# iden3/circom-witnesscalc

Measured on AMD Instinct MI355X. Metric: witnesses/sec, higher is better.
Workload: dtype u32

## Files before the change

### circom-witnesscalc_amd/__init__.py

```python
import ctypes
import os
import subprocess

import numpy as np

_HERE = os.path.dirname(os.path.abspath(__file__))
LIB_PATH = os.environ.get("CWC_LIB_PATH") or os.path.join(_HERE, "libcircom_witnesscalc_amd.so")
_lib = None


class GwStatus(ctypes.Structure):
    _fields_ = [("code", ctypes.c_int), ("error_msg", ctypes.c_void_p)]


class GraphInfo(ctypes.Structure):
    _fields_ = [(n, ctypes.c_uint64) for n in ("n_nodes", "n_op", "n_input_nodes", "n_const", "n_inputs",
                                                "n_witness", "depth", "algorithmic_bytes_per_set")]


class Timing(ctypes.Structure):
    _fields_ = [("tile_width", ctypes.c_uint32), ("n_launches", ctypes.c_uint32), ("n_bundles", ctypes.c_uint64),
                ("n_slots", ctypes.c_uint64), ("interp_ms", ctypes.c_float), ("pack_ms", ctypes.c_float),
                ("divider", ctypes.c_uint32), ("streams", ctypes.c_uint32)]


class ProgramStats(ctypes.Structure):
    _fields_ = [("tile_width", ctypes.c_uint32), ("divider", ctypes.c_uint32), ("streams", ctypes.c_uint32), ("n_classes", ctypes.c_uint32),
                ("n_bundles", ctypes.c_uint64), ("n_fused_nodes", ctypes.c_uint64), ("class_bundles", ctypes.c_uint64 * 16),
                ("class_nodes", ctypes.c_uint64 * 16), ("model_wave_cycles", ctypes.c_double), ("lanes_active_mean", ctypes.c_double),
                ("values_per_bundle_mean", ctypes.c_double), ("chain_floor_cycles", ctypes.c_double), ("n_scan_steps", ctypes.c_uint64), ("n_conv_products", ctypes.c_uint64)]


CLASS_NAMES = ["INPUT", "MUL", "LIN", "DIV", "CMPZ", "CMPS", "BIT", "IDIVMOD", "TERN", "DIVREQ", "DIVGET", "MULQ", "SYNC", "MULF", "SCAN"]


class E2eStats(ctypes.Structure):
    _fields_ = [("n_sets", ctypes.c_size_t), ("sub_batch", ctypes.c_size_t), ("parse_threads", ctypes.c_uint32), ("write_threads", ctypes.c_uint32),
                ("parse_seconds", ctypes.c_double), ("wait_for_drain_seconds", ctypes.c_double), ("total_seconds", ctypes.c_double),
                ("witness_bytes", ctypes.c_uint64), ("failed_sets", ctypes.c_uint64)]


class Handoff(ctypes.Structure):
    _fields_ = [("struct_size", ctypes.c_uint32), ("form", ctypes.c_uint32), ("hip_stream", ctypes.c_void_p), ("done_event", ctypes.c_void_p)]


FORM_CANONICAL, FORM_MONTGOMERY = 0, 1


class WitnessCalcError(RuntimeError):
    pass


def pinned_rows(shape):
    import weakref
    n = int(np.prod(shape))
    ptr = lib().gwb_host_alloc(n)
    if not ptr:
        raise WitnessCalcError("gwb_host_alloc(%d) failed" % n)
    buf = (ctypes.c_uint8 * max(n, 1)).from_address(ptr)
    weakref.finalize(buf, lib().gwb_host_free, ptr)
    return np.frombuffer(buf, dtype=np.uint8, count=n).reshape(shape)


EXPORTED_SYMBOLS = [
    "gw_calc_witness", "gwb_graph_load", "gwb_graph_free", "gwb_graph_info", "gwb_graph_serialize",
    "gwb_inputs_from_json", "gwb_set_tile_width", "gwb_calc_witness_batch_device", "gwb_calc_witness_batch_host",
    "gwb_last_timing", "gwb_wtns_size", "gwb_wtns_from_witness", "gwb_graph_export", "gwb_graph_import",
    "gwb_free_status", "gwb_profile_classes", "gwb_pick_tile_width", "gwb_inputs_from_json_batch", "gwb_wtns_save_batch",
    "gwb_host_alloc", "gwb_host_free", "gwb_timing_history", "gwb_calc_witness_batch_handoff", "gwb_ubench_modmul", "gwb_graph_pick_tile_width", "gwb_graph_broadcast",
    "gwb_builder_new", "gwb_builder_free", "gwb_builder_input", "gwb_builder_constant", "gwb_builder_uno", "gwb_builder_duo", "gwb_builder_tres",
    "gwb_builder_witness", "gwb_builder_input_signal", "gwb_builder_node_count", "gwb_builder_finish",
    "gwb_ubench_modmul_block", "gwb_program_stats", "gwb_calc_witness_json_to_wtns", "gwb_model_class_cycles",
    "gwb_graphgen_bigint_class", "gwb_graphgen_rsa_long_div_class", "gwb_graph_op_histogram",
    "gwb_kernel_source_hash", "gwb_pack_schedule", "gwb_pack_schedule_of_blob", "gwb_rccl_unique_id", "gwb_rccl_comm_init", "gwb_rccl_comm_ranks", "gwb_rccl_comm_destroy",
    "gwb_wave_census",
]


def build(verbose=False, diag=False):
    cmd = ["make", "-C", os.path.join(_HERE, "csrc"), "-j4"] + (["all", "diag"] if diag else [])
    if not verbose:
        cmd.insert(1, "-s")
    subprocess.check_call(cmd)
    subprocess.check_call(["make"] + ([] if verbose else ["-s"]) + ["-C", os.path.join(_HERE, "r1cs"), "-j4"])


DIAG_LIB_PATH = os.path.join(_HERE, "libcircom_witnesscalc_amd_diag.so")


def lib():
    global _lib
    if _lib is None:
        if not os.path.exists(LIB_PATH):
            raise WitnessCalcError("HIP extension %s is missing: run __graft_entry__.build() "
                                   "(there is no CPU fallback)" % LIB_PATH)
        try:
            import torch
        except ImportError:
            pass
        L = ctypes.CDLL(LIB_PATH)
        vp, sz, u32p = ctypes.c_void_p, ctypes.c_size_t, ctypes.POINTER(ctypes.c_uint32)
        stp = ctypes.POINTER(GwStatus)
        L.gw_calc_witness.restype = ctypes.c_int
        L.gw_calc_witness.argtypes = [ctypes.c_char_p, vp, sz, ctypes.POINTER(vp), ctypes.POINTER(sz), stp]
        L.gwb_graph_load.restype = ctypes.c_int
        L.gwb_graph_load.argtypes = [vp, sz, ctypes.POINTER(vp), stp]
        L.gwb_graph_free.argtypes = [vp]
        L.gwb_graph_info.argtypes = [vp, ctypes.POINTER(GraphInfo)]
        L.gwb_graph_serialize.argtypes = [vp, ctypes.POINTER(vp), ctypes.POINTER(sz), stp]
        L.gwb_inputs_from_json.argtypes = [vp, ctypes.c_char_p, vp, stp]
        L.gwb_set_tile_width.argtypes = [vp, ctypes.c_uint32]
        L.gwb_calc_witness_batch_device.argtypes = [vp, vp, sz, vp, vp, vp, stp]
        L.gwb_calc_witness_batch_host.argtypes = [vp, vp, sz, vp, vp, stp]
        L.gwb_last_timing.argtypes = [vp, ctypes.POINTER(Timing)]
        L.gwb_host_alloc.restype = ctypes.c_void_p
        L.gwb_host_alloc.argtypes = [sz]
        L.gwb_host_free.restype = None
        L.gwb_host_free.argtypes = [ctypes.c_void_p]
        L.gwb_timing_history.restype = ctypes.c_int
        L.gwb_timing_history.argtypes = [ctypes.c_void_p, sz, ctypes.c_void_p, ctypes.c_void_p, ctypes.POINTER(sz)]
        L.gwb_wtns_size.restype = sz
        L.gwb_wtns_size.argtypes = [sz]
        L.gwb_wtns_from_witness.argtypes = [vp, sz, vp]
        L.gwb_graph_export.argtypes = [vp, ctypes.c_uint32, ctypes.POINTER(vp), ctypes.POINTER(sz), stp]
        L.gwb_graph_import.argtypes = [vp, sz, ctypes.POINTER(vp), stp]
        L.gwb_free_status.argtypes = [stp]
        if hasattr(L, "gwb_graphgen_bigint_class"):
            L.gwb_graphgen_bigint_class.argtypes = [ctypes.c_uint32, ctypes.c_uint32, ctypes.c_uint32, ctypes.POINTER(vp), ctypes.POINTER(sz), stp]
            L.gwb_graphgen_rsa_long_div_class.argtypes = [ctypes.c_uint32, ctypes.c_uint32, ctypes.c_uint32, ctypes.c_int, ctypes.POINTER(vp), ctypes.POINTER(sz), stp]
            L.gwb_graph_op_histogram.argtypes = [vp, ctypes.POINTER(ctypes.c_uint64), sz]
        L.gwb_profile_classes.argtypes = [vp, vp, sz, vp, vp, vp, stp]
        if hasattr(L, "gwb_wave_census"):
            L.gwb_wave_census.argtypes = [vp, vp, sz, vp, vp, vp, sz, stp]
        L.gwb_inputs_from_json_batch.argtypes = [vp, ctypes.c_char_p, sz, vp, sz, ctypes.POINTER(sz), stp]
        L.gwb_wtns_save_batch.argtypes = [vp, sz, sz, ctypes.c_char_p, stp]
        L.gwb_calc_witness_batch_handoff.argtypes = [vp, vp, sz, vp, vp, ctypes.POINTER(Handoff), stp]
        L.gwb_ubench_modmul.restype = ctypes.c_double
        L.gwb_ubench_modmul.argtypes = [ctypes.c_uint32, ctypes.c_uint32]
        L.gwb_ubench_modmul_block.restype = ctypes.c_double
        L.gwb_model_class_cycles.restype = ctypes.c_double
        L.gwb_kernel_source_hash.restype = ctypes.c_char_p
        L.gwb_kernel_source_hash.argtypes = []
        L.gwb_model_class_cycles.argtypes = [ctypes.c_uint32]
        L.gwb_ubench_modmul_block.argtypes = [ctypes.c_uint32, ctypes.c_uint32]
        L.gwb_program_stats.argtypes = [vp, ctypes.c_uint32, ctypes.POINTER(ProgramStats)]
        if hasattr(L, "gwb_pack_schedule"):
            L.gwb_pack_schedule.argtypes = [vp, ctypes.c_uint32, vp, sz, vp, sz, u32p, u32p, u32p, stp]
            L.gwb_pack_schedule_of_blob.argtypes = [vp, sz, vp, sz, vp, sz, u32p, u32p, u32p, stp]
        L.gwb_calc_witness_json_to_wtns.argtypes = [vp, ctypes.c_char_p, sz, ctypes.c_char_p, sz, ctypes.POINTER(sz), vp, sz, ctypes.POINTER(E2eStats), stp]
        L.gwb_graph_pick_tile_width.restype = ctypes.c_uint32
        L.gwb_graph_pick_tile_width.argtypes = [vp, sz]
        L.gwb_pick_tile_width.restype = ctypes.c_uint32
        L.gwb_pick_tile_width.argtypes = [sz]
        u32 = ctypes.c_uint32
        L.gwb_builder_new.restype = vp
        L.gwb_builder_new.argtypes = []
        L.gwb_builder_free.restype = None
        L.gwb_builder_free.argtypes = [vp]
        for name, args in (("input", [u32]), ("constant", [ctypes.c_char_p, sz]), ("uno", [u32, u32]), ("duo", [u32, u32, u32]), ("tres", [u32, u32, u32, u32])):
            f = getattr(L, "gwb_builder_" + name)
            f.restype = u32
            f.argtypes = [vp] + args
        L.gwb_builder_witness.argtypes = [vp, u32]
        L.gwb_builder_input_signal.argtypes = [vp, ctypes.c_char_p, u32, u32]
        L.gwb_builder_node_count.restype = ctypes.c_uint64
        L.gwb_builder_node_count.argtypes = [vp]
        L.gwb_builder_finish.argtypes = [vp, ctypes.POINTER(vp), ctypes.POINTER(sz), stp]
        _lib = L
    return _lib


_libc = ctypes.CDLL(None)
_libc.free.argtypes = [ctypes.c_void_p]


def _take_status(st):
    msg = ctypes.string_at(st.error_msg).decode("utf-8", "replace") if st.error_msg else ""
    lib().gwb_free_status(ctypes.byref(st))
    return msg


def _check(rc, st):
    msg = _take_status(st)
    if rc != 0:
        raise WitnessCalcError(msg or "call failed")


def wtns_save_batch(witness, path_pattern):
    witness = np.ascontiguousarray(witness, dtype=np.uint8)
    st = GwStatus()
    rc = lib().gwb_wtns_save_batch(witness.ctypes.data, witness.shape[1], witness.shape[0], path_pattern.encode(), ctypes.byref(st))
    _check(rc, st)


def ubench_modmul(waves_per_simd=4, iters=2000, block=False):
    if block:
        return float(lib().gwb_ubench_modmul_block(waves_per_simd, iters))
    return float(lib().gwb_ubench_modmul(waves_per_simd, iters))


def kernel_source_hash():
    return lib().gwb_kernel_source_hash().decode()


def model_cycles():
    return {n: float(lib().gwb_model_class_cycles(c)) for c, n in enumerate(CLASS_NAMES)}


def graphgen_native(kind, **kw):
    out, n, st = ctypes.c_void_p(), ctypes.c_size_t(), GwStatus()
    L = lib()
    if kind == "bigint":
        rc = L.gwb_graphgen_bigint_class(int(kw.get("k", 8)), int(kw.get("n_bits", 64)), int(kw.get("rounds", 4)), ctypes.byref(out), ctypes.byref(n), ctypes.byref(st))
    elif kind == "rsa":
        rc = L.gwb_graphgen_rsa_long_div_class(int(kw.get("n", 121)), int(kw.get("k", 17)), int(kw.get("muls", 2)), 1 if kw.get("range_checks", True) else 0,
                                               ctypes.byref(out), ctypes.byref(n), ctypes.byref(st))
    else:
        raise ValueError(kind)
    _check(rc, st)
    data = ctypes.string_at(out.value, n.value)
    _libc.free(out)
    return data


def pick_tile_width(batch):
    return int(lib().gwb_pick_tile_width(batch))


def calc_witness_wtns(inputs_json, graph_data):
    if isinstance(inputs_json, str):
        inputs_json = inputs_json.encode("utf-8")
    graph_data = bytes(graph_data)
    out, n, st = ctypes.c_void_p(), ctypes.c_size_t(), GwStatus()
    rc = lib().gw_calc_witness(inputs_json, graph_data, len(graph_data), ctypes.byref(out), ctypes.byref(n),
                               ctypes.byref(st))
    _check(rc, st)
    data = ctypes.string_at(out.value, n.value)
    _libc.free(out)
    return data


def calc_witness(inputs_json, graph_data):
    w = calc_witness_wtns(inputs_json, graph_data)
    body = w[76:]
    return [int.from_bytes(body[i:i + 32], "little") for i in range(0, len(body), 32)]


def wtns_from_witness(witness):
    if not isinstance(witness, np.ndarray):
        witness = np.frombuffer(b"".join(int(x).to_bytes(32, "little") for x in witness), dtype=np.uint8)
    witness = np.ascontiguousarray(witness, dtype=np.uint8).reshape(-1, 32)
    n = witness.shape[0]
    out = np.zeros(lib().gwb_wtns_size(n), dtype=np.uint8)
    if lib().gwb_wtns_from_witness(witness.ctypes.data, n, out.ctypes.data) != 0:
        raise WitnessCalcError("gwb_wtns_from_witness failed")
    return out.tobytes()


class Graph:

    def __init__(self, graph_data=None, _handle=None):
        self._h = ctypes.c_void_p()
        if _handle is not None:
            self._h = _handle
        else:
            graph_data = bytes(graph_data)
            st = GwStatus()
            rc = lib().gwb_graph_load(graph_data, len(graph_data), ctypes.byref(self._h), ctypes.byref(st))
            _check(rc, st)
        info = GraphInfo()
        lib().gwb_graph_info(self._h, ctypes.byref(info))
        for name, _ in GraphInfo._fields_:
            setattr(self, name, int(getattr(info, name)))

    def close(self):
        if getattr(self, "_h", None) and _lib is not None:
            _lib.gwb_graph_free(self._h)
            self._h = None

    __del__ = close

    @classmethod
    def from_blob(cls, blob):
        blob = bytes(blob)
        h, st = ctypes.c_void_p(), GwStatus()
        rc = lib().gwb_graph_import(blob, len(blob), ctypes.byref(h), ctypes.byref(st))
        _check(rc, st)
        return cls(_handle=h)

    def op_histogram(self):
        h = (ctypes.c_uint64 * 24)()
        if lib().gwb_graph_op_histogram(self._h, h, 24) != 0:
            raise WitnessCalcError("gwb_graph_op_histogram failed")
        names = ["Mul", "Div", "Add", "Sub", "Pow", "Idiv", "Mod", "Eq", "Neq", "Lt", "Gt", "Leq", "Geq", "Land", "Lor", "Shl", "Shr", "Bor", "Band", "Bxor",
                 "Neg", "TernCond", "Input", "Const"]
        return dict(sorted(((nm, int(h[i])) for i, nm in enumerate(names) if h[i]), key=lambda kv: -kv[1]))

    def export_blob(self, tile_width):
        out, n, st = ctypes.c_void_p(), ctypes.c_size_t(), GwStatus()
        rc = lib().gwb_graph_export(self._h, tile_width, ctypes.byref(out), ctypes.byref(n), ctypes.byref(st))
        _check(rc, st)
        data = ctypes.string_at(out.value, n.value)
        _libc.free(out)
        return data

    def serialize(self):
        out, n, st = ctypes.c_void_p(), ctypes.c_size_t(), GwStatus()
        rc = lib().gwb_graph_serialize(self._h, ctypes.byref(out), ctypes.byref(n), ctypes.byref(st))
        _check(rc, st)
        data = ctypes.string_at(out.value, n.value)
        _libc.free(out)
        return data

    def pick_tile_width(self, batch):
        key = int(lib().gwb_graph_pick_tile_width(self._h, batch))
        if key == 0:
            raise WitnessCalcError("gwb_graph_pick_tile_width failed")
        return key

    def set_tile_width(self, t):
        if lib().gwb_set_tile_width(self._h, t) != 0:
            raise WitnessCalcError("tile width must be 0 or a power of two in 1..64")

    def inputs_from_json(self, inputs_json):
        if isinstance(inputs_json, str):
            inputs_json = inputs_json.encode("utf-8")
        row = np.zeros((self.n_inputs, 32), dtype=np.uint8)
        st = GwStatus()
        rc = lib().gwb_inputs_from_json(self._h, inputs_json, row.ctypes.data, ctypes.byref(st))
        _check(rc, st)
        return row

    def inputs_from_json_batch(self, text):
        if isinstance(text, str):
            text = text.encode("utf-8")
        n = ctypes.c_size_t()
        st = GwStatus()
        lib().gwb_inputs_from_json_batch(self._h, text, len(text), None, 0, ctypes.byref(n), ctypes.byref(st))
        msg = _take_status(st)
        if "rows buffer too small" not in msg and msg:
            raise WitnessCalcError(msg)
        rows = np.zeros((n.value, self.n_inputs, 32), dtype=np.uint8)
        st = GwStatus()
        rc = lib().gwb_inputs_from_json_batch(self._h, text, len(text), rows.ctypes.data, n.value, ctypes.byref(n), ctypes.byref(st))
        _check(rc, st)
        return rows

    def json_to_wtns(self, text, path_pattern, first_index=0, with_status=True):
        if isinstance(text, str):
            text = text.encode("utf-8")
        n = ctypes.c_size_t()
        cap = max(1, text.count(b"\n") + 1, text.count(b"{"))
        status = np.zeros(cap, dtype=np.uint32)
        es, st = E2eStats(), GwStatus()
        rc = lib().gwb_calc_witness_json_to_wtns(self._h, text, len(text), path_pattern.encode(), first_index, ctypes.byref(n),
                                                  status.ctypes.data if with_status else None, cap if with_status else 0,
                                                  ctypes.byref(es), ctypes.byref(st))
        _check(rc, st)
        return status[:n.value], {k: getattr(es, k) for k, _ in E2eStats._fields_}

    def calc_witness_batch(self, inputs, out=None):
        inputs = np.ascontiguousarray(inputs, dtype=np.uint8)
        b = inputs.shape[0]
        assert inputs.shape[1:] == (self.n_inputs, 32), inputs.shape
        if out is None:
            wit = np.empty((b, self.n_witness, 32), dtype=np.uint8)
        else:
            wit = out
            assert wit.dtype == np.uint8 and wit.shape == (b, self.n_witness, 32) and wit.flags["C_CONTIGUOUS"]
        status = np.zeros(b, dtype=np.uint32)
        st = GwStatus()
        rc = lib().gwb_calc_witness_batch_host(self._h, inputs.ctypes.data, b, wit.ctypes.data, status.ctypes.data,
                                               ctypes.byref(st))
        _check(rc, st)
        return wit, status

    def calc_witness_batch_device(self, d_inputs, d_witness, d_status, stream=None, montgomery=False, done_event=None):
        import torch
        b = d_inputs.shape[0]
        assert d_inputs.is_cuda and d_witness.is_cuda and d_status.is_cuda
        assert d_inputs.is_contiguous() and d_witness.is_contiguous() and d_status.is_contiguous()
        assert tuple(d_inputs.shape[1:]) == (self.n_inputs, 32) and tuple(d_witness.shape) == (b, self.n_witness, 32)
        s = stream if stream is not None else torch.cuda.current_stream()
        st = GwStatus()
        if montgomery or done_event is not None:
            if done_event is not None:
                done_event.record(s)
            h = Handoff(ctypes.sizeof(Handoff), FORM_MONTGOMERY if montgomery else FORM_CANONICAL, s.cuda_stream,
                        done_event.cuda_event if done_event is not None else None)
            rc = lib().gwb_calc_witness_batch_handoff(self._h, d_inputs.data_ptr(), b, d_witness.data_ptr(), d_status.data_ptr(),
                                                      ctypes.byref(h), ctypes.byref(st))
        else:
            rc = lib().gwb_calc_witness_batch_device(self._h, d_inputs.data_ptr(), b, d_witness.data_ptr(),
                                                     d_status.data_ptr(), s.cuda_stream, ctypes.byref(st))
        _check(rc, st)

    def timing_history(self, max_launches):
        a = np.zeros(max_launches, dtype=np.float32)
        b = np.zeros(max_launches, dtype=np.float32)
        n = ctypes.c_size_t(0)
        if lib().gwb_timing_history(self._h, max_launches, a.ctypes.data, b.ctypes.data, ctypes.byref(n)) != 0:
            raise WitnessCalcError("gwb_timing_history failed")
        return a[:n.value], b[:n.value]

    def profile_classes(self, d_inputs, d_witness, d_status):
        out = np.zeros(96, dtype=np.uint64)
        st = GwStatus()
        rc = lib().gwb_profile_classes(self._h, d_inputs.data_ptr(), d_inputs.shape[0], d_witness.data_ptr(),
                                       d_status.data_ptr(), out.ctypes.data, ctypes.byref(st))
        _check(rc, st)
        names = ["INPUT", "MUL", "LIN", "DIV", "CMPZ", "CMPS", "BIT", "IDIVMOD", "TERN", "DIVREQ", "DIVGET", "MULQ"]
        res = {n: tuple(int(x) for x in out[4 * i:4 * i + 4]) for i, n in enumerate(names)}
        res["MULF"] = tuple(int(x) for x in out[64:68])
        res["SCAN"] = tuple(int(x) for x in out[68:72])
        res["_scan_kinds"] = {k: tuple(int(x) for x in out[72 + 4 * i:76 + 4 * i]) for i, k in enumerate(("carry", "division", "convolution", "borrow", "comparison"))}
        res["_sections"] = {"MUL": tuple(int(x) for x in out[48:54]), "LIN": tuple(int(x) for x in out[56:62])}
        res["_issue_part"] = {"MUL": int(out[92]), "LIN": int(out[93])}
        res["_pack"] = {"cycles": int(out[94]), "passes": int(out[95])}
        n = int(out[63])
        res["_waves"] = {"n": n, "max_cycles": int(out[54]), "min_cycles": (1 << 40) - int(out[55]) if n else 0,
                         "mean_cycles": int(out[62]) // n if n else 0}
        return res

    def wave_census(self, d_inputs, d_witness, d_status):
        out = np.zeros(3 * 8192, dtype=np.uint64)
        st = GwStatus()
        rc = lib().gwb_wave_census(self._h, d_inputs.data_ptr(), d_inputs.shape[0], d_witness.data_ptr(),
                                   d_status.data_ptr(), out.ctypes.data, out.size, ctypes.byref(st))
        _check(rc, st)
        rec = out.reshape(-1, 3)
        idx = [i for i in range(rec.shape[0]) if rec[i, 1]]
        res = []
        for i in idx:
            w0 = int(rec[i, 0])
            role, wpw = (w0 >> 40) & 255, (w0 >> 48) & 255
            res.append({"workgroup": i // wpw, "wave": i % wpw, "xcc": (w0 >> 32) & 15, "se": (w0 >> 13) & 7, "sh": (w0 >> 12) & 1, "cu": (w0 >> 8) & 15, "simd": (w0 >> 4) & 3,
                        "divider": role & 1, "stream": (role >> 1) & 7, "has_tile": (role >> 4) & 1, "start": int(rec[i, 1]), "end": int(rec[i, 2])})
        return res

    def program_stats(self, key=0):
        ps = ProgramStats()
        if lib().gwb_program_stats(self._h, key, ctypes.byref(ps)) != 0:
            raise WitnessCalcError("gwb_program_stats: no such program")
        n = ps.n_classes
        return {"tile_width": ps.tile_width, "divider": ps.divider, "streams": ps.streams, "n_bundles": ps.n_bundles,
                "n_fused_nodes": ps.n_fused_nodes, "n_scan_steps": ps.n_scan_steps, "n_conv_products": ps.n_conv_products, "chain_floor_cycles": ps.chain_floor_cycles, "model_wave_cycles": ps.model_wave_cycles, "lanes_active_mean": ps.lanes_active_mean, "values_per_bundle_mean": ps.values_per_bundle_mean,
                "class_bundles": {CLASS_NAMES[c]: int(ps.class_bundles[c]) for c in range(n) if ps.class_bundles[c]},
                "class_nodes": {CLASS_NAMES[c]: int(ps.class_nodes[c]) for c in range(n) if ps.class_nodes[c]}}

    def pack_schedule(self, key):
        return _pack_schedule(lambda *a: lib().gwb_pack_schedule(self._h, key, *a))

    def last_timing(self):
        t = Timing()
        if lib().gwb_last_timing(self._h, ctypes.byref(t)) != 0:
            raise WitnessCalcError("gwb_last_timing failed")
        return {n: getattr(t, n) for n, _ in Timing._fields_}


def _pack_schedule(call):
    nw, nr, ni, st = ctypes.c_uint32(), ctypes.c_uint32(), ctypes.c_uint32(), GwStatus()
    _check(call(None, 0, None, 0, ctypes.byref(nw), ctypes.byref(nr), ctypes.byref(ni), ctypes.byref(st)), st)
    order, ready = np.zeros(nw.value, dtype=np.uint32), np.zeros(nr.value, dtype=np.uint32)
    _check(call(order.ctypes.data, order.size, ready.ctypes.data, ready.size, ctypes.byref(nw), ctypes.byref(nr), ctypes.byref(ni), ctypes.byref(st)), st)
    return order, ready, int(ni.value)


def pack_schedule_of_blob(blob):
    blob = bytes(blob)
    return _pack_schedule(lambda *a: lib().gwb_pack_schedule_of_blob(blob, len(blob), *a))


R1CS_LIB_PATH = os.environ.get("CWC_R1CS_LIB_PATH") or os.path.join(_HERE, "libcwc_r1cs.so")
R1CS_SATISFIED = 0xFFFFFFFF
_r1cs_lib = None


class R1csInfo(ctypes.Structure):
    _fields_ = [(n, ctypes.c_uint32) for n in ("n_wires", "n_pub_out", "n_pub_in", "n_prv_in", "n_constraints")] + \
               [(n, ctypes.c_uint64) for n in ("n_labels", "n_factors_a", "n_factors_b", "n_factors_c")]


class R1csQapInfo(ctypes.Structure):
    _fields_ = [("n_rows", ctypes.c_uint64), ("domain_power", ctypes.c_uint32), ("domain_size", ctypes.c_uint64),
                ("workspace_bytes_per_row", ctypes.c_uint64)]


class ZkeyInfo(ctypes.Structure):
    _fields_ = [("n_vars", ctypes.c_uint32), ("n_public", ctypes.c_uint32), ("domain_size", ctypes.c_uint32), ("n_coefs", ctypes.c_uint64)]


class PtauInfo(ctypes.Structure):
    _fields_ = [("power", ctypes.c_uint32), ("ceremony_power", ctypes.c_uint32), ("prepared", ctypes.c_uint32),
                ("n_contributions", ctypes.c_uint32)]


def r1cs_lib():
    global _r1cs_lib
    if _r1cs_lib is None:
        if not os.path.exists(R1CS_LIB_PATH):
            raise WitnessCalcError("R1CS library %s is missing: run __graft_entry__.build()" % R1CS_LIB_PATH)
        try:
            import torch
        except ImportError:
            pass
        L = ctypes.CDLL(R1CS_LIB_PATH)
        vp, sz, u32 = ctypes.c_void_p, ctypes.c_size_t, ctypes.c_uint32
        stp = ctypes.POINTER(GwStatus)
        L.gwb_r1cs_load.argtypes = [vp, sz, ctypes.POINTER(vp), stp]
        L.gwb_r1cs_free.restype = None
        L.gwb_r1cs_free.argtypes = [vp]
        L.gwb_r1cs_info.argtypes = [vp, ctypes.POINTER(R1csInfo)]
        L.gwb_r1cs_set_tile_width.argtypes = [vp, u32]
        L.gwb_r1cs_check_batch_device.argtypes = [vp, vp, sz, sz, u32, vp, vp, vp, stp]
        L.gwb_r1cs_check_batch_host.argtypes = [vp, vp, sz, sz, vp, vp, stp]
        L.gwb_r1cs_check_wtns.argtypes = [vp, vp, sz, vp, vp, stp]
        L.gwb_r1cs_qap_info.argtypes = [vp, ctypes.POINTER(R1csQapInfo), stp]
        L.gwb_r1cs_qap_batch_device.argtypes = [vp, vp, sz, sz, u32, vp, u32, vp, stp]
        L.gwb_r1cs_qap_batch_host.argtypes = [vp, vp, sz, sz, vp, u32, stp]
        L.gwb_r1cs_qap_wtns.argtypes = [vp, vp, sz, vp, u32, stp]
        L.gwb_r1cs_qap_time_phases.argtypes = [vp, ctypes.c_int]
        L.gwb_r1cs_qap_phase_ms.argtypes = [vp, ctypes.POINTER(ctypes.c_float)]
        L.gwb_r1cs_modmul_rate.argtypes = [ctypes.POINTER(ctypes.c_double)]
        L.gwb_zkey_load.argtypes = [vp, sz, ctypes.POINTER(vp), stp]
        L.gwb_zkey_free.restype = None
        L.gwb_zkey_free.argtypes = [vp]
        L.gwb_zkey_info.argtypes = [vp, ctypes.POINTER(ZkeyInfo)]
        L.gwb_groth16_prove_batch_device.argtypes = [vp, vp, vp, sz, sz, u32, vp, vp, vp, stp]
        L.gwb_groth16_prove_batch_host.argtypes = [vp, vp, vp, sz, sz, vp, vp, stp]
        L.gwb_groth16_prove_wtns.argtypes = [vp, vp, vp, sz, vp, vp, stp]
        L.gwb_groth16_time_phases.argtypes = [vp, ctypes.c_int]
        L.gwb_groth16_phase_ms.argtypes = [vp, ctypes.POINTER(ctypes.c_float)]
        L.gwb_zkey_qap_info.argtypes = [vp, ctypes.POINTER(R1csQapInfo), stp]
        L.gwb_zkey_qap_batch_device.argtypes = [vp, vp, sz, sz, u32, vp, u32, vp, stp]
        L.gwb_zkey_qap_batch_host.argtypes = [vp, vp, sz, sz, vp, u32, stp]
        L.gwb_zkey_set_tile_width.argtypes = [vp, u32]
        L.gwb_zkey_check_r1cs.argtypes = [vp, vp, stp]
        L.gwb_g16vk_from_zkey.argtypes = [vp, ctypes.POINTER(vp), stp]
        L.gwb_g16vk_load.argtypes = [vp, sz, u32, ctypes.POINTER(vp), stp]
        L.gwb_g16vk_info.argtypes = [vp, ctypes.POINTER(ctypes.c_uint32)]
        L.gwb_g16vk_points.argtypes = [vp, vp, sz]
        L.gwb_g16vk_alphabeta.argtypes = [vp, vp, stp]
        L.gwb_g16vk_free.restype = None
        L.gwb_g16vk_free.argtypes = [vp]
        L.gwb_groth16_verify_batch_device.argtypes = [vp, vp, vp, sz, sz, vp, vp, stp]
        L.gwb_groth16_verify_batch_host.argtypes = [vp, vp, vp, sz, sz, vp, stp]
        L.gwb_bn254_pairing_batch_device.argtypes = [vp, vp, sz, vp, vp, stp]
        L.gwb_groth16_setup.argtypes = [vp, vp, ctypes.POINTER(vp), ctypes.POINTER(sz), stp]
        L.gwb_groth16_setup_free.restype = None
        L.gwb_groth16_setup_free.argtypes = [vp]
        L.gwb_bn254_gen_mul_batch_device.argtypes = [vp, sz, u32, vp, vp, stp]
        L.gwb_groth16_setup_phase_ms.argtypes = [ctypes.POINTER(ctypes.c_float)]
        L.gwb_ptau_info.argtypes = [vp, sz, ctypes.POINTER(PtauInfo), stp]
        L.gwb_ptau_check.argtypes = [vp, sz, u32, u32, stp]
        L.gwb_groth16_setup_ptau.argtypes = [vp, vp, sz, vp, u32, ctypes.POINTER(vp), ctypes.POINTER(sz), stp]
        L.gwb_bn254_point_idft_batch_device.argtypes = [vp, u32, u32, vp, vp, stp]
        L.gwb_groth16_setup_ptau_phase_ms.argtypes = [ctypes.POINTER(ctypes.c_float)]
        L.gwb_bn254_g2_check_batch_device.argtypes = [vp, sz, u32, u32, vp, vp, stp]
        L.gwb_zkey_check_g2.argtypes = [vp, stp]
        L.gwb_zkey_check_wtns.argtypes = [vp, vp, sz, stp]
        L.gwb_ptau_check_g2.argtypes = [vp, sz, u32, u32, stp]
        L.gwb_groth16_contribute.argtypes = [vp, sz, ctypes.c_char_p, vp, ctypes.POINTER(vp), ctypes.POINTER(sz), vp, stp]
        L.gwb_groth16_contribute_phase_ms.argtypes = [ctypes.POINTER(ctypes.c_float)]
        L.gwb_zkey_verify_contributions.argtypes = [vp, sz, vp, ctypes.POINTER(sz), stp]
        L.gwb_zkey_verify_step.argtypes = [vp, sz, vp, sz, vp, stp]
        L.gwb_zkey_contributions.argtypes = [vp, sz, ctypes.POINTER(vp), ctypes.POINTER(sz), stp]
        L.gwb_blake2b512.restype = None
        L.gwb_blake2b512.argtypes = [vp, sz, vp]
        L.gwb_zkey_contribution_challenge.restype = None
        L.gwb_zkey_contribution_challenge.argtypes = [vp, vp]
        L.gwb_bn254_g1_scale_batch_device.argtypes = [vp, sz, vp, vp, vp, stp]
        L.gwb_bn254_g1_lincomb128_device.argtypes = [vp, vp, sz, vp, vp, stp]
        _r1cs_lib = L
    return _r1cs_lib


def _r1cs_check(rc, st):
    msg = ctypes.string_at(st.error_msg).decode("utf-8", "replace") if st.error_msg else ""
    if st.error_msg:
        _libc.free(st.error_msg)
    if rc != 0:
        raise WitnessCalcError(msg or "call failed")


def modmul_rate():
    rate = ctypes.c_double()
    if r1cs_lib().gwb_r1cs_modmul_rate(ctypes.byref(rate)) != 0:
        raise WitnessCalcError("gwb_r1cs_modmul_rate failed")
    return rate.value


def _qap_info(h, src):
    info = R1csQapInfo()
    st = GwStatus()
    rc = getattr(r1cs_lib(), "gwb_%s_qap_info" % src)(h, ctypes.byref(info), ctypes.byref(st))
    _r1cs_check(rc, st)
    return {n: int(getattr(info, n)) for n, _ in R1csQapInfo._fields_}


def _qap_batch(h, src, witness_rows, montgomery_out):
    if isinstance(witness_rows, tuple):
        witness_rows = witness_rows[0]
    w = np.ascontiguousarray(witness_rows, dtype=np.uint8)
    assert w.ndim == 3 and w.shape[2] == 32, w.shape
    b = w.shape[0]
    out = np.zeros((b, _qap_info(h, src)["domain_size"], 32), dtype=np.uint8)
    st = GwStatus()
    rc = getattr(r1cs_lib(), "gwb_%s_qap_batch_host" % src)(h, w.ctypes.data, w.shape[1], b, out.ctypes.data,
                                                            FORM_MONTGOMERY if montgomery_out else FORM_CANONICAL, ctypes.byref(st))
    _r1cs_check(rc, st)
    return out


def _qap_batch_device(h, src, d_witness, stream, montgomery, montgomery_out):
    import torch
    assert d_witness.is_cuda and d_witness.is_contiguous() and d_witness.dtype == torch.uint8
    assert d_witness.dim() == 3 and d_witness.shape[2] == 32, tuple(d_witness.shape)
    b = d_witness.shape[0]
    n = _qap_info(h, src)["domain_size"]
    s = stream if stream is not None else torch.cuda.current_stream(d_witness.device)
    out = torch.empty((b, n, 32), dtype=torch.uint8, device=d_witness.device)
    st = GwStatus()
    with torch.cuda.device(d_witness.device):
        rc = getattr(r1cs_lib(), "gwb_%s_qap_batch_device" % src)(h, d_witness.data_ptr(), d_witness.shape[1], b,
                                                                  FORM_MONTGOMERY if montgomery else FORM_CANONICAL, out.data_ptr(),
                                                                  FORM_MONTGOMERY if montgomery_out else FORM_CANONICAL, s.cuda_stream,
                                                                  ctypes.byref(st))
    _r1cs_check(rc, st)
    if b:
        out.record_stream(s)
    return out


class R1cs:

    def __init__(self, data):
        self._h = ctypes.c_void_p()
        data = bytes(data)
        st = GwStatus()
        rc = r1cs_lib().gwb_r1cs_load(data, len(data), ctypes.byref(self._h), ctypes.byref(st))
        _r1cs_check(rc, st)
        info = R1csInfo()
        r1cs_lib().gwb_r1cs_info(self._h, ctypes.byref(info))
        self.info = {n: int(getattr(info, n)) for n, _ in R1csInfo._fields_}

    def close(self):
        if getattr(self, "_h", None) and _r1cs_lib is not None:
            _r1cs_lib.gwb_r1cs_free(self._h)
            self._h = None

    __del__ = close

    def set_tile_width(self, t):
        if r1cs_lib().gwb_r1cs_set_tile_width(self._h, t) != 0:
            raise WitnessCalcError("tile width must be 0 or a power of two in 1..64")

    def check_batch(self, witness_rows):
        if isinstance(witness_rows, tuple):
            witness_rows = witness_rows[0]
        w = np.ascontiguousarray(witness_rows, dtype=np.uint8)
        assert w.ndim == 3 and w.shape[2] == 32, w.shape
        b = w.shape[0]
        first = np.zeros(b, dtype=np.uint32)
        nfail = np.zeros(b, dtype=np.uint32)
        st = GwStatus()
        rc = r1cs_lib().gwb_r1cs_check_batch_host(self._h, w.ctypes.data, w.shape[1], b, first.ctypes.data, nfail.ctypes.data, ctypes.byref(st))
        _r1cs_check(rc, st)
        return first, nfail

    def check_batch_device(self, d_witness, stream=None, montgomery=False):
        import torch
        assert d_witness.is_cuda and d_witness.is_contiguous() and d_witness.dtype == torch.uint8
        assert d_witness.dim() == 3 and d_witness.shape[2] == 32, tuple(d_witness.shape)
        b = d_witness.shape[0]
        s = stream if stream is not None else torch.cuda.current_stream(d_witness.device)
        first = torch.empty(b, dtype=torch.int32, device=d_witness.device)
        nfail = torch.empty(b, dtype=torch.int32, device=d_witness.device)
        st = GwStatus()
        with torch.cuda.device(d_witness.device):
            rc = r1cs_lib().gwb_r1cs_check_batch_device(self._h, d_witness.data_ptr(), d_witness.shape[1], b,
                                                        FORM_MONTGOMERY if montgomery else FORM_CANONICAL, first.data_ptr(),
                                                        nfail.data_ptr(), s.cuda_stream, ctypes.byref(st))
        _r1cs_check(rc, st)
        return first, nfail

    def check_wtns(self, wtns):
        wtns = bytes(wtns)
        first, nfail = ctypes.c_uint32(), ctypes.c_uint32()
        st = GwStatus()
        rc = r1cs_lib().gwb_r1cs_check_wtns(self._h, wtns, len(wtns), ctypes.byref(first), ctypes.byref(nfail), ctypes.byref(st))
        _r1cs_check(rc, st)
        return int(first.value), int(nfail.value)

    def qap_info(self):
        return _qap_info(self._h, "r1cs")

    def qap_batch(self, witness_rows, montgomery_out=False):
        return _qap_batch(self._h, "r1cs", witness_rows, montgomery_out)

    def qap_batch_device(self, d_witness, stream=None, montgomery=False, montgomery_out=False):
        return _qap_batch_device(self._h, "r1cs", d_witness, stream, montgomery, montgomery_out)

    def qap_time_phases(self, on=True):
        if r1cs_lib().gwb_r1cs_qap_time_phases(self._h, 1 if on else 0) != 0:
            raise WitnessCalcError("gwb_r1cs_qap_time_phases failed")

    def qap_phase_ms(self):
        ms = (ctypes.c_float * 4)()
        if r1cs_lib().gwb_r1cs_qap_phase_ms(self._h, ms) != 0:
            raise WitnessCalcError("no QAP phase times (qap_time_phases not on, or no QAP call yet)")
        return dict(zip(("evaluation", "inverse_outer", "fused_inner", "forward_outer"), (float(x) for x in ms)))

    def qap_wtns(self, wtns, montgomery_out=False):
        wtns = bytes(wtns)
        h = np.zeros((self.qap_info()["domain_size"], 32), dtype=np.uint8)
        st = GwStatus()
        rc = r1cs_lib().gwb_r1cs_qap_wtns(self._h, wtns, len(wtns), h.ctypes.data,
                                          FORM_MONTGOMERY if montgomery_out else FORM_CANONICAL, ctypes.byref(st))
        _r1cs_check(rc, st)
        return h



GROTH16_PROOF_BYTES = 256
GROTH16_PHASES = ("witness_map", "scalars_sort", "g1_msms", "g2_msm", "assembly")


def _rs_array(rs, b):
    if rs is None:
        return None
    if isinstance(rs, np.ndarray):
        a = np.ascontiguousarray(rs, dtype=np.uint8)
    else:
        a = np.frombuffer(b"".join(int(x).to_bytes(32, "little") for pair in rs for x in pair), dtype=np.uint8).copy()
    assert a.size == b * 64, "rs must hold [batch][2][32 B]"
    return a


def _dec(b):
    return str(int.from_bytes(bytes(b), "little"))


def proof_json(proof):
    p = bytes(proof)
    c = [_dec(p[32 * k:32 * k + 32]) for k in range(8)]
    z = lambda lo, hi: "1" if any(p[lo:hi]) else "0"
    return {"pi_a": [c[0], c[1], z(0, 64)], "pi_b": [[c[2], c[3]], [c[4], c[5]], [z(64, 192), "0"]],
            "pi_c": [c[6], c[7], z(192, 256)], "protocol": "groth16", "curve": "bn128"}


class Groth16:

    def __init__(self, zkey_bytes, r1cs=None, check_g2=False):
        self._h = ctypes.c_void_p()
        self.r1cs = r1cs
        data = bytes(zkey_bytes)
        st = GwStatus()
        rc = r1cs_lib().gwb_zkey_load(data, len(data), ctypes.byref(self._h), ctypes.byref(st))
        _r1cs_check(rc, st)
        info = ZkeyInfo()
        r1cs_lib().gwb_zkey_info(self._h, ctypes.byref(info))
        self.info = {n: int(getattr(info, n)) for n, _ in ZkeyInfo._fields_}
        if check_g2:
            self.check_g2()

    def close(self):
        if getattr(self, "_h", None) and _r1cs_lib is not None:
            _r1cs_lib.gwb_zkey_free(self._h)
            self._h = None

    __del__ = close

    def _r1cs_handle(self):
# ... 577 lines not shown
```

### circom-witnesscalc_amd/csrc/kernels.hip

```cpp
#include <hip/hip_runtime.h>
#include <stdlib.h>

#include "fr_gfx950.hpp"
#include "scan_gfx950.hpp"
#include "program_dev.h"

namespace cwc {

__device__ __forceinline__ Fr fr_from_u4(const uint4& lo, const uint4& hi) {
    return Fr{{lo.x, lo.y, lo.z, lo.w, hi.x, hi.y, hi.z, hi.w}};
}

__device__ __forceinline__ bool wave_any(bool p) { return __ballot(p) != 0ull; }

struct InterpDims {
    uint32_t n_bundles, n_slots, n_inputs, batch, n_const, n_div_requests, trash_off;
    const uint32_t* div_lanes;
    uint32_t n_streams, stream_first[MAX_STREAMS], stream_count[MAX_STREAMS], stream_div_requests[MAX_STREAMS], stream_cref_first[MAX_STREAMS];
    uint4* pack_out;
    const uint2* pack_entries;
    const uint32_t* pack_ready;
    uint32_t n_inline, pack_mont, n_witness;
};
static const uint32_t ST_DIVIDER_TIMEOUT = 0x80000000u;
static const uint32_t ST_SYNC_TIMEOUT = 0x40000000u;

__device__ __forceinline__ bool mbox_wait(const volatile uint32_t* seq, uint32_t need) {
    for (uint32_t spins = 0; spins < (1u << 22); ++spins) {
        if (*seq >= need) return true;
        __builtin_amdgcn_s_sleep(8);
    }
    return false;
}
__device__ __noinline__ bool post_wait(uint32_t* word, uint32_t need) {
#pragma nounroll
    for (uint32_t spins = 0; spins < (1u << 22); ++spins) {
        if (__hip_atomic_load(word, __ATOMIC_ACQUIRE, __HIP_MEMORY_SCOPE_AGENT) >= need) return true;
        __builtin_amdgcn_s_sleep(8);
    }
    return false;
}
typedef uint32_t u32x4 __attribute__((ext_vector_type(4)));
typedef int i32x4 __attribute__((ext_vector_type(4)));
typedef __attribute__((address_space(3))) char lds_char;

__device__ __forceinline__ void dma16(uint32_t lds_addr, uint32_t voff, const i32x4& rsrc, uint32_t soff) {
    asm volatile("s_mov_b32 m0, %0\n\ts_nop 0\n\tbuffer_load_dwordx4 %1, %2, %3 offen lds"
                 :: "s"(lds_addr), "v"(voff), "s"(rsrc), "s"(soff) : "memory");
}
__device__ __forceinline__ i32x4 make_rsrc_words(const void* base, uint32_t bytes) {
    const uint64_t a = (uint64_t)base;
    return i32x4{(int)(uint32_t)a, (int)((uint32_t)(a >> 32) & 0xffffu), (int)bytes, 0x00020000};
}

template <int T, bool PROF, int W, int PACK, int MODE = 0>
__global__ __launch_bounds__((W > 0 ? (W + 1) * PACK : PACK) * 64) void interp_kernel(const uint32_t* __restrict__ hdr, const uint4* __restrict__ recs,
                                                    const uint32_t* __restrict__ crefs, InterpDims p, WsTable wst,
                                                    const uint4* __restrict__ inputs, uint32_t* __restrict__ status,
                                                    unsigned long long* __restrict__ prof) {
    constexpr int G = 64 / T;
    constexpr bool M2 = MODE == 2 || MODE == 3, WIDE = MODE == 3;
    constexpr uint32_t HI = 16u * T;
    constexpr bool DIVIDER = W > 0;
    constexpr uint32_t NW = (W > 0 ? (uint32_t)W : 1u) * (uint32_t)PACK;
    constexpr uint32_t WD = W > 0 ? (uint32_t)W : 1u;
    constexpr uint32_t AREA = lds_area_bytes((uint32_t)W, LDS_BYTES);
    constexpr uint32_t ML = mbox_lanes((uint32_t)W), MB = mbox_bytes((uint32_t)W);
    const uint32_t batch = p.batch;
    const uint32_t lane = threadIdx.x & 63u;
    const uint32_t wave = (uint32_t)__builtin_amdgcn_readfirstlane((int)(threadIdx.x >> 6));
    const uint32_t n_tiles = (batch + T - 1) / T;
    const uint32_t t = lane % T;
    const uint32_t j = (G == 1) ? 0u : lane / T;
    const uint32_t NS = p.n_streams;
    const uint32_t stream = wave < NW ? wave % NS : 0u;
    const uint32_t tile_raw = blockIdx.x * (NW / NS) + (wave < NW ? wave : 0u) / NS;
    const uint32_t tile = tile_raw < n_tiles ? tile_raw : n_tiles - 1;
    const uint32_t set = tile * T + t;
    const uint32_t set_c = set < batch ? set : batch - 1;
    [[maybe_unused]] auto census_slot = [&]() -> unsigned long long* {
        const uint32_t wv = blockIdx.x * (blockDim.x >> 6) + wave;
        return lane == 0 && wv < CENSUS_MAX_WAVES ? prof + PROF_WORDS + CENSUS_WORDS * wv : nullptr;
    };
    if constexpr (PROF) {
        if (unsigned long long* c = census_slot()) {
            const uint32_t w_of = wave < NW ? wave : (wave - NW) * WD;
            const uint32_t has_tile = blockIdx.x * (NW / NS) + w_of / NS < n_tiles ? 1u : 0u;
            const unsigned long long role = (wave >= NW ? 1u : 0u) | (w_of % NS) << 1 | has_tile << 4 | (blockDim.x >> 6) << 8;
            constexpr int HWREG_HW_ID = 4 | 31 << 11, HWREG_XCC_ID = 20 | 31 << 11;
            c[0] = (unsigned long long)__builtin_amdgcn_s_getreg(HWREG_HW_ID) | (unsigned long long)(__builtin_amdgcn_s_getreg(HWREG_XCC_ID) & 15u) << 32 | role << 40;
            c[1] = __builtin_amdgcn_s_memtime();
        }
    }
    const uint64_t tile_bytes = ws_tile_bytes(p.n_const, p.n_slots, T);
    const uint32_t chunk = tile / wst.tiles_per_chunk, tile_in_chunk = tile % wst.tiles_per_chunk;
    char* tile_base = reinterpret_cast<char*>(wst.base[chunk]) + (uint64_t)tile_in_chunk * tile_bytes;
    const __amdgpu_buffer_rsrc_t rsrc = __builtin_amdgcn_make_buffer_rsrc(tile_base, 0, (int)(uint32_t)tile_bytes, 0x00020000);
    const i32x4 rsrc_rec = make_rsrc_words(recs, (p.n_bundles + REC_AHEAD) * (uint32_t)G * 16u);
    uint32_t* const sync_words = reinterpret_cast<uint32_t*>(tile_base + ws_sync_offset(p.n_const, p.n_slots, T));
    static_assert(NW + PACK <= 16, "sequence words: 64 bytes");
    __shared__ uint4 lds[(NW * AREA + (DIVIDER ? NW * MB + 64u : 0u)) / 16];
    const uint32_t area = wave * AREA;
    const uint32_t lds0 = (uint32_t)(uintptr_t)(lds_char*)(char*)lds + area;
    const uint32_t t16 = 16u * t, lane16 = 16u * lane, j16 = 16u * j;
    char* const ldsb = reinterpret_cast<char*>(lds) + area;
    char* const mbox_all = reinterpret_cast<char*>(lds) + NW * AREA;
    char* const mbox = mbox_all + (wave < NW ? wave : 0u) * MB;
    volatile uint32_t* const seq = reinterpret_cast<volatile uint32_t*>(mbox_all + NW * MB);
    if (DIVIDER || NW > 1) {
        if (DIVIDER && threadIdx.x < NW + (uint32_t)PACK) seq[threadIdx.x] = 0;
        if (NS > 1 && wave < NW && stream == 0 && lane < MAX_STREAMS && tile_raw < n_tiles) {
            __hip_atomic_store(sync_words + lane, 0u, __ATOMIC_RELAXED, __HIP_MEMORY_SCOPE_AGENT);
            __builtin_amdgcn_fence(__ATOMIC_RELEASE, "agent");
        }
        if (wave < NW && stream == 0 && j == 0 && tile_raw < n_tiles && set < batch) status[set] = 0;
        __syncthreads();
    } else {
        if (j == 0 && tile_raw < n_tiles && set < batch) status[set] = 0;
    }
    if (DIVIDER) {
        if (wave >= NW) {
            const uint32_t first_w = (wave - NW) * WD, first_tile = blockIdx.x * (NW / NS) + first_w / NS;
            if (first_tile >= n_tiles) return;
            const uint32_t n_active = NS > 1 ? 1u : n_tiles - first_tile < WD ? n_tiles - first_tile : WD;
            char* const mbox_d = mbox_all + first_w * MB;
            const uint32_t n_requests = NS > 1 ? p.stream_div_requests[first_w % NS] : p.n_div_requests;
            uint32_t div_lanes_base = 0;
            for (uint32_t q = 0; NS > 1 && q < first_w % NS; ++q) div_lanes_base += p.stream_div_requests[q];
            [[maybe_unused]] uint32_t pk_next = 0;
            [[maybe_unused]] uint2 pk_e0 = make_uint2(0u, 0u), pk_e1 = pk_e0;
            [[maybe_unused]] unsigned long long pk_cycles = 0, pk_passes = 0;
            const bool inl = W == 1 && NS == 1 && p.n_inline > 0;
            const char* const pk_tile = reinterpret_cast<const char*>(wst.base[first_tile / wst.tiles_per_chunk]) + (uint64_t)(first_tile % wst.tiles_per_chunk) * tile_bytes;
            const uint32_t pk_set = first_tile * T + t;
            auto pk_load = [&](const uint2& e, uint4& lo, uint4& hi) {
                const uint32_t ref = e.y & ~REF_CANON;
                const uint32_t slot = (ref & REF_CONST) ? (ref & ~REF_CONST) : p.n_const + ref;
                const uint4* q = reinterpret_cast<const uint4*>(pk_tile) + (size_t)slot * (2 * T);
                lo = q[t];
                hi = q[T + t];
            };
            auto pk_store = [&](const uint2& e, const uint4& lo, const uint4& hi, uint32_t limit) {
                const bool valid = pk_next + j < limit && pk_set < batch, canon = (e.y & REF_CANON) != 0;
                const Fr v = fr_from_u4(lo, hi);
                Fr c = v;
                if (p.pack_mont) {
                    if (wave_any(both(valid, canon))) c = u256_select(canon, fr_mul(v, fr_r2()), v);
                } else {
                    if (wave_any(both(valid, !canon))) c = u256_select(canon, v, fr_from_mont(v));
                }
                if (valid) {
                    uint4* o = p.pack_out + ((size_t)pk_set * p.n_witness + e.x) * 2;
                    o[0] = make_uint4(c.v[0], c.v[1], c.v[2], c.v[3]);
                    o[1] = make_uint4(c.v[4], c.v[5], c.v[6], c.v[7]);
                }
            };
            auto pk_run = [&](uint32_t limit, uint32_t need) {
                if (pk_next >= limit) return;
                unsigned long long t0 = 0;
                if (PROF) t0 = __builtin_amdgcn_s_memtime();
                uint4 lo, hi;
                pk_load(pk_e0, lo, hi);
                for (;;) {
                    const uint32_t nb = pk_next + (uint32_t)G;
                    const bool more = nb < limit && seq[first_w] < need;
                    uint4 lo1 = lo, hi1 = hi;
                    if (more) pk_load(pk_e1, lo1, hi1);
                    const uint2 e2 = p.pack_entries[nb + (uint32_t)G + j];
                    pk_store(pk_e0, lo, hi, limit);
                    pk_next = nb;
                    pk_e0 = pk_e1;
                    pk_e1 = e2;
                    if (PROF) ++pk_passes;
                    if (!more) break;
                    lo = lo1;
                    hi = hi1;
                }
                if (PROF) pk_cycles += __builtin_amdgcn_s_memtime() - t0;
            };
            if constexpr (W == 1) {
                if (inl) {
                    pk_e0 = p.pack_entries[j];
                    pk_e1 = p.pack_entries[(uint32_t)G + j];
                }
            }
            for (uint32_t k = 0; k < n_requests; ++k) {
                if constexpr (W == 1) {
                    if (inl) {
                        const uint32_t lim = p.pack_ready[k] < p.n_inline ? p.pack_ready[k] : p.n_inline;
                        pk_run(lim / (uint32_t)G * (uint32_t)G, k + 1);
                    }
                }
                bool ok = true;
                for (uint32_t w = 0; w < n_active; ++w) ok = ok && mbox_wait(seq + first_w + w, k + 1);
                if (!ok) {
                    if (first_tile * T + t < batch) atomicOr(&status[first_tile * T + t], ST_DIVIDER_TIMEOUT);
                    break;
                }
                __builtin_amdgcn_fence(__ATOMIC_ACQUIRE, "workgroup");
                const uint32_t lanes_k = p.div_lanes[div_lanes_base + k];
                const uint32_t total = n_active * lanes_k;
                for (uint32_t g0 = 0; g0 < total; g0 += 64u) {
                    const uint32_t g = g0 + lane;
                    const bool valid = g < total;
                    const uint32_t w = valid ? g / lanes_k : 0u, i = valid ? g % lanes_k : 0u;
                    char* mb = mbox_d + w * MB + 16u * i;
                    const uint4* qa = reinterpret_cast<const uint4*>(mb);
                    const uint4* qb = reinterpret_cast<const uint4*>(mb + 32u * ML);
                    Fr a = fr_from_u4(qa[0], qa[ML]), b = fr_from_u4(qb[0], qb[ML]);
                    if (!valid) b = fr_zero();
                    const Fr inv = fr_inv(b);
                    const Fr r = u256_select(u256_is_zero(b), fr_zero(), fr_mul(a, inv));
                    if (valid) {
                        uint4* qr = reinterpret_cast<uint4*>(mb);
                        qr[0] = make_uint4(r.v[0], r.v[1], r.v[2], r.v[3]);
                        qr[ML] = make_uint4(r.v[4], r.v[5], r.v[6], r.v[7]);
                    }
                }
                __builtin_amdgcn_fence(__ATOMIC_RELEASE, "workgroup");
                if (lane == 0) seq[wave] = k + 1;
            }
            if constexpr (W == 1) {
                if (inl) {
                    pk_run(p.pack_ready[n_requests] < p.n_inline ? p.pack_ready[n_requests] : p.n_inline, 0xffffffffu);
                    if (PROF && lane == 0 && first_tile % 64u == 0) {
                        atomicAdd(&prof[94], pk_cycles);
                        atomicAdd(&prof[95], pk_passes);
                    }
                }
            }
            if constexpr (PROF) {
                if (unsigned long long* c = census_slot()) c[2] = __builtin_amdgcn_s_memtime();
            }
            return;
        }
    }
    if (tile_raw >= n_tiles) return;
    uint32_t div_seq = 0;
    uint32_t n_posts = 0, n_waits = 0;
    uint32_t cref_row = p.stream_cref_first[stream];

    auto ld = [&](uint32_t off) -> Fr {
        const u32x4 lo = __builtin_amdgcn_raw_buffer_load_b128(rsrc, (int)off, 0, 0);
        const u32x4 hi = __builtin_amdgcn_raw_buffer_load_b128(rsrc, (int)off + (int)HI, 0, 0);
        return Fr{{lo.x, lo.y, lo.z, lo.w, hi.x, hi.y, hi.z, hi.w}};
    };
    auto ld_lds = [&](uint32_t addr) -> Fr {
        const uint4* q = reinterpret_cast<const uint4*>(ldsb + addr);
        const uint4 lo = q[0], hi = q[LDS_HALF_BYTES / 16];
        return fr_from_u4(lo, hi);
    };
    auto ld_rec2 = [&](uint32_t bundle, uint32_t half) -> uint2 {
        return *reinterpret_cast<const uint2*>(ldsb + LDS_REC_OFF + (bundle % REC_AHEAD) * REC_BYTES + lane16 + 8u * half);
    };
    const uint32_t B0 = p.stream_first[stream], NBND = B0 + p.stream_count[stream];
    if (NBND == B0) return;
    auto clampb = [&](uint32_t b) { return b < NBND ? b : NBND - 1; };
    auto stage_rec = [&](uint32_t bundle) {
        dma16(lds0 + LDS_REC_OFF + (bundle % REC_AHEAD) * REC_BYTES, j16, rsrc_rec, bundle * (uint32_t)G * 16u);
    };
    constexpr uint32_t DMA_BIAS = 3u * LDS_HALF_BYTES;
    const i32x4 rsrc_dma = make_rsrc_words(tile_base - DMA_BIAS, (uint32_t)tile_bytes + DMA_BIAS);
    const uint32_t dma_soff0 = DMA_BIAS, dma_soff1 = DMA_BIAS + HI - LDS_HALF_BYTES, dma_soff2 = DMA_BIAS - 2u * LDS_HALF_BYTES,
                   dma_soff3 = DMA_BIAS + HI - 3u * LDS_HALF_BYTES;
    static_assert(LDS_HALF_BYTES == 1024, "instruction offsets below are written out");
    auto stage_operands = [&](uint32_t bundle, const uint2& offs) {
        const uint32_t s = lds0 + LDS_STAGE_OFF + (bundle % OPND_AHEAD) * STAGE_BYTES;
        const uint32_t ao = offs.x + t16, bo = offs.y + t16;
        asm volatile("s_mov_b32 m0, %0\n\ts_nop 0\n\t"
                     "buffer_load_dwordx4 %1, %3, %4 offen lds\n\t"
                     "buffer_load_dwordx4 %1, %3, %5 offen offset:1024 lds\n\t"
                     "buffer_load_dwordx4 %2, %3, %6 offen offset:2048 lds\n\t"
                     "buffer_load_dwordx4 %2, %3, %7 offen offset:3072 lds"
                     :: "s"(s), "v"(ao), "v"(bo), "s"(rsrc_dma), "s"(dma_soff0), "s"(dma_soff1), "s"(dma_soff2), "s"(dma_soff3) : "memory");
    };
    uint32_t err_bits = 0;
    Fr pv = fr_p();
#pragma unroll
    for (int i = 0; i < 8; ++i) asm volatile("" : "+v"(pv.v[i]));
    constexpr bool COOP = (uint32_t)T <= COOP_MAX_T;
    const uint32_t cq = lane & 3u, cv = lane >> 2;
    const uint32_t t16c = 16u * (cv % T);
    const uint32_t coop_chunk = (cq >> 1) * LDS_HALF_BYTES + (cq & 1u) * 8u;
    const uint32_t coop_ring_off = 16u * cv + coop_chunk;
    const uint32_t coop_dst_off = t16c + (cq >> 1) * HI + (cq & 1u) * 8u;
    uint32_t nq0 = cq == 0 ? CWC_P0 : cq == 1 ? CWC_P2 : cq == 2 ? CWC_P4 : CWC_P6;
    uint32_t nq1 = cq == 0 ? CWC_P1 : cq == 1 ? CWC_P3 : cq == 2 ? CWC_P5 : CWC_P7;
    asm volatile("" : "+v"(nq0), "+v"(nq1));
    const uint32_t trash_doff = p.trash_off | t16;
    constexpr int C_PROF = 12;
    unsigned long long pf[C_PROF][2], psec[2][7] = {{0, 0, 0, 0, 0, 0, 0}, {0, 0, 0, 0, 0, 0, 0}};
    unsigned long long pf_fused[2] = {0, 0};
    unsigned long long pf_scan[5][2] = {{0, 0}, {0, 0}, {0, 0}, {0, 0}, {0, 0}};
    if (PROF) {
#pragma unroll
        for (int c = 0; c < C_PROF; ++c) pf[c][0] = pf[c][1] = 0;
    }
#define CWC_STAMP(var) unsigned long long var = 0; if (PROF) asm volatile("s_memtime %0\n\ts_waitcnt lgkmcnt(0)" : "=s"(var)::"memory")
#define CWC_SHADOW_ISSUE()                                                                                                                  \
    stage_rec(b + 4);                                                                                                                       \
    __builtin_amdgcn_raw_buffer_store_b128(u32x4{r_prev.v[0], r_prev.v[1], r_prev.v[2], r_prev.v[3]}, rsrc, (int)doff_prev, 0, 0);          \
    __builtin_amdgcn_raw_buffer_store_b128(u32x4{r_prev.v[4], r_prev.v[5], r_prev.v[6], r_prev.v[7]}, rsrc, (int)doff_prev + (int)HI, 0, 0)
#define CWC_NEXT_HEADER(var)                                                                                                                 \
    asm volatile("s_mov_b32 %0, xnack_mask_lo\n\ts_load_dword xnack_mask_lo, %1, %2" : "=&s"(var) : "s"(hdr), "s"(hdr_off_n2) : "memory"); \
    hdr_off_n2 += 4u

    static_assert(OPND_AHEAD == 2 && REC_AHEAD == 4, "the counted waits below are written for this pipeline depth");
#pragma unroll
    for (uint32_t q = 0; q < REC_AHEAD; ++q) stage_rec(B0 + q);
    asm volatile("s_waitcnt vmcnt(0)" ::: "memory");
    stage_operands(B0, ld_rec2(B0, 0));
    stage_operands(B0 + 1, ld_rec2(B0 + 1, 0));
    uint2 rec_hi = ld_rec2(B0, 1);
    uint2 rec_hi_n1 = ld_rec2(B0 + 1, 1);
    uint32_t h_cur = hdr[B0], h_n1 = hdr[clampb(B0 + 1)];
    asm volatile("s_waitcnt vmcnt(0)" ::: "memory");
    const unsigned long long t_wave0 = PROF ? __builtin_amdgcn_s_memtime() : 0ull;
    asm volatile("s_load_dword xnack_mask_lo, %0, %1\n\ts_waitcnt lgkmcnt(0)" :: "s"(hdr), "s"(4u * B0 + 8u) : "memory");
    uint32_t hdr_off_n2 = 4u * B0 + 12u;
    Fr r_prev = fr_zero();
    uint32_t doff_prev = trash_doff;
    for (uint32_t b = B0; b < NBND; ++b) {
        CWC_STAMP(st0);
        const uint32_t h = h_cur;
        asm volatile("s_waitcnt vmcnt(7)" ::: "memory");
        CWC_STAMP(st1);
        if constexpr (COOP) {
            uint32_t cls_q = h & HDR_CLASS_MASK;
            asm volatile("" : "+s"(cls_q));
            static_assert(C_MULQ == 11 && C_SYNC == 12 && C_MULF == 13 && C_SCAN == 14 && C_COUNT == 15, "one compare (class >= C_MULQ) leads to the narrow classes");
            const bool narrow_cls = MODE == 1 ? cls_q >= C_MULQ : cls_q == C_MULQ;
            if (M2 ? __builtin_expect(narrow_cls, 0) : narrow_cls) {
            if (MODE != 1 || cls_q == C_MULQ) {
                const uint32_t la = rec_hi.y + (t16c | (t16c << 16));
                const Fr a_op = ld_lds(la & 0xffffu);
                const uint2 bq = *reinterpret_cast<const uint2*>(ldsb + (la >> 16) + coop_chunk);
                const uint2 aq = *reinterpret_cast<const uint2*>(ldsb + (la & 0xffffu) + coop_chunk);
                const uint4 rec_full_n2 = *reinterpret_cast<const uint4*>(ldsb + LDS_REC_OFF + ((b + 2) % REC_AHEAD) * REC_BYTES + lane16);
                const uint2 rec_n2 = make_uint2(rec_full_n2.x, rec_full_n2.y), rec_hi_n2 = make_uint2(rec_full_n2.z, rec_full_n2.w);
                CWC_SHADOW_ISSUE();
                asm volatile("s_waitcnt lgkmcnt(0)" :: "v"(a_op.v[0]), "v"(a_op.v[4]), "v"(bq.x), "v"(aq.x), "v"(rec_n2.x), "v"(rec_hi_n2.x) : "memory");
                uint32_t h_n2;
                CWC_NEXT_HEADER(h_n2);
                CWC_STAMP(st2);
                stage_operands(b + 2, rec_n2);
                CWC_STAMP(st3);
                uint32_t out[2];
                if (h & (HDR_LIN_ADD | HDR_LIN_SUB)) {
                    fr_mul_coop4r(a_op, aq.x, aq.y, bq.x, bq.y, nq0, nq1, rec_hi.x & CTRL_SUB_MASK, out);
                } else {
                    fr_mul_coop4(a_op, bq.x, bq.y, nq0, nq1, out);
                }
                CWC_STAMP(st4);
                *reinterpret_cast<uint2*>(ldsb + LDS_RING_OFF + (b % RING_BUNDLES) * RING_SLOT_BYTES + coop_ring_off) = make_uint2(out[0], out[1]);
                {
                    typedef uint32_t u32x2 __attribute__((ext_vector_type(2)));
                    __builtin_amdgcn_raw_buffer_store_b64(u32x2{out[0], out[1]}, rsrc, (int)((rec_hi.x & ~CTRL_MASK) + coop_dst_off), 0, 0);
                }
                doff_prev = trash_doff;
                rec_hi = rec_hi_n1;
                rec_hi_n1 = rec_hi_n2;
                h_cur = h_n1;
                h_n1 = h_n2;
                __builtin_amdgcn_fence(__ATOMIC_ACQ_REL, "wavefront");
                if (PROF) {
                    asm volatile("s_waitcnt lgkmcnt(0)" ::: "memory");
                    const unsigned long long t_now = __builtin_amdgcn_s_memtime();
                    pf[C_MULQ][0] += t_now - st0;
                    pf[C_MULQ][1] += 1;
                    (void)st2; (void)st3; (void)st4;
                }
                continue;
            }
            if constexpr (MODE == 1 && (uint32_t)T <= COOP_FUSE_MAX_T) {
            if (cls_q == C_MULF) {
                constexpr int QP_MAIN = T == 1 ? 0xA0  : 0x00 , QP_EXTRA = T == 1 ? 0xF5  : 0xAA ;
                const uint32_t mx = (uint32_t)__builtin_amdgcn_mov_dpp((int)rec_hi.x, QP_MAIN, 0xf, 0xf, false);
                const uint32_t my = (uint32_t)__builtin_amdgcn_mov_dpp((int)rec_hi.y, QP_MAIN, 0xf, 0xf, false);
                const uint32_t xx = (uint32_t)__builtin_amdgcn_mov_dpp((int)rec_hi.x, QP_EXTRA, 0xf, 0xf, false);
                const uint32_t xy = (uint32_t)__builtin_amdgcn_mov_dpp((int)rec_hi.y, QP_EXTRA, 0xf, 0xf, false);
                const uint32_t la = my + (t16c | (t16c << 16)), lx = xy + (t16c | (t16c << 16));
                const Fr a_op = ld_lds(la & 0xffffu);
                const uint2 bq = *reinterpret_cast<const uint2*>(ldsb + (la >> 16) + coop_chunk);
                const Fr x2_full = ld_lds(lx & 0xffffu);
                const uint2 x2q = *reinterpret_cast<const uint2*>(ldsb + (lx & 0xffffu) + coop_chunk);
                const uint2 x3q = *reinterpret_cast<const uint2*>(ldsb + (lx >> 16) + coop_chunk);
                const uint4 rec_full_n2 = *reinterpret_cast<const uint4*>(ldsb + LDS_REC_OFF + ((b + 2) % REC_AHEAD) * REC_BYTES + lane16);
                const uint2 rec_n2 = make_uint2(rec_full_n2.x, rec_full_n2.y), rec_hi_n2 = make_uint2(rec_full_n2.z, rec_full_n2.w);
                CWC_SHADOW_ISSUE();
                asm volatile("s_waitcnt lgkmcnt(0)" :: "v"(a_op.v[0]), "v"(a_op.v[4]), "v"(bq.x), "v"(x2_full.v[0]), "v"(x2_full.v[4]), "v"(x2q.x), "v"(x3q.x), "v"(rec_n2.x), "v"(rec_hi_n2.x) : "memory");
                uint32_t h_n2;
                CWC_NEXT_HEADER(h_n2);
                stage_operands(b + 2, rec_n2);
                uint32_t out[2];
                fr_mul_coop4(a_op, bq.x, bq.y, nq0, nq1, out);
                const uint32_t op2 = mx & CTRL_SUB_MASK, op3 = xx & CTRL_SUB_MASK;
                if (h & HDR_F_S2MUL) {
                    uint32_t o2[2];
                    fr_mul_coop4(x2_full, out[0], out[1], nq0, nq1, o2);
                    out[0] = op2 == FOP_MUL ? o2[0] : out[0];
                    out[1] = op2 == FOP_MUL ? o2[1] : out[1];
                }
                auto lin_stage = [&](uint32_t op, const uint2& xq) {
                    const bool rs = op == FOP_RSUB;
                    uint32_t o[2];
                    fr_addsub_coop4(rs ? xq.x : out[0], rs ? xq.y : out[1], rs ? out[0] : xq.x, rs ? out[1] : xq.y, nq0, nq1, op == FOP_ADD ? 0u : 1u, o);
                    out[0] = op >= FOP_ADD ? o[0] : out[0];
                    out[1] = op >= FOP_ADD ? o[1] : out[1];
                };
                if (h & HDR_F_S2LIN) lin_stage(op2, x2q);
                if (h & HDR_F_S3LIN) lin_stage(op3, x3q);
                *reinterpret_cast<uint2*>(ldsb + LDS_RING_OFF + (b % RING_BUNDLES) * RING_SLOT_BYTES + coop_ring_off) = make_uint2(out[0], out[1]);
                {
                    typedef uint32_t u32x2 __attribute__((ext_vector_type(2)));
                    __builtin_amdgcn_raw_buffer_store_b64(u32x2{out[0], out[1]}, rsrc, (int)((mx & ~CTRL_MASK) + coop_dst_off), 0, 0);
                }
                doff_prev = trash_doff;
                rec_hi = rec_hi_n1;
                rec_hi_n1 = rec_hi_n2;
                h_cur = h_n1;
                h_n1 = h_n2;
                __builtin_amdgcn_fence(__ATOMIC_ACQ_REL, "wavefront");
                if (PROF) {
                    asm volatile("s_waitcnt lgkmcnt(0)" ::: "memory");
                    const unsigned long long t_now = __builtin_amdgcn_s_memtime();
                    pf_fused[0] += t_now - st0;
                    pf_fused[1] += 1;
                }
                continue;
            }
            }
            }
        }
        const uint32_t ctrl = rec_hi.x & CTRL_MASK;
        const uint32_t doff = (rec_hi.x & ~CTRL_MASK) | t16;
        const uint32_t la = rec_hi.y + (t16 | (t16 << 16));
        const Fr a_op = ld_lds(la & 0xffffu), b_op = ld_lds(la >> 16);
        const uint4 rec_full_n2 = *reinterpret_cast<const uint4*>(ldsb + LDS_REC_OFF + ((b + 2) % REC_AHEAD) * REC_BYTES + lane16);
        const uint2 rec_n2 = make_uint2(rec_full_n2.x, rec_full_n2.y), rec_hi_n2 = make_uint2(rec_full_n2.z, rec_full_n2.w);
        CWC_SHADOW_ISSUE();
        unsigned long long st_iss = 0;
        if (PROF) st_iss = __builtin_amdgcn_s_memtime();
        uint32_t h_n2;
        unsigned long long st2 = 0, st3 = 0;
        auto wait_and_stage = [&]() {
            asm volatile("s_waitcnt lgkmcnt(0)" :: "v"(a_op.v[0]), "v"(a_op.v[4]), "v"(b_op.v[0]), "v"(b_op.v[4]), "v"(rec_n2.x), "v"(rec_hi_n2.x) : "memory");
            CWC_NEXT_HEADER(h_n2);
            if (PROF) asm volatile("s_memtime %0\n\ts_waitcnt lgkmcnt(0)" : "=s"(st2)::"memory");
            stage_operands(b + 2, rec_n2);
            if (PROF) asm volatile("s_memtime %0\n\ts_waitcnt lgkmcnt(0)" : "=s"(st3)::"memory");
        };

        const uint32_t cls = h & HDR_CLASS_MASK;
        uint32_t cls_hot = cls, cls_hot2 = cls;
        asm volatile("" : "+s"(cls_hot));
        asm volatile("" : "+s"(cls_hot2));
        const bool active = (ctrl & CTRL_ACTIVE) != 0;
        const uint32_t sub = ctrl & CTRL_SUB_MASK;
        auto finish = [&](const Fr& r) {
            CWC_STAMP(st4);
            r_prev = r;
            doff_prev = doff;
            {
                uint4* q = reinterpret_cast<uint4*>(ldsb + LDS_RING_OFF + (b % RING_BUNDLES) * RING_SLOT_BYTES + lane16);
                q[0] = make_uint4(r.v[0], r.v[1], r.v[2], r.v[3]);
                q[LDS_HALF_BYTES / 16] = make_uint4(r.v[4], r.v[5], r.v[6], r.v[7]);
            }
            rec_hi = rec_hi_n1;
            rec_hi_n1 = rec_hi_n2;
            h_cur = h_n1;
            h_n1 = h_n2;
            __builtin_amdgcn_fence(__ATOMIC_ACQ_REL, "wavefront");
            if (PROF) {
                asm volatile("s_waitcnt lgkmcnt(0)" ::: "memory");
                const unsigned long long t_now = __builtin_amdgcn_s_memtime();
    #pragma unroll
                for (int c = 0; c < C_PROF; ++c)
                    if (cls == (uint32_t)c) {
                        pf[c][0] += t_now - st0;
                        pf[c][1] += 1;
                    }
                if (M2 && cls == C_SCAN) {
                    pf_fused[0] += t_now - st0;
                    pf_fused[1] += 1;
                    const int kind = (h & HDR_SCAN_CONV) ? 2 : (h & HDR_SCAN_BORROW) ? 3 : (h & HDR_SCAN_LEX) ? 4 : (h & HDR_SCAN_DIV) ? 1 : 0;
#pragma unroll
                    for (int q = 0; q < 5; ++q)
                        if (kind == q) {
                            pf_scan[q][0] += t_now - st0;
                            pf_scan[q][1] += 1;
                        }
                }
                if (cls == C_MUL || cls == C_LIN) {
                    unsigned long long* q = psec[cls == C_MUL ? 0 : 1];
                    q[0] += st1 - st0;
                    q[1] += st2 - st1;
                    q[2] += st3 - st2;
                    q[3] += st4 - st3;
                    q[4] += t_now - st4;
                    q[5] += 1;
                    q[6] += st_iss - st1;
                }
            }
        };
        Fr r;
        auto one_out = [&]() -> Fr { return (h & HDR_OUT_CANON) ? Fr{{1u, 0u, 0u, 0u, 0u, 0u, 0u, 0u}} : fr_one(); };
        if (cls_hot2 == C_LIN) {
            wait_and_stage();
            if (!(h & HDR_LIN_SUB)) {
                r = fr_add_wave(a_op, b_op, pv);
            } else if (!(h & HDR_LIN_ADD)) {
                r = fr_sub_wave(a_op, b_op, pv);
            } else {
                const unsigned long long subm = __ballot(sub == SUB_SUB);
                r = fr_addsub_wave(a_op, b_op, pv, sub == SUB_SUB ? ~0u : 0u, subm, ~subm);
            }
            finish(r);
            continue;
        }
        wait_and_stage();
        if (__builtin_expect(cls_hot == C_MUL, WIDE ? 0 : 1)) {
            if constexpr (M2) {
                if (h & HDR_MUL_CC) {
                    auto limb_product = [&](const Fr& x, const Fr& y) -> Fr {
                        const uint64_t p00 = (uint64_t)x.v[0] * y.v[0], p01 = (uint64_t)x.v[0] * y.v[1], p10 = (uint64_t)x.v[1] * y.v[0], p11 = (uint64_t)x.v[1] * y.v[1];
                        const uint64_t m1 = (p00 >> 32) + (uint32_t)p01 + (uint32_t)p10;
                        const uint64_t m2 = (m1 >> 32) + (p01 >> 32) + (p10 >> 32) + (uint32_t)p11;
                        Fr z = fr_zero();
                        z.v[0] = (uint32_t)p00;
                        z.v[1] = (uint32_t)m1;
                        z.v[2] = (uint32_t)m2;
                        z.v[3] = (uint32_t)((m2 >> 32) + (p11 >> 32));
                        return z;
                    };
                    const uint32_t hi_a = a_op.v[2] | a_op.v[3] | a_op.v[4] | a_op.v[5] | a_op.v[6] | a_op.v[7], hi_b = b_op.v[2] | b_op.v[3] | b_op.v[4] | b_op.v[5] | b_op.v[6] | b_op.v[7];
                    if (!wave_any((hi_a | hi_b) != 0u)) {
                        r = limb_product(a_op, b_op);
                    } else if (WIDE && !wave_any(((a_op.v[3] | b_op.v[3]) >> 30 | a_op.v[4] | a_op.v[5] | a_op.v[6] | a_op.v[7] | b_op.v[4] | b_op.v[5] | b_op.v[6] | b_op.v[7]) != 0u)) {
                        uint32_t z[8] = {0, 0, 0, 0, 0, 0, 0, 0};
#pragma unroll
                        for (int i = 0; i < 4; ++i) {
                            uint32_t carry = 0;
#pragma unroll
                            for (int jj = 0; jj < 4; ++jj) {
                                const uint64_t t = (uint64_t)a_op.v[i] * b_op.v[jj] + z[i + jj] + carry;
                                z[i + jj] = (uint32_t)t;
                                carry = (uint32_t)(t >> 32);
                            }
                            z[i + 4] = carry;
                        }
#pragma unroll
                        for (int k = 0; k < 8; ++k) r.v[k] = z[k];
                    } else {
                        Fr na, nb;
                        (void)u256_sub(na, fr_p(), a_op);
                        (void)u256_sub(nb, fr_p(), b_op);
                        const bool a_neg = hi_a != 0u, b_neg = hi_b != 0u;
                        const Fr ma = u256_select(a_neg, na, a_op), mb = u256_select(b_neg, nb, b_op);
                        if (!wave_any((ma.v[2] | ma.v[3] | ma.v[4] | ma.v[5] | ma.v[6] | ma.v[7] | mb.v[2] | mb.v[3] | mb.v[4] | mb.v[5] | mb.v[6] | mb.v[7]) != 0u)) {
                            const Fr z = limb_product(ma, mb);
                            Fr nz;
                            (void)u256_sub(nz, fr_p(), z);
                            r = u256_select(both(a_neg != b_neg, !u256_is_zero(z)), nz, z);
                        } else {
                            r = fr_mul_wave(fr_mul_wave(a_op, fr_r2(), pv), b_op, pv);
                        }
                    }
                    finish(r);
                    continue;
                }
            }
            r = fr_mul_wave(a_op, b_op, pv);
            if ((h & (HDR_LIN_ADD | HDR_LIN_SUB)) == (HDR_LIN_ADD | HDR_LIN_SUB)) {
                const unsigned long long subm = __ballot(sub == SUB_SUB);
                r = u256_select(sub <= SUB_SUB, fr_addsub_wave(a_op, b_op, pv, sub == SUB_SUB ? ~0u : 0u, subm, ~subm), r);
            } else if (h & HDR_LIN_ADD) {
                r = u256_select(sub == SUB_ADD, fr_add_wave(a_op, b_op, pv), r);
            } else if (h & HDR_LIN_SUB) {
                r = u256_select(sub == SUB_SUB, fr_sub_wave(a_op, b_op, pv), r);
            }
            finish(r);
            continue;
        }
        if constexpr (M2 && (uint32_t)T <= SCAN_MAX_T) {
            uint32_t cls_scan = cls;
            asm volatile("" : "+s"(cls_scan));
            if (WIDE ? __builtin_expect(cls_scan == C_SCAN, 1) : (cls_scan == C_SCAN)) {
                r = fr_zero();
                if constexpr (M2 && (uint32_t)T <= SCAN_MAX_T) {
                    if (h & HDR_SCAN_CONV) {
                        const uint32_t k = (h >> HDR_SCAN_ITER_SHIFT) + 1u;
                        const bool holds_y = active && lane < k * (uint32_t)T;
                        if (!wave_any(both(active, (a_op.v[2] | a_op.v[3] | a_op.v[4] | a_op.v[5] | a_op.v[6] | a_op.v[7] | b_op.v[2] | b_op.v[3] | b_op.v[4] | b_op.v[5] | b_op.v[6] | b_op.v[7]) != 0u))) {
                            uint32_t col[5];
                            conv_limb_columns<T>(k, lane, ((uint64_t)a_op.v[1] << 32) | a_op.v[0], holds_y ? (((uint64_t)b_op.v[1] << 32) | b_op.v[0]) : 0ull, col);
#pragma unroll
                            for (int w = 0; w < 5; ++w) r.v[w] = col[w];
                        } else {
                            Fr yy = u256_select(holds_y, b_op, fr_zero());
                            for (uint32_t i = 0; i < k; ++i) {
                                Fr xi;
#pragma unroll
                                for (int w = 0; w < 8; ++w) {
                                    if constexpr (T == 1) {
                                        xi.v[w] = (uint32_t)__builtin_amdgcn_readlane((int)a_op.v[w], (int)i);
                                    } else {
                                        const uint32_t e = (uint32_t)__builtin_amdgcn_readlane((int)a_op.v[w], (int)(2 * i)), o = (uint32_t)__builtin_amdgcn_readlane((int)a_op.v[w], (int)(2 * i + 1));
                                        xi.v[w] = (lane & 1u) ? o : e;
                                    }
                                }
                                r = fr_add_wave(r, fr_mul_wave(fr_mul_wave(xi, fr_r2(), pv), yy, pv), pv);
#pragma unroll
                                for (int w = 0; w < 8; ++w) yy.v[w] = wave_shr_lanes<T>(yy.v[w]);
                            }
                        }
                        finish(r);
                        continue;
                    }
                    constexpr int QP_OUT = T == 1 ? 0xA0  : 0x44 , QP_ACC = T == 1 ? 0xF5  : 0xEE ;
                    constexpr int D = 2 * T;
                    const uint32_t sh = (h >> HDR_SCAN_SHIFT_SHIFT) & 0xffu, iters = (h >> HDR_SCAN_ITER_SHIFT) + 1u;
                    const bool start = (sub & SCAN_START) != 0, role_acc = (sub & SCAN_ROLE_ACC) != 0;
                    const Fr x = fr_quad_perm<QP_OUT>(a_op), acc0 = fr_quad_perm<QP_OUT>(b_op);
                    if (WIDE && (h & (HDR_SCAN_BORROW | HDR_SCAN_LEX))) {
                        const Fr y = fr_quad_perm<QP_ACC>(a_op);
                        const bool seg = start || !active;
                        const uint32_t a0 = both(both(start, active), !u256_is_zero(acc0)) ? 1u : 0u;
                        auto less = [](const Fr& a, const Fr& b) {
// ... 282 lines not shown
                const Fr x = (h & HDR_A_CANON) ? a_op : fr_from_mont(a_op), y = (h & HDR_B_CANON) ? b_op : fr_from_mont(b_op);
                auto less = [](const Fr& a, const Fr& b) {
                    Fr t;
                    const uint32_t borrow = u256_sub(t, a, b);
                    if constexpr (M2) asm volatile("" ::"v"(t.v[7]));
                    return borrow != 0;
                };
                bool lt, gt;
                bool limb_sized = false;
                if constexpr (M2) limb_sized = !wave_any(both(active, (x.v[4] | x.v[5] | x.v[6] | x.v[7] | y.v[4] | y.v[5] | y.v[6] | y.v[7]) != 0u));
                if (M2 && limb_sized) {
                    uint32_t d[4], bw = 0;
#pragma unroll
                    for (int k = 0; k < 4; ++k) d[k] = sbb32(x.v[k], y.v[k], bw);
                    lt = bw != 0u;
                    gt = both(bw == 0u, (d[0] | d[1] | d[2] | d[3]) != 0u);
                } else {
                    const bool xn = less(fr_half(), x), yn = less(fr_half(), y);
                    const bool same = xn == yn, xy = less(x, y), yx = less(y, x);
                    lt = same ? xy : xn;
                    gt = same ? yx : yn;
                }
                const bool v = either(either(both(sub == SUB_LT, lt), both(sub == SUB_GT, gt)), either(both(sub == SUB_LEQ, !gt), both(both(sub != SUB_LT, both(sub != SUB_GT, sub != SUB_LEQ)), !lt)));
                r = u256_select(v, one_out(), fr_zero());
                break;
            }
            case C_BIT: {
                const Fr x = (h & HDR_A_CANON) ? a_op : fr_from_mont(a_op);
                const uint32_t kx = rec_hi.y >> 20;
                const bool is_x = sub == SUB_BITX;
                if (h & HDR_BITX_ALL) {
                    const Fr e = u256_shr(x, kx);
                    r = u256_select((e.v[0] & 1u) != 0u, one_out(), fr_zero());
                    break;
                }
                const Fr y = (h & HDR_B_CANON) ? b_op : fr_from_mont(b_op);
                auto bit_result = [&](const Fr& d) -> Fr {
                    if (h & HDR_OUT_CANON) return d;
                    const bool small = both(d.v[0] < 2u, (d.v[1] | d.v[2] | d.v[3] | d.v[4] | d.v[5] | d.v[6] | d.v[7]) == 0u);
                    if (wave_any(!small)) return fr_mul_wave(d, fr_r2(), pv);
                    return u256_select(d.v[0] != 0u, fr_one(), fr_zero());
                };
                if (h & (HDR_BIT_ALL_SHR | HDR_BIT_ALL_BAND)) {
                    Fr d;
#pragma unroll
                    for (int i = 0; i < 8; ++i) d.v[i] = x.v[i] & y.v[i];
                    if (h & HDR_BIT_ALL_SHR) {
                        const bool big = either((y.v[1] | y.v[2] | y.v[3] | y.v[4] | y.v[5] | y.v[6] | y.v[7]) != 0u, y.v[0] >= 254u);
                        const Fr sh = u256_select(big, fr_zero(), u256_shr(x, big ? 0u : y.v[0]));
                        d = u256_select(sub == SUB_SHR, sh, d);
                    }
                    r = bit_result(d);
                    break;
                }
                uint32_t hi_or = 0;
#pragma unroll
                for (int i = 1; i < 8; ++i) hi_or |= y.v[i];
                const bool big = either(hi_or != 0u, y.v[0] >= 254u);
                const uint32_t n = is_x ? kx : big ? 0u : y.v[0];
                const bool shifts = either(either(sub == SUB_SHL, sub == SUB_SHR), is_x);
                Fr d = u256_shr(x, n);
                if (wave_any(sub == SUB_SHL)) d = u256_select(sub == SUB_SHL, u256_shl(x, n), d);
                d = u256_select(both(big, !is_x), fr_zero(), d);
                d.v[0] &= is_x ? 1u : 0xffffffffu;
#pragma unroll
                for (int i = 1; i < 8; ++i) d.v[i] = is_x ? 0u : d.v[i];
                {
                    const bool over = both(sub == SUB_SHL, !u256_lt(d, fr_p()));
                    err_bits |= both(over, active) ? ST_SHL_OVERFLOW : 0u;
                    d = u256_select(over, fr_zero(), d);
                }
                {
                    const uint32_t m_and = sub == SUB_BAND ? 0xffffffffu : 0u, m_or = sub == SUB_BAND ? 0u : 0xffffffffu, m_xor = (sub == SUB_BAND || sub == SUB_BOR) ? 0u : 0xffffffffu;
                    Fr e;
#pragma unroll
                    for (int i = 0; i < 8; ++i) {
                        const uint32_t a = x.v[i] & y.v[i], o = x.v[i] | y.v[i];
                        e.v[i] = (a & m_and) | ((o & m_or) & ~(a & m_xor));
                    }
                    Fr em;
                    const uint32_t br = u256_sub(em, e, fr_p());
                    err_bits |= both(both(br == 0u, u256_is_zero(em)), both(active, !shifts)) ? ST_BITOP_EQ_R : 0u;
                    e = u256_select(br == 0u, em, e);
                    d = u256_select(shifts, d, e);
                }
                r = bit_result(d);
                break;
            }
            case C_IDIVMOD: {
                const Fr x = (h & HDR_A_CANON) ? a_op : fr_from_mont(a_op), y = (h & HDR_B_CANON) ? b_op : fr_from_mont(b_op);
                const bool yz = u256_is_zero(y);
                Fr ys = y;
                ys.v[0] |= yz ? 1u : 0u;
                Fr q, rem;
                bool two_words = false;
                if constexpr (WIDE) two_words = !wave_any(both(both(active, !yz), either((ys.v[2] | ys.v[3]) == 0u, (ys.v[4] | ys.v[5] | ys.v[6] | ys.v[7]) != 0u)));
                if (!wave_any((x.v[4] | x.v[5] | x.v[6] | x.v[7] | ys.v[2] | ys.v[3] | ys.v[4] | ys.v[5] | ys.v[6] | ys.v[7]) != 0u)) {
                    u128_divrem_64(q, rem, x, ys);
                } else if (WIDE && two_words) {
                    const bool sub = either(yz, !active);
                    Fr yy = ys;
                    yy.v[0] = sub ? 0u : ys.v[0];
                    yy.v[1] = sub ? 0u : ys.v[1];
                    yy.v[2] = sub ? 1u : ys.v[2];
                    yy.v[3] = sub ? 0u : ys.v[3];
#pragma unroll
                    for (int k = 4; k < 8; ++k) yy.v[k] = 0u;
                    u256_divrem_128(q, rem, x, yy);
                } else {
                    const uint32_t lx = u256_bitlen(x), ly = u256_bitlen(ys);
                    const uint32_t my_dig = lx >= ly ? (lx - ly + 32u) >> 5 : 0u;
                    uint32_t dig = 0;
#pragma unroll
                    for (uint32_t dd = 1; dd <= 8; ++dd) dig = wave_any(my_dig >= dd) ? dd : dig;
                    u256_divrem_digits(q, rem, x, ys, dig, ly);
                }
                const Fr d = u256_select(yz, fr_zero(), u256_select(sub == SUB_IDIV, q, rem));
                r = (h & HDR_OUT_CANON) ? d : fr_mul_wave(d, fr_r2(), pv);
                break;
            }
            case C_TERN: {
                const uint32_t cr = crefs[(size_t)cref_row * G + j];
                ++cref_row;
                const Fr y = ld(cr + t16);
                r = u256_select(u256_is_zero(a_op), y, b_op);
                break;
            }
            case C_SYNC: {
                r = fr_zero();
                if (h & HDR_POST) {
                    asm volatile("s_waitcnt vmcnt(0)" ::: "memory");
                    ++n_posts;
                    if (lane == 0) __hip_atomic_store(sync_words + stream, n_posts, __ATOMIC_RELEASE, __HIP_MEMORY_SCOPE_AGENT);
                }
                if (h & HDR_WAIT) {
                    ++n_waits;
                    if (!post_wait(sync_words, n_waits)) err_bits |= ST_SYNC_TIMEOUT;
                }
                break;
            }
            case C_SCAN: r = fr_zero(); break;
            default: r = fr_zero(); break;
        }
        finish(r);
    }
    __builtin_amdgcn_raw_buffer_store_b128(u32x4{r_prev.v[0], r_prev.v[1], r_prev.v[2], r_prev.v[3]}, rsrc, (int)doff_prev, 0, 0);
    __builtin_amdgcn_raw_buffer_store_b128(u32x4{r_prev.v[4], r_prev.v[5], r_prev.v[6], r_prev.v[7]}, rsrc, (int)doff_prev + (int)HI, 0, 0);
    if (PROF && lane == 0) {
        const unsigned long long cyc = __builtin_amdgcn_s_memtime() - t_wave0;
        atomicMax(&prof[54], cyc);
        atomicMax(&prof[55], (1ull << 40) - cyc);
        atomicAdd(&prof[62], cyc);
        atomicAdd(&prof[63], 1ull);
    }
    if constexpr (PROF) {
        if (unsigned long long* c = census_slot()) c[2] = __builtin_amdgcn_s_memtime();
    }
    if (PROF && lane == 0 && (tile % 64u) == 0u) {
#pragma unroll
        for (int c = 0; c < C_PROF; ++c) {
            atomicAdd(&prof[c * 4 + 0], pf[c][0]);
            atomicAdd(&prof[c * 4 + 3], pf[c][1]);
        }
        atomicAdd(&prof[M2 ? 68 : 64], pf_fused[0]);
        atomicAdd(&prof[M2 ? 71 : 67], pf_fused[1]);
        if (M2) {
#pragma unroll
            for (int q = 0; q < 5; ++q) {
                atomicAdd(&prof[72 + 4 * q], pf_scan[q][0]);
                atomicAdd(&prof[75 + 4 * q], pf_scan[q][1]);
            }
        }
#pragma unroll
        for (int k = 0; k < 2; ++k)
#pragma unroll
            for (int q = 0; q < 6; ++q) atomicAdd(&prof[48 + 8 * k + q], psec[k][q]);
        atomicAdd(&prof[92], psec[0][6]);
        atomicAdd(&prof[93], psec[1][6]);
    }
    if (err_bits && set < batch) atomicOr(&status[set], err_bits);
}

__global__ __launch_bounds__(256) void fill_consts_kernel(ProgramDev p, WsTable wst, uint32_t n_tiles, uint32_t T) {
    const uint32_t e = blockIdx.x * 256u + threadIdx.x;
    const uint32_t pieces = p.n_const * 2u * T;
    if (e >= pieces) return;
    const uint4 v = reinterpret_cast<const uint4*>(p.consts)[(size_t)(e / (2u * T)) * 2u + (e / T) % 2u];
    const uint64_t tile_bytes = ws_tile_bytes(p.n_const, p.n_slots, T);
    for (uint32_t tile = blockIdx.y; tile < n_tiles; tile += gridDim.y) {
        char* tb = reinterpret_cast<char*>(wst.base[tile / wst.tiles_per_chunk]) + (uint64_t)(tile % wst.tiles_per_chunk) * tile_bytes;
        reinterpret_cast<uint4*>(tb)[e] = v;
    }
}

template <bool MONT>
__device__ __forceinline__ Fr pack_form(const Fr& v, bool canon) {
    if (MONT) return canon ? fr_mul(v, fr_r2()) : v;
    return canon ? v : fr_from_mont(v);
}

template <bool MONT, int TT>
__global__ __launch_bounds__(256) void pack_kernel(ProgramDev p, WsTable wst, uint4* __restrict__ out, uint32_t batch, uint32_t T_, uint32_t first) {
    const uint32_t T = TT ? (uint32_t)TT : T_;
    const uint32_t wi = first + blockIdx.x * 256u + threadIdx.x;
    if (wi >= p.n_witness) return;
    const uint32_t w = first ? p.pack_order[wi] : wi;
    const uint32_t ref_raw = p.witness_refs[w];
    const bool canon = (ref_raw & REF_CANON) != 0;
    const uint32_t ref = ref_raw & ~REF_CANON;
    const uint32_t n_tiles = (batch + T - 1) / T;
    const uint64_t tile_bytes = ws_tile_bytes(p.n_const, p.n_slots, T);
    const uint32_t slot = (ref & REF_CONST) ? (ref & ~REF_CONST) : p.n_const + ref;
    for (uint32_t tile = blockIdx.y; tile < n_tiles; tile += gridDim.y) {
        const char* tb = reinterpret_cast<const char*>(wst.base[tile / wst.tiles_per_chunk]) + (uint64_t)(tile % wst.tiles_per_chunk) * tile_bytes;
        const uint4* q = reinterpret_cast<const uint4*>(tb) + (size_t)slot * (2 * T);
        if (TT != 0 && TT <= 4) {
            uint4 lo[TT ? TT : 1], hi[TT ? TT : 1];
#pragma unroll
            for (int t = 0; t < TT; ++t) {
                lo[t] = q[t];
                hi[t] = q[TT + t];
            }
#pragma unroll
            for (int t = 0; t < TT; ++t) {
                const uint32_t set = tile * TT + t;
                if (set >= batch) break;
                const Fr c = pack_form<MONT>(fr_from_u4(lo[t], hi[t]), canon);
                uint4* o = out + ((size_t)set * p.n_witness + w) * 2;
                o[0] = make_uint4(c.v[0], c.v[1], c.v[2], c.v[3]);
                o[1] = make_uint4(c.v[4], c.v[5], c.v[6], c.v[7]);
            }
        } else {
            for (uint32_t t = 0; t < T; ++t) {
                const uint32_t set = tile * T + t;
                if (set >= batch) break;
                const Fr c = pack_form<MONT>(fr_from_u4(q[t], q[T + t]), canon);
                uint4* o = out + ((size_t)set * p.n_witness + w) * 2;
                o[0] = make_uint4(c.v[0], c.v[1], c.v[2], c.v[3]);
                o[1] = make_uint4(c.v[4], c.v[5], c.v[6], c.v[7]);
            }
        }
    }
}

template <bool MONT, int TT>
__global__ __launch_bounds__(256) void pack_kernel_v3(ProgramDev p, WsTable wst, uint4* __restrict__ out, uint32_t batch, uint32_t first) {
    constexpr uint32_t T = TT, WPB = 256u / T;
    const uint32_t t = threadIdx.x % T, wi = first + blockIdx.x * WPB + threadIdx.x / T;
    if (wi >= p.n_witness) return;
    const uint32_t w = first ? p.pack_order[wi] : wi;
    const uint32_t ref_raw = p.witness_refs[w];
    const bool canon = (ref_raw & REF_CANON) != 0;
    const uint32_t ref = ref_raw & ~REF_CANON;
    const uint32_t n_tiles = (batch + T - 1) / T;
    const uint64_t tile_bytes = ws_tile_bytes(p.n_const, p.n_slots, T);
    const uint32_t slot = (ref & REF_CONST) ? (ref & ~REF_CONST) : p.n_const + ref;
    for (uint32_t tile = blockIdx.y; tile < n_tiles; tile += gridDim.y) {
        const uint32_t set = tile * T + t;
        if (set >= batch) continue;
        const char* tb = reinterpret_cast<const char*>(wst.base[tile / wst.tiles_per_chunk]) + (uint64_t)(tile % wst.tiles_per_chunk) * tile_bytes;
        const uint4* q = reinterpret_cast<const uint4*>(tb) + (size_t)slot * (2 * T);
        const Fr c = pack_form<MONT>(fr_from_u4(q[t], q[T + t]), canon);
        uint4* o = out + ((size_t)set * p.n_witness + w) * 2;
        o[0] = make_uint4(c.v[0], c.v[1], c.v[2], c.v[3]);
        o[1] = make_uint4(c.v[4], c.v[5], c.v[6], c.v[7]);
    }
}

template <bool MONT>
__global__ __launch_bounds__(256) void pack_kernel_v1(ProgramDev p, WsTable wst, uint4* __restrict__ out, uint32_t batch, uint32_t T, uint32_t first) {
    const uint32_t wi = first + blockIdx.x * 64u + threadIdx.x;
    if (wi >= p.n_witness) return;
    const uint32_t w = first ? p.pack_order[wi] : wi;
    const uint32_t ref_raw = p.witness_refs[w];
    const bool canon = (ref_raw & REF_CANON) != 0;
    const uint32_t ref = ref_raw & ~REF_CANON;
    const uint32_t n_tiles = (batch + T - 1) / T;
    const uint64_t tile_bytes = ws_tile_bytes(p.n_const, p.n_slots, T);
    const uint32_t slot = (ref & REF_CONST) ? (ref & ~REF_CONST) : p.n_const + ref;
    for (uint32_t tile = blockIdx.y; tile < n_tiles; tile += gridDim.y) {
        const char* tb = reinterpret_cast<const char*>(wst.base[tile / wst.tiles_per_chunk]) + (uint64_t)(tile % wst.tiles_per_chunk) * tile_bytes;
        const uint4* q0 = reinterpret_cast<const uint4*>(tb) + (size_t)slot * (2 * T);
        for (uint32_t t = threadIdx.y; t < T; t += blockDim.y) {
            const uint32_t set = tile * T + t;
            if (set >= batch) break;
            const uint4* q = q0 + t;
            const Fr c = pack_form<MONT>(fr_from_u4(q[0], q[T]), canon);
            uint4* o = out + ((size_t)set * p.n_witness + w) * 2;
            o[0] = make_uint4(c.v[0], c.v[1], c.v[2], c.v[3]);
            o[1] = make_uint4(c.v[4], c.v[5], c.v[6], c.v[7]);
        }
    }
}

hipError_t launch_interp(uint32_t T, uint32_t W, uint32_t pack, uint32_t n_div_requests, const uint32_t* div_lanes, const ProgramDev& p,
                         const WsTable& wst, const void* inputs, uint32_t* status, uint32_t batch, hipStream_t stream, unsigned long long* prof,
                         void* out, uint32_t n_inline, bool montgomery) {
    const uint32_t tiles = (batch + T - 1) / T, nw = (W ? W : 1u) * pack, ns = p.n_streams ? p.n_streams : 1u;
    if (nw == 0 || nw % ns != 0 || (ns > 1 && W > 1)) return hipErrorInvalidValue;
    const uint32_t tiles_per_wg = nw / ns;
    dim3 grid((tiles + tiles_per_wg - 1) / tiles_per_wg), block((W ? (W + 1) * pack : pack) * 64);
    const uint4* in = (const uint4*)inputs;
    InterpDims dims{p.n_bundles, p.n_slots, p.n_inputs, batch, p.n_const, n_div_requests, p.trash_off, div_lanes, ns, {0, 0, 0, 0}, {0, 0, 0, 0}, {0, 0, 0, 0}, {0, 0, 0, 0},
                    (uint4*)out, reinterpret_cast<const uint2*>(p.pack_entries), p.pack_ready, 0u, montgomery ? 1u : 0u, p.n_witness};
    if (W == 1 && ns == 1 && out && p.pack_entries && p.pack_ready) dims.n_inline = n_inline < p.n_ready_last ? n_inline : p.n_ready_last;
    for (uint32_t s = 0; s < MAX_STREAMS; ++s) {
        dims.stream_first[s] = p.stream_first[s];
        dims.stream_count[s] = p.stream_count[s];
        dims.stream_div_requests[s] = p.stream_div_requests[s];
        dims.stream_cref_first[s] = p.stream_cref_first[s];
    }
    if (ns == 1) {
        dims.stream_first[0] = 0;
        dims.stream_count[0] = p.n_bundles;
        dims.stream_div_requests[0] = n_div_requests;
    }
    const uint4* recs = reinterpret_cast<const uint4*>(p.recs);
    const uint32_t mode = p.has_fused;
    static_assert(SCAN_MAX_T == COOP_FUSE_MAX_T, "the instances with a MODE are made for tile widths up to COOP_FUSE_MAX_T");
    if (mode > 3 || (mode && (T > COOP_FUSE_MAX_T || W > 1))) return hipErrorInvalidValue;
#define CWC_LAUNCH3(TT, PP, WW, KK)                                                                                                     \
    do {                                                                                                                                \
        if constexpr ((uint32_t)(TT) <= COOP_FUSE_MAX_T && (WW) <= 1) {                                                                 \
            if (mode == 3) interp_kernel<TT, PP, WW, KK, 3><<<grid, block, 0, stream>>>(p.hdr, recs, p.crefs, dims, wst, in, status, prof); \
            else if (mode == 2) interp_kernel<TT, PP, WW, KK, 2><<<grid, block, 0, stream>>>(p.hdr, recs, p.crefs, dims, wst, in, status, prof); \
            else if (mode == 1) interp_kernel<TT, PP, WW, KK, 1><<<grid, block, 0, stream>>>(p.hdr, recs, p.crefs, dims, wst, in, status, prof); \
            else interp_kernel<TT, PP, WW, KK, 0><<<grid, block, 0, stream>>>(p.hdr, recs, p.crefs, dims, wst, in, status, prof);     \
        } else {                                                                                                                        \
            interp_kernel<TT, PP, WW, KK, 0><<<grid, block, 0, stream>>>(p.hdr, recs, p.crefs, dims, wst, in, status, prof);          \
        }                                                                                                                               \
    } while (0)
#define CWC_LAUNCH2(TT, PP)                                  \
    if (W == 0 && pack == 1) CWC_LAUNCH3(TT, PP, 0, 1);      \
    else if (W == 0 && pack == 4) CWC_LAUNCH3(TT, PP, 0, 4); \
    else if (W == 1 && pack == 1) CWC_LAUNCH3(TT, PP, 1, 1); \
    else if (W == 1 && pack == 2) CWC_LAUNCH3(TT, PP, 1, 2); \
    else if (W == 1 && pack == 4) CWC_LAUNCH3(TT, PP, 1, 4); \
    else if (W == 3 && pack == 1) CWC_LAUNCH3(TT, PP, 3, 1); \
    else if (W == 4 && pack == 1) CWC_LAUNCH3(TT, PP, 4, 1); \
    else return hipErrorInvalidValue;
#ifdef CWC_DIAG
#define CWC_LAUNCH_PROF(TT, WW, KK) CWC_LAUNCH3(TT, true, WW, KK)
#define CWC_LAUNCH2_PROF(TT) CWC_LAUNCH2(TT, true)
#else
#define CWC_LAUNCH_PROF(TT, WW, KK) return hipErrorNotSupported
#define CWC_LAUNCH2_PROF(TT) return hipErrorNotSupported;
#endif
#define CWC_LAUNCH(TT)                                    \
    case TT:                                              \
        if (prof) { CWC_LAUNCH2_PROF(TT) } else { CWC_LAUNCH2(TT, false) } \
        break;
    switch (T) {
        CWC_LAUNCH(1) CWC_LAUNCH(2) CWC_LAUNCH(4) CWC_LAUNCH(8) CWC_LAUNCH(16) CWC_LAUNCH(32)
        case 64:
            if (W != 0) return hipErrorInvalidValue;
            if (pack == 4) { if (prof) { CWC_LAUNCH_PROF(64, 0, 4); } else CWC_LAUNCH3(64, false, 0, 4); }
            else if (pack == 1) { if (prof) { CWC_LAUNCH_PROF(64, 0, 1); } else CWC_LAUNCH3(64, false, 0, 1); }
            else return hipErrorInvalidValue;
            break;
        default: return hipErrorInvalidValue;
    }
#undef CWC_LAUNCH_PROF
#undef CWC_LAUNCH2_PROF
#undef CWC_LAUNCH
#undef CWC_LAUNCH2
#undef CWC_LAUNCH3
    return hipGetLastError();
}

#ifndef CWC_KSRC_HASH
#define CWC_KSRC_HASH "unstamped"
#endif
extern "C" const char* gwb_kernel_source_hash() { return CWC_KSRC_HASH; }
extern "C" int gwb_kernels_have_diagnostics() {
#ifdef CWC_DIAG
    return 1;
#else
    return 0;
#endif
}

__global__ void warm_kernel() {}
hipError_t launch_warm(hipStream_t stream) {
    warm_kernel<<<1, 64, 0, stream>>>();
    return hipGetLastError();
}

hipError_t launch_fill_consts(uint32_t T, const ProgramDev& p, const WsTable& wst, uint32_t n_tiles, hipStream_t stream) {
    if (n_tiles == 0 || p.n_const == 0) return hipSuccess;
    dim3 grid((p.n_const * 2u * T + 255u) / 256u, n_tiles < 16384u ? n_tiles : 16384u), block(256);
    fill_consts_kernel<<<grid, block, 0, stream>>>(p, wst, n_tiles, T);
    return hipGetLastError();
}

hipError_t launch_pack(uint32_t T, const ProgramDev& p, const WsTable& wst, void* out, uint32_t batch, hipStream_t stream, bool montgomery, uint32_t first) {
    if (p.n_witness == 0 || batch == 0 || first >= p.n_witness) return hipSuccess;
    const uint32_t count = p.n_witness - first;
    const uint32_t n_tiles = (batch + T - 1) / T;
    static const bool v1 = getenv("CWC_PACK_V1") != nullptr;
    if (v1 || T > 4) {
        dim3 grid((count + 63) / 64, n_tiles < 32768u ? n_tiles : 32768u), block(64, T < 4 ? T : 4);
        if (montgomery) pack_kernel_v1<true><<<grid, block, 0, stream>>>(p, wst, (uint4*)out, batch, T, first);
        else pack_kernel_v1<false><<<grid, block, 0, stream>>>(p, wst, (uint4*)out, batch, T, first);
        return hipGetLastError();
    }
    static const int pack_shape = getenv("CWC_PACK") ? atoi(getenv("CWC_PACK")) : 3;
    if (pack_shape == 3 && T >= 2) {
        dim3 grid3((count + 256 / T - 1) / (256 / T), n_tiles < 32768u ? n_tiles : 32768u), block3(256);
#define CWC_PACK3(MM, TT) pack_kernel_v3<MM, TT><<<grid3, block3, 0, stream>>>(p, wst, (uint4*)out, batch, first)
        if (montgomery) {
            if (T == 2) CWC_PACK3(true, 2); else CWC_PACK3(true, 4);
        } else {
            if (T == 2) CWC_PACK3(false, 2); else CWC_PACK3(false, 4);
        }
#undef CWC_PACK3
        return hipGetLastError();
    }
    dim3 grid((count + 255) / 256, n_tiles < 32768u ? n_tiles : 32768u), block(256);
#define CWC_PACK(MM, TT) pack_kernel<MM, TT><<<grid, block, 0, stream>>>(p, wst, (uint4*)out, batch, T, first)
    if (montgomery) {
        if (T == 1) CWC_PACK(true, 1); else if (T == 2) CWC_PACK(true, 2); else CWC_PACK(true, 4);
    } else {
        if (T == 1) CWC_PACK(false, 1); else if (T == 2) CWC_PACK(false, 2); else CWC_PACK(false, 4);
    }
#undef CWC_PACK
    return hipGetLastError();
}

__global__ __launch_bounds__(1024) void modmul_ubench_kernel(uint32_t* sink, uint32_t iters) {
    Fr a = fr_r2(), b = fr_one();
    a.v[0] ^= threadIdx.x + blockIdx.x * 977u;
    for (uint32_t it = 0; it < iters; ++it) {
        a = fr_mul(a, b);
        b = fr_mul(b, a);
    }
    if (a.v[0] == 0x1234567u && b.v[3] == 7u) sink[0] = a.v[1];
}
__global__ __launch_bounds__(512) void modmul_block_ubench_kernel(uint32_t* sink, uint32_t iters) {
    Fr a = fr_r2(), b = fr_one(), pv = fr_p();
#pragma unroll
    for (int i = 0; i < 8; ++i) asm volatile("" : "+v"(pv.v[i]));
    a.v[0] ^= threadIdx.x + blockIdx.x * 977u;
    for (uint32_t it = 0; it < iters; ++it) {
        a = fr_mul_wave(a, b, pv);
        b = fr_mul_wave(b, a, pv);
    }
    if (a.v[0] == 0x1234567u && b.v[3] == 7u) sink[0] = a.v[1];
}
hipError_t launch_modmul_ubench(uint32_t n_cus, uint32_t waves_per_simd, uint32_t iters, uint32_t* sink, hipStream_t stream, bool block_multiplier) {
    if (block_multiplier) {
        if (waves_per_simd > 2) return hipErrorInvalidValue;
        modmul_block_ubench_kernel<<<n_cus, 256 * waves_per_simd, 0, stream>>>(sink, iters);
    } else {
        modmul_ubench_kernel<<<n_cus, 256 * waves_per_simd, 0, stream>>>(sink, iters);
    }
    return hipGetLastError();
}

}
```

### circom-witnesscalc_amd/csrc/pack_schedule.cc

```cpp
#include "runtime_internal.hpp"

namespace cwcrt {

static const double kCyclesDividerServe = 52200, kCyclesPackPass = 2300;

std::string make_pack_schedule(const Program& p, PackSchedule& out) {
    const uint32_t nw = p.n_witness, G = p.G, nreq = p.n_div_requests;
    out.order.resize(nw);
    out.ready.assign((size_t)nreq + 1, 0u);
    out.n_inline = 0;
    for (uint32_t i = 0; i < nw; ++i) out.order[i] = i;
    if (p.divider != 1 || p.n_streams != 1 || nreq == 0 || nw == 0 || G == 0) return "";
    if (p.hdr.size() < p.n_bundles || p.recs.size() < (size_t)p.n_bundles * G * 4 || p.witness_refs.size() < nw) return "pack schedule: truncated program";
    const uint64_t slot_bytes = 32ull * p.T, first_off = (uint64_t)p.n_const * slot_bytes, end_off = ((uint64_t)p.n_const + p.n_slots) * slot_bytes;
    const uint32_t kNever = 0xffffffffu;
    std::vector<uint32_t> producer(p.n_slots, kNever), req_bundle;
    req_bundle.reserve(nreq);
    for (uint32_t b = 0; b < p.n_bundles; ++b) {
        if ((p.hdr[b] & HDR_CLASS_MASK) == C_DIVREQ) req_bundle.push_back(b);
        for (uint32_t i = 0; i < G; ++i) {
            const uint64_t dst = p.recs[((size_t)b * G + i) * 4 + 2] & ~CTRL_MASK;
            if (dst >= first_off && dst < end_off) producer[(dst - first_off) / slot_bytes] = b;
        }
    }
    if (req_bundle.size() != nreq) return "pack schedule: the program has " + std::to_string(req_bundle.size()) + " request bundles, its header says " + std::to_string(nreq);
    std::vector<uint32_t> at(nw);
    for (uint32_t w = 0; w < nw; ++w) {
        const uint32_t ref = p.witness_refs[w];
        if (ref & REF_CONST) {
            at[w] = 0;
            continue;
        }
        const uint32_t slot = ref & ~REF_CANON;
        if (slot >= p.n_slots || producer[slot] == kNever) return "pack schedule: witness " + std::to_string(w) + " names a slot that no bundle writes";
        const uint32_t k = (uint32_t)(std::upper_bound(req_bundle.begin(), req_bundle.end(), producer[slot]) - req_bundle.begin());
        at[w] = k + 2;
    }
    std::stable_sort(out.order.begin(), out.order.end(), [&](uint32_t a, uint32_t b) { return at[a] < at[b]; });
    for (uint32_t w = 0; w < nw; ++w)
        if (at[w] <= nreq) out.ready[at[w]]++;
    for (uint32_t k = 1; k <= nreq; ++k) out.ready[k] += out.ready[k - 1];
    double pass_cycles = kCyclesPackPass;
    if (const char* e = getenv("CWC_PACK_PASS_CYCLES")) pass_cycles = std::max(1.0, atof(e));
    double clock = 0, div_free = 0, served = 0;
    uint32_t next = 0, k = 0;
    for (uint32_t b = 0; b < p.n_bundles && k <= nreq; ++b) {
        const uint32_t cls = p.hdr[b] & HDR_CLASS_MASK;
        clock += model_class_cycles((int)cls);
        if (cls == C_DIVREQ) {
            const uint32_t limit = std::min(out.ready[k], nw) / G * G;
            const double gap = clock - div_free;
            if (gap > 0 && limit > next) next += (uint32_t)std::min<double>(std::floor(gap / pass_cycles) * G, limit - next);
            served = std::max(clock, div_free) + kCyclesDividerServe;
            div_free = served;
            ++k;
        } else if (cls == C_DIVGET) {
            clock = std::max(clock, served);
        }
    }
    out.n_inline = std::min(next, out.ready[nreq]);
    return "";
}

}

static int schedule_out(const Program& p, uint32_t* pack_order, size_t order_cap, uint32_t* pack_ready, size_t ready_cap, uint32_t* n_witness, uint32_t* n_ready,
                        uint32_t* n_inline, gw_status_t* status) {
    PackSchedule s;
    const std::string err = make_pack_schedule(p, s);
    if (!err.empty()) return fail(status, err);
    if (n_witness) *n_witness = (uint32_t)s.order.size();
    if (n_ready) *n_ready = (uint32_t)s.ready.size();
    if (n_inline) *n_inline = s.n_inline;
    if (pack_order && order_cap >= s.order.size() && !s.order.empty()) memcpy(pack_order, s.order.data(), s.order.size() * 4);
    if (pack_ready && ready_cap >= s.ready.size()) memcpy(pack_ready, s.ready.data(), s.ready.size() * 4);
    set_status(status, OK, "");
    return 0;
}

extern "C" int gwb_pack_schedule_of_blob(const void* blob, size_t len, uint32_t* pack_order, size_t order_cap, uint32_t* pack_ready, size_t ready_cap,
                                         uint32_t* n_witness, uint32_t* n_ready, uint32_t* n_inline, gw_status_t* status) {
    return guarded(status, [&]() -> int {
        if (!blob) return fail(status, "null argument");
        if (len < 24 + 8) return fail(status, "bad blob: too short");
        const uint8_t* b = (const uint8_t*)blob;
        uint64_t tr[3];
        memcpy(tr, b + len - 24, 24);
        if (tr[2] != blob_checksum(b, len - 24)) return fail(status, "bad blob: checksum mismatch (truncated or corrupted)");
        if (tr[0] > tr[1] || tr[1] > len - 24) return fail(status, "bad blob trailer");
        Program p;
        std::string err;
        if (!program_from_blob(b, (size_t)tr[0], p, err) || !validate_program(p, err)) return fail(status, "bad program blob: " + err);
        return schedule_out(p, pack_order, order_cap, pack_ready, ready_cap, n_witness, n_ready, n_inline, status);
    });
}

extern "C" int gwb_pack_schedule(gwb_graph_t* g, uint32_t program_key, uint32_t* pack_order, size_t order_cap, uint32_t* pack_ready, size_t ready_cap,
                                 uint32_t* n_witness, uint32_t* n_ready, uint32_t* n_inline, gw_status_t* status) {
    return guarded(status, [&]() -> int {
        if (!g) return fail(status, "null argument");
        std::lock_guard<std::mutex> lk(g->mu);
        Program tmp;
        const Program* p = nullptr;
        if ((program_key & ~KEY_MODE_MASK) == 64) program_key = 64;
        auto it = g->progs.find(program_key);
        auto pre = g->compiled.find(program_key);
        std::string err;
        if (it != g->progs.end()) {
            p = &it->second->host;
        } else if (pre != g->compiled.end()) {
            p = pre->second.get();
        } else {
            if (!g->has_graph) return fail(status, "imported handle has no program for that key");
            if (!compile_program(g->graph, program_key & ~KEY_MODE_MASK, key_divider_waves(program_key), tmp, err, key_streams(program_key))) return fail(status, err);
            p = &tmp;
        }
        return schedule_out(*p, pack_order, order_cap, pack_ready, ready_cap, n_witness, n_ready, n_inline, status);
    });
}
```

### circom-witnesscalc_amd/csrc/pipeline.cc

```cpp
#include "runtime_internal.hpp"

namespace cwcrt {


void set_status(gw_status_t* st, GW_ERROR_CODE code, const std::string& msg) {
    if (!st) return;
    st->code = code;
    if (code == OK && msg.empty()) {
        st->error_msg = nullptr;
        return;
    }
    st->error_msg = (char*)malloc(msg.size() + 1);
    if (st->error_msg) memcpy(st->error_msg, msg.c_str(), msg.size() + 1);
}
int fail(gw_status_t* st, const std::string& msg) {
    set_status(st, ERROR, msg);
    return 1;
}
std::string upload_program(DeviceProgram& dp) {
    const Program& p = dp.host;
    auto al = [](size_t x) { return (x + 255) & ~(size_t)255; };
    const size_t o_hdr = 0, o_recs = o_hdr + al(p.hdr.size() * 4 + 16), o_crefs = o_recs + al(p.recs.size() * 4 + REC_AHEAD * 1024u),
                 o_consts = o_crefs + al(p.crefs.size() * 4 + 256), o_wit = o_consts + al(p.consts.size() * 4 + 32),
                 o_div = o_wit + al(p.witness_refs.size() * 4 + 4), o_order = o_div + al(p.div_lanes.size() * 4 + 4),
                 o_entries = o_order + al(p.witness_refs.size() * 4 + 4), o_ready = o_entries + al((p.witness_refs.size() + PACK_ENTRY_PAD) * 8),
                 total = o_ready + al(((size_t)p.n_div_requests + 1) * 4);
    {
        const std::string serr = make_pack_schedule(p, dp.sched);
        if (!serr.empty()) return serr;
    }
    HIP_TRY(hipMalloc(&dp.d_blob, total));
    char* d = (char*)dp.d_blob;
    HIP_TRY(hipMemset(d, 0, total));
    if (!p.hdr.empty()) HIP_TRY(hipMemcpy(d + o_hdr, p.hdr.data(), p.hdr.size() * 4, hipMemcpyHostToDevice));
    if (!p.recs.empty()) HIP_TRY(hipMemcpy(d + o_recs, p.recs.data(), p.recs.size() * 4, hipMemcpyHostToDevice));
    if (!p.crefs.empty()) HIP_TRY(hipMemcpy(d + o_crefs, p.crefs.data(), p.crefs.size() * 4, hipMemcpyHostToDevice));
    if (!p.consts.empty()) HIP_TRY(hipMemcpy(d + o_consts, p.consts.data(), p.consts.size() * 4, hipMemcpyHostToDevice));
    if (!p.witness_refs.empty()) HIP_TRY(hipMemcpy(d + o_wit, p.witness_refs.data(), p.witness_refs.size() * 4, hipMemcpyHostToDevice));
    dp.dev.hdr = (const uint32_t*)(d + o_hdr);
    dp.dev.recs = (const uint32_t*)(d + o_recs);
    dp.dev.crefs = (const uint32_t*)(d + o_crefs);
    dp.dev.consts = (const uint32_t*)(d + o_consts);
    if (!p.div_lanes.empty()) HIP_TRY(hipMemcpy(d + o_div, p.div_lanes.data(), p.div_lanes.size() * 4, hipMemcpyHostToDevice));
    dp.dev.witness_refs = (const uint32_t*)(d + o_wit);
    dp.dev.div_lanes = (const uint32_t*)(d + o_div);
    dp.dev.n_bundles = p.n_bundles;
    dp.dev.n_slots = p.n_slots;
    dp.dev.n_inputs = p.n_inputs;
    dp.dev.n_witness = p.n_witness;
    dp.dev.n_const = p.n_const;
    dp.dev.trash_off = p.trash_off;
    dp.dev.has_fused = 0;
    for (uint32_t h : p.hdr) dp.dev.has_fused |= (h & HDR_CLASS_MASK) == C_MULF ? 1u : ((h & HDR_CLASS_MASK) == C_SCAN || ((h & HDR_CLASS_MASK) == C_MUL && (h & HDR_MUL_CC))) ? 2u : 0u;
    if (dp.dev.has_fused == 2u && getenv("CWC_FORCE_MODE3")) dp.dev.has_fused = 3u;
    if (dp.dev.has_fused == 2u)
        for (uint32_t h : p.hdr)
            if ((h & HDR_CLASS_MASK) == C_SCAN && !(h & HDR_SCAN_CONV) &&
                ((h & (HDR_SCAN_BORROW | HDR_SCAN_LEX)) || (!(h & HDR_SCAN_DIV) && ((h >> HDR_SCAN_SHIFT_SHIFT) & 0xffu) != 64u))) {
                dp.dev.has_fused = 3u;
                break;
            }
    {
        const PackSchedule& sc = dp.sched;
        std::vector<uint32_t> entries(sc.order.size() * 2);
        for (size_t i = 0; i < sc.order.size(); ++i) {
            entries[2 * i] = sc.order[i];
            entries[2 * i + 1] = p.witness_refs[sc.order[i]];
        }
        if (!sc.order.empty()) HIP_TRY(hipMemcpy(d + o_order, sc.order.data(), sc.order.size() * 4, hipMemcpyHostToDevice));
        if (!entries.empty()) HIP_TRY(hipMemcpy(d + o_entries, entries.data(), entries.size() * 4, hipMemcpyHostToDevice));
        HIP_TRY(hipMemcpy(d + o_ready, sc.ready.data(), sc.ready.size() * 4, hipMemcpyHostToDevice));
        dp.dev.pack_order = (const uint32_t*)(d + o_order);
        dp.dev.pack_entries = (const uint32_t*)(d + o_entries);
        dp.dev.pack_ready = (const uint32_t*)(d + o_ready);
        dp.dev.n_inline = sc.n_inline;
        dp.dev.n_ready_last = sc.ready.back();
    }
    dp.dev.n_streams = p.n_streams;
    for (uint32_t s = 0; s < MAX_STREAMS; ++s) {
        dp.dev.stream_first[s] = p.stream_first[s];
        dp.dev.stream_count[s] = p.stream_count[s];
        dp.dev.stream_div_requests[s] = p.stream_div_requests[s];
        dp.dev.stream_cref_first[s] = p.stream_cref_first[s];
    }
    return "";
}

static bool stream_pair_workgroups(uint32_t divider, uint64_t tiles, uint32_t streams) {
    if (streams != 2 || divider != 1) return false;
    if (const char* e = getenv("CWC_STREAM_TILES_PER_WORKGROUP")) return atoi(e) == 2;
    return tiles > 256;
}
uint32_t waves_per_workgroup(uint32_t divider, uint64_t tiles, uint32_t streams) {
    if (stream_pair_workgroups(divider, tiles, streams)) return 4u;
    if (streams > 1) return divider ? streams : 4u;
    const char* e = getenv("CWC_WAVES_PER_WORKGROUP");
    if (divider == 1) return e ? (atoi(e) >= 4 ? 2u : 1u) : (tiles > 256 ? 2u : 1u);
    if (divider) return 1;
    if (e) return atoi(e) == 4 ? 4u : 1u;
    return tiles > 512 ? 4u : 1u;
}

uint64_t workspace_budget() {
    const char* e = getenv("CWC_WORKSPACE_GB");
    double gb = e ? atof(e) : 8.0;
    if (gb < 1e-4) gb = 1e-4;
    return (uint64_t)(gb * (double)(1ull << 30));
}
}

extern "C" uint32_t gwb_pick_tile_width(size_t batch) {
    size_t target = 2048, divider_tiles = 1024;
    if (const char* e = getenv("CWC_TARGET_WAVES")) {
        long v = atol(e);
        if (v > 0) target = (size_t)v;
    }
    if (const char* e = getenv("CWC_DIVIDER_TILES")) divider_tiles = (size_t)atol(e);
    uint32_t t = batch <= 256 ? 1 : batch <= 1024 ? 2 : 4;
    while (t < 64 && (batch + t - 1) / t > target) t *= 2;
    const size_t tiles = (batch + t - 1) / t;
    return t | (tiles <= divider_tiles && t < 64 ? KEY_DIVIDER : 0u);
}

namespace cwcrt {

std::string check_device() {
    int n = 0;
    hipError_t e = hipGetDeviceCount(&n);
    if (e != hipSuccess || n <= 0)
        return std::string("no HIP device available (") + (e != hipSuccess ? hipGetErrorString(e) : "device count 0") +
               "); this library has no CPU fallback";
    static const std::string xnack_refusal = []() -> std::string {
        int dev = 0;
        hipDeviceProp_t prop;
        if (hipGetDevice(&dev) != hipSuccess || hipGetDeviceProperties(&prop, dev) != hipSuccess) {
            (void)hipGetLastError();
            return "";
        }
        return strstr(prop.gcnArchName, "xnack+") ? std::string("device ") + prop.gcnArchName + ": XNACK-enabled devices are not supported (run with HSA_XNACK=0)" : "";
    }();
    return xnack_refusal;
}

double estimate_cycles(const Program& p, size_t batch) {
    const double wide = p.T >= 8 ? 1.10 : 1.0;
    if (p.n_streams > 1) {
        const double tiles = (double)((batch + p.T - 1) / p.T);
        if (stream_pair_workgroups(p.divider, (uint64_t)tiles, p.n_streams)) {
            constexpr double kTwoWaves = 0.62, kPackCyclesPerValue = 0.028;
            double t = 0;
            for (uint32_t s = 0; s < p.n_streams; ++s) {
                const double own = std::max(p.stream_cycles[s], p.stream_chain_cycles[s]);
                const double simd = (p.stream_cycles[s] + model_class_cycles(C_DIV) * p.stream_div_requests[s]) * kTwoWaves;
                t = std::max(t, std::max(own, simd));
            }
            const double rounds = std::max(1.0, tiles / 512.0);
            return t * (p.T >= 4 ? 1.2 * wide : 1.0) * rounds + kPackCyclesPerValue * (double)p.n_witness * (double)batch;
        }
        const double t = program_wave_cycles(p);
        double busy = 0;
        for (uint32_t s = 0; s < p.n_streams; ++s) busy += (p.stream_cycles[s] + model_class_cycles(C_DIV) * p.stream_div_requests[s]) / t;
        const double wgs = p.divider ? tiles : std::ceil(tiles * p.n_streams / 4.0);
        const double wg_per_cu = p.divider ? (p.n_streams == 4 ? 1.0 : 3.0) : 2.0;
        const double rounds = std::max(1.0, wgs / (256.0 * wg_per_cu));
        const double crowd = std::max(1.0, 1.1 * (tiles / rounds) * busy / 1024.0);
        return t * (p.T >= 4 ? 1.2 * wide : p.T == 2 ? 1.08 : 1.0) * crowd * rounds;
    }
    const double per_wave = program_wave_cycles(p) * wide;
    const double heavy = program_wave_cycles_mul_div(p) * wide;
    const double waves = (double)((batch + p.T - 1) / p.T);
    const double two_per_simd = (1.3 * heavy + 1.9 * (per_wave - heavy)) / per_wave;
    if (p.divider == 4) return per_wave * 1.30 * (waves <= 1024 ? 1.0 : waves / 1024);
    if (p.divider == 3) return per_wave * 1.08 * (waves <= 768 ? 1.0 : two_per_simd * (waves <= 1536 ? 1.0 : waves / 1536));
    const double resident = waves * (p.divider == 1 ? 2.0 : 1.0);
    double crowd = resident <= 1024 ? 1.0 : two_per_simd;
    if (p.divider == 1 && resident > 1024) crowd = 1.0 + 0.75 * (crowd - 1.0);
    const double rounds = resident <= 2048 ? 1.0 : resident / 2048;
    return per_wave * crowd * rounds;
}

std::vector<uint32_t> candidate_keys(const ProgramStats& stats, size_t batch, uint32_t rule, uint32_t min_t) {
    size_t divider_tiles = 1024;
    if (const char* e = getenv("CWC_DIVIDER_TILES")) divider_tiles = (size_t)atol(e);
    const bool has_div = stats.class_nodes[C_DIV] > 0;
    const uint32_t t0 = rule & ~KEY_MODE_MASK;
    std::vector<uint32_t> keys;
    for (uint32_t t = std::max(min_t, t0 >= 4 ? t0 / 4 : 1u); t <= t0 * 2 && t <= 32 && (batch >= 64 || t == t0); t *= 2)
        for (uint32_t mode : {0u, KEY_DIVIDER, KEY_TRIPLE, KEY_GROUP}) {
            const size_t tiles = (batch + t - 1) / t;
            if (tiles > 4 * 2048) continue;
            const bool divider_fits = has_div && tiles <= divider_tiles;
            if (mode == 0 && divider_fits) continue;
            if (mode == KEY_DIVIDER && !divider_fits) continue;
            if (mode == KEY_TRIPLE && !(has_div && tiles > 512 && tiles <= 768 && !getenv("CWC_NO_GROUP_DIVIDER"))) continue;
            if (mode == KEY_GROUP && !(has_div && tiles > 512 && tiles <= 1024 && !getenv("CWC_NO_GROUP_DIVIDER"))) continue;
            keys.push_back(t | mode);
            if ((mode == 0 || mode == KEY_DIVIDER) && t < 64 && !getenv("CWC_NO_STREAMS")) {
                if (tiles <= 256) keys.push_back(t | mode | KEY_STREAMS4);
                else if (tiles <= 340) keys.push_back(t | mode | KEY_STREAMS2);
                else if (mode == KEY_DIVIDER && t >= 2 && tiles <= 512 && !getenv("CWC_INLINE_PACK") && !getenv("CWC_INLINE_PACK_ROWS"))
                    keys.push_back(t | mode | KEY_STREAMS2);
            }
        }
    return keys;
}

gwb_graph::Refined refine_choice(const Graph& graph, const ProgramStats& stats, size_t batch, uint32_t rule, uint32_t min_t) {
    gwb_graph::Refined r;
    try {
        double best_cost = -1;
        std::unique_ptr<SharedRewrites, void (*)(SharedRewrites*)> rewrites(make_shared_rewrites(), free_shared_rewrites);
        for (uint32_t key : candidate_keys(stats, batch, rule, min_t)) {
            std::unique_ptr<Program> p(new Program());
            std::string err;
            if (!compile_program(graph, key & ~KEY_MODE_MASK, key_divider_waves(key), *p, err, key_streams(key), false, rewrites.get())) continue;
            const double cost = estimate_cycles(*p, batch);
            if (best_cost < 0 || cost < best_cost) {
                best_cost = cost;
                r.best = key;
            }
            r.programs[key] = std::move(p);
        }
    } catch (...) {
        r.best = 0;
        r.programs.clear();
    }
    return r;
}

uint32_t pick_tile_width(gwb_graph* g, size_t batch, bool allow_quick) {
    if (!g->has_graph && !g->progs.empty()) return g->progs.begin()->first;
    if (g->forced_T) return g->forced_T;
    if (const char* e = getenv("CWC_TILE_WIDTH")) {
        const uint32_t key = (uint32_t)atoi(e), t = key & ~KEY_MODE_MASK;
        if (t >= 1 && t <= 64 && !(t & (t - 1))) return key;
    }
    uint32_t rule = gwb_pick_tile_width(batch);
    uint32_t min_t = 1;
    {
        double budget = 960.0;
        if (const char* e = getenv("CWC_PROGRAM_MB")) budget = atof(e);
        const double per_bundle_t1 = 4.0 + 64.0 * 16.0;
        auto levels = [&](uint32_t t) { return (double)(t <= SCAN_MAX_T && !getenv("CWC_NO_SCAN") && g->stats.depth_scan ? g->stats.depth_scan : g->stats.depth); };
        while (min_t < 16 && levels(min_t) * 1.25 * (4.0 + (per_bundle_t1 - 4.0) / min_t) > budget * 1048576.0) min_t *= 2;
        if ((rule & ~KEY_MODE_MASK) < min_t) rule = min_t | ((rule & KEY_MODE_MASK) && min_t < 64 ? (rule & KEY_MODE_MASK) : 0u);
    }
    if (getenv("CWC_STATIC_TILE_RULE") || !g->has_graph) return rule;
    auto hit = g->chosen.find(batch);
    if (hit != g->chosen.end()) return hit->second;
    if (batch < 64 && g->graph.nodes.size() <= 2000000 && !getenv("CWC_NO_QUICK_FIRST_CALL")) {
        auto job = g->refining.find(batch);
        if (job != g->refining.end()) {
            if (!allow_quick) {
                if (g->refine_gate) g->refine_gate->store(true);
                job->second.wait();
            }
            if (job->second.wait_for(std::chrono::seconds(0)) != std::future_status::ready) return g->provisional[batch];
            gwb_graph::Refined r = job->second.get();
            g->refining.erase(job);
            const uint32_t quick_key = g->provisional[batch];
            g->provisional.erase(batch);
            if (r.best == 0) {
                g->chosen[batch] = quick_key;
                return quick_key;
            }
            for (auto& kv : r.programs) {
                if (g->progs.count(kv.first)) {
                    if (g->filled_prog == g->progs[kv.first].get()) g->filled_prog = nullptr;
                    g->progs.erase(kv.first);
                }
                g->compiled[kv.first] = std::move(kv.second);
            }
            g->chosen[batch] = r.best;
            return r.best;
        }
        const bool has_div0 = g->stats.class_nodes[C_DIV] > 0;
        const uint32_t t1 = std::max(1u, min_t);
        const uint32_t quick_key = t1 | (has_div0 && t1 < 64 ? KEY_DIVIDER : 0u) | (t1 < 64 && !getenv("CWC_NO_STREAMS") ? KEY_STREAMS4 : 0u);
        if (allow_quick && !g->progs.count(quick_key) && !g->compiled.count(quick_key)) {
            std::unique_ptr<Program> p(new Program());
            std::string err;
            if (compile_program(g->graph, quick_key & ~KEY_MODE_MASK, key_divider_waves(quick_key), *p, err, key_streams(quick_key), true)) g->compiled[quick_key] = std::move(p);
        }
        if (allow_quick && (g->progs.count(quick_key) || g->compiled.count(quick_key))) {
            const Graph* graph = &g->graph;
            const ProgramStats stats = g->stats;
            g->provisional[batch] = quick_key;
            const std::string cache_file = batch == 1 && !g->cache_written ? g->cache_path : std::string();
            const std::vector<InputSignal> inputs = cache_file.empty() ? std::vector<InputSignal>() : g->inputs;
            if (!cache_file.empty()) g->cache_written = true;
            if (!g->refine_gate) g->refine_gate = std::make_shared<std::atomic<bool>>(false);
            g->refine_gate->store(false);
            std::shared_ptr<std::atomic<bool>> gate = g->refine_gate;
            g->refining[batch] = std::async(std::launch::async, [graph, stats, batch, rule, min_t, cache_file, inputs, gate]() {
                for (int waited = 0; !gate->load() && waited < 2000; ++waited) std::this_thread::sleep_for(std::chrono::milliseconds(1));
                gwb_graph::Refined r = refine_choice(*graph, stats, batch, rule, min_t);
                auto best = r.programs.find(r.best);
                if (!cache_file.empty() && r.best && best != r.programs.end()) {
                    try {
                        const std::vector<uint8_t> b0 = exported_bytes(*best->second, inputs), b = cache_wrap(cache_file, b0.data(), b0.size());
                        write_file_atomically(cache_file, b.data(), b.size());
                        if (getenv("CWC_DEBUG_CACHE")) fprintf(stderr, "program cache: wrote %s (program key %#x, %zu bytes)\n", cache_file.c_str(), r.best, b.size());
                    } catch (...) {
                    }
                }
                return r;
            });
            return quick_key;
        }
    }
    const bool debug = getenv("CWC_DEBUG_COST") != nullptr;
    uint32_t best = rule;
    double best_cost = -1;
    const std::vector<uint32_t> keys = candidate_keys(g->stats, batch, rule, min_t);
    std::unique_ptr<SharedRewrites, void (*)(SharedRewrites*)> rewrites(make_shared_rewrites(), free_shared_rewrites);
    std::vector<std::pair<uint32_t, std::future<std::unique_ptr<Program>>>> jobs;
    for (uint32_t key : keys)
        if (!g->progs.count(key) && !g->compiled.count(key)) {
            const Graph* graph = &g->graph;
            SharedRewrites* shared = rewrites.get();
            jobs.emplace_back(key, std::async(std::launch::async, [graph, key, shared]() {
                                  std::unique_ptr<Program> p(new Program());
                                  std::string err;
                                  if (!compile_program(*graph, key & ~KEY_MODE_MASK, key_divider_waves(key), *p, err, key_streams(key), false, shared)) p.reset();
                                  return p;
                              }));
        }
    for (auto& j : jobs) {
        std::unique_ptr<Program> p = j.second.get();
        if (p) g->compiled[j.first] = std::move(p);
    }
    for (uint32_t key : keys) {
        const Program* p = nullptr;
        auto up = g->progs.find(key);
        auto pre = g->compiled.find(key);
        if (up != g->progs.end()) p = &up->second->host;
        else if (pre != g->compiled.end()) p = pre->second.get();
        else continue;
        const double cost = estimate_cycles(*p, batch);
        if (debug) fprintf(stderr, "cost model: batch %zu key %#x -> %.1f Mcycles\n", batch, key, cost / 1e6);
        if (best_cost < 0 || cost < best_cost) {
            best_cost = cost;
            best = key;
        }
    }
    g->chosen[batch] = best;
    return best;
}

std::string get_program(gwb_graph* g, uint32_t key, DeviceProgram** out) {
    const uint32_t T = key & ~KEY_MODE_MASK;
    if (T == 64) key = T;
    auto it = g->progs.find(key);
    if (it != g->progs.end()) {
        *out = it->second.get();
        return "";
    }
    if (!g->has_graph) return "imported graph handle has no program for tile width " + std::to_string(T);
    std::unique_ptr<DeviceProgram> dp(new DeviceProgram());
    std::string err;
    auto pre = g->compiled.find(key);
    if (pre != g->compiled.end()) {
        dp->host = std::move(*pre->second);
        g->compiled.erase(pre);
    } else if (!compile_program(g->graph, T, key_divider_waves(key), dp->host, err, key_streams(key))) {
        return err;
    }
    err = upload_program(*dp);
    if (!err.empty()) return err;
    *out = dp.get();
    g->progs[key] = std::move(dp);
    return "";
}

static const bool kInlinePackDefault = true;
std::string run_device(gwb_graph* g, const void* d_inputs, size_t batch, void* d_witness, uint32_t* d_status,
                       hipStream_t stream, bool montgomery, hipEvent_t done_event) {
    if (batch == 0) return "";
    if (batch > 0x7fffffffull) return "batch too large";
    static const bool dbg_steps = getenv("CWC_DEBUG_SINGLE") != nullptr;
    auto now_ms = []() { return std::chrono::duration<double, std::milli>(std::chrono::steady_clock::now().time_since_epoch()).count(); };
    const double t_0 = dbg_steps ? now_ms() : 0.0;
    const uint32_t key = pick_tile_width(g, batch);
    struct OpenGate {
        gwb_graph* g;
        ~OpenGate() {
            if (g->refine_gate) g->refine_gate->store(true);
        }
    } open_gate{g};
    const double t_1 = dbg_steps ? now_ms() : 0.0;
    DeviceProgram* dp = nullptr;
    std::string err = get_program(g, key, &dp);
    if (!err.empty()) return err;
    const double t_2 = dbg_steps ? now_ms() : 0.0;
    g->last_key = (key & ~KEY_MODE_MASK) == 64 ? 64u : key;
    const Program& p = dp->host;
    const uint32_t T = p.T;
    if (!g->last_done) HIP_TRY(hipEventCreateWithFlags(&g->last_done, hipEventDisableTiming));
    if (g->has_last && g->last_stream != stream) HIP_TRY(hipStreamWaitEvent(stream, g->last_done, 0));
    struct OrderGuard {
        gwb_graph* g;
        hipStream_t stream;
        ~OrderGuard() {
            if (hipEventRecord(g->last_done, stream) == hipSuccess) {
                g->last_stream = stream;
                g->has_last = true;
            } else {
                (void)hipGetLastError();
                g->has_last = false;
                (void)hipDeviceSynchronize();
            }
        }
    } order_guard{g, stream};
    const uint64_t bytes_per_tile = ws_tile_bytes(p.n_const, p.n_slots, T);
    const uint64_t budget = workspace_budget();
    if (bytes_per_tile > 0xffffffffull) return "graph too large for the 4 GiB tile window";
    uint64_t max_tiles = budget / bytes_per_tile;
    if (max_tiles == 0) max_tiles = 1;
    const uint64_t tiles_total = (batch + T - 1) / T;
    const uint64_t chunk_tiles = tiles_total < max_tiles ? tiles_total : max_tiles;
    const size_t need = (size_t)(chunk_tiles * bytes_per_tile);
    const size_t chunk_sets = (size_t)chunk_tiles * T;
    const size_t n_chunks = (batch + chunk_sets - 1) / chunk_sets;
    size_t per_launch = n_chunks < WS_MAX_CHUNKS ? n_chunks : WS_MAX_CHUNKS;
    if (const char* e = getenv("CWC_STREAMS")) {
        const long v = atol(e);
        if (v >= 1 && (size_t)v < per_launch) per_launch = (size_t)v;
    }
    bool refill = g->filled_prog != dp || g->filled_tiles_per_chunk != chunk_tiles || g->filled_chunks < per_launch;
    for (size_t l = 0; l < per_launch; ++l) {
        if (need > g->vals_bytes[l]) {
            if (g->d_vals[l]) HIP_TRY(hipFree(g->d_vals[l]));
            g->d_vals[l] = nullptr;
            g->vals_bytes[l] = 0;
            g->filled_prog = nullptr;
            refill = true;
            HIP_TRY(hipMalloc(&g->d_vals[l], need));
            g->vals_bytes[l] = need;
        }
    }
    if (refill) {
        WsTable all;
        memset(&all, 0, sizeof all);
        all.tiles_per_chunk = (uint32_t)chunk_tiles;
        all.n_chunks = (uint32_t)per_launch;
        for (size_t l = 0; l < per_launch; ++l) all.base[l] = g->d_vals[l];
        HIP_TRY(launch_fill_consts(T, dp->dev, all, (uint32_t)(per_launch * chunk_tiles), stream));
        g->filled_prog = dp;
        g->filled_tiles_per_chunk = chunk_tiles;
        g->filled_chunks = per_launch;
    }
    const double t_3 = dbg_steps ? now_ms() : 0.0;
    g->last_call_launches = 0;
    g->timing = gwb_timing_t{};
    g->timing.tile_width = T;
    g->timing.divider = p.divider;
    g->timing.streams = p.n_streams;
    g->timing.n_bundles = p.n_bundles;
    g->timing.n_slots = p.n_slots;
    uint32_t n_inline = kInlinePackDefault ? dp->dev.n_inline : 0u;
    if (const char* e = getenv("CWC_INLINE_PACK")) n_inline = atoi(e) >= 2 ? dp->dev.n_ready_last : atoi(e) == 1 ? dp->dev.n_inline : 0u;
    if (const char* e = getenv("CWC_INLINE_PACK_ROWS")) n_inline = std::min<uint32_t>(n_inline, (uint32_t)atol(e));
    const size_t launch_sets = per_launch * chunk_sets;
    for (size_t s0 = 0; s0 < batch; s0 += launch_sets) {
        const uint32_t nb = (uint32_t)((batch - s0) < launch_sets ? (batch - s0) : launch_sets);
        WsTable wst;
        memset(&wst, 0, sizeof wst);
        wst.tiles_per_chunk = (uint32_t)chunk_tiles;
        wst.n_chunks = (uint32_t)((nb + chunk_sets - 1) / chunk_sets);
        for (uint32_t l = 0; l < wst.n_chunks; ++l) wst.base[l] = g->d_vals[l];
        hipEvent_t e0, e1, e2;
        if (g->pending.size() >= gwb_graph::kHistory) {
            e0 = g->pending.front().start, e1 = g->pending.front().after_interp, e2 = g->pending.front().after_pack;
            g->pending.pop_front();
        } else {
            e0 = e1 = e2 = nullptr;
            const bool ok = hipEventCreate(&e0) == hipSuccess && hipEventCreate(&e1) == hipSuccess && hipEventCreate(&e2) == hipSuccess;
            if (!ok) {
                for (hipEvent_t e : {e0, e1, e2})
                    if (e) (void)hipEventDestroy(e);
                return "hipEventCreate failed";
            }
        }
        g->pending.push_back(gwb_graph::ChunkEvents{e0, e1, e2});
        HIP_TRY(hipEventRecord(e0, stream));
        void* const out = (char*)d_witness + s0 * (size_t)p.n_witness * 32;
        HIP_TRY(launch_interp(T, p.divider, waves_per_workgroup(p.divider, (nb + T - 1) / T, p.n_streams), p.n_div_requests, dp->dev.div_lanes, dp->dev, wst, (const char*)d_inputs + s0 * p.n_inputs * 32, d_status + s0, nb, stream, g->d_prof,
                              out, n_inline, montgomery));
        HIP_TRY(hipEventRecord(e1, stream));
        HIP_TRY(launch_pack(T, dp->dev, wst, out, nb, stream, montgomery, n_inline));
        HIP_TRY(hipEventRecord(e2, stream));
        g->last_call_launches++;
        g->timing.n_launches++;
    }
    g->timing_pending = true;
    if (done_event) HIP_TRY(hipEventRecord(done_event, stream));
    if (g->refine_gate) g->refine_gate->store(true);
    if (dbg_steps && now_ms() - t_0 > 20.0)
        fprintf(stderr, "run_device: program choice %.1f ms, program on the device %.1f ms, workspace + constants %.1f ms, launches %.1f ms\n", t_1 - t_0, t_2 - t_1, t_3 - t_2, now_ms() - t_3);
    return "";
}

bool is_pinned_host(const void* p) {
    hipPointerAttribute_t a;
    memset(&a, 0, sizeof a);
    if (hipPointerGetAttributes(&a, p) != hipSuccess) {
        (void)hipGetLastError();
        return false;
    }
    return a.type == hipMemoryTypeHost;
}

unsigned env_threads(const char* name, unsigned cap) {
    long v = 0;
    if (const char* e = getenv(name)) v = atol(e);
    if (v <= 0) {
        v = (long)std::thread::hardware_concurrency();
        if (cap && v > (long)cap) v = cap;
    }
    return v < 1 ? 1u : (unsigned)v;
}

unsigned copy_threads() {
    long v = 0;
    if (const char* e = getenv("CWC_COPY_THREADS")) v = atol(e);
    if (v <= 0) {
        v = (long)std::thread::hardware_concurrency();
        if (v > 16) v = 16;
    }
    return v < 1 ? 1u : (unsigned)v;
}

std::string device_to_host_rows(gwb_graph* g, void* dst, const void* d_src, size_t bytes) {
    if (bytes == 0) return "";
    if (!g->copy_stream) HIP_TRY(hipStreamCreateWithFlags(&g->copy_stream, hipStreamNonBlocking));
    if (is_pinned_host(dst)) {
        HIP_TRY(hipMemcpyAsync(dst, d_src, bytes, hipMemcpyDeviceToHost, g->copy_stream));
        HIP_TRY(hipStreamSynchronize(g->copy_stream));
        return "";
    }
    size_t slice = 32u << 20;
    if (const char* e = getenv("CWC_COPY_SLICE_MB")) {
        const long v = atol(e);
        if (v >= 1 && v <= 1024) slice = (size_t)v << 20;
    }
    if (bytes < slice) slice = std::max<size_t>(g->stage_bytes, (bytes + (1u << 20) - 1) & ~(size_t)((1u << 20) - 1));
    const int n_stage = bytes > slice ? 2 : 1;
    if (g->stage_bytes < slice) {
        for (int i = 0; i < 2; ++i) {
            if (g->stage[i]) HIP_TRY(hipHostFree(g->stage[i]));
            g->stage[i] = nullptr;
        }
        g->stage_bytes = 0;
        for (int i = 0; i < n_stage; ++i) HIP_TRY(hipHostMalloc(&g->stage[i], slice, hipHostMallocDefault));
        g->stage_bytes = slice;
    }
    if (n_stage == 2 && !g->stage[1]) HIP_TRY(hipHostMalloc(&g->stage[1], g->stage_bytes, hipHostMallocDefault));
    for (int i = 0; i < 2; ++i)
        if (!g->stage_done[i]) HIP_TRY(hipEventCreateWithFlags(&g->stage_done[i], hipEventDisableTiming));
    const size_t n_slices = (bytes + slice - 1) / slice;
    const unsigned n_workers = bytes < (8u << 20) ? 1u : copy_threads();
    std::atomic<long> ready{0};
    std::atomic<bool> abort{false};
    std::vector<std::atomic<unsigned>> consumed(n_slices);
    for (auto& c : consumed) c.store(0);
    auto stripe_copy = [&](unsigned w, size_t k) {
        const size_t off = k * slice, len = bytes - off < slice ? bytes - off : slice;
        const size_t per = ((len + n_workers - 1) / n_workers + 4095) & ~(size_t)4095;
        const size_t a = (size_t)w * per, b = a + per < len ? a + per : len;
        if (a < b) memcpy((char*)dst + off + a, (const char*)g->stage[k & 1] + a, b - a);
    };
    std::vector<std::thread> workers;
    for (unsigned w = 1; w < n_workers; ++w)
        workers.emplace_back([&, w]() {
            for (size_t k = 0; k < n_slices; ++k) {
                while (ready.load(std::memory_order_acquire) <= (long)k) {
                    if (abort.load()) return;
                    std::this_thread::yield();
                }
                stripe_copy(w, k);
                consumed[k].fetch_add(1, std::memory_order_release);
            }
        });
    std::string err;
    auto issue = [&](size_t k) -> std::string {
        const size_t off = k * slice, len = bytes - off < slice ? bytes - off : slice;
        HIP_TRY(hipMemcpyAsync(g->stage[k & 1], (const char*)d_src + off, len, hipMemcpyDeviceToHost, g->copy_stream));
        HIP_TRY(hipEventRecord(g->stage_done[k & 1], g->copy_stream));
        return "";
    };
    err = issue(0);
    for (size_t k = 0; k < n_slices && err.empty(); ++k) {
        if (k + 1 < n_slices) {
            if (k >= 1)
                while (consumed[k - 1].load(std::memory_order_acquire) < n_workers) std::this_thread::yield();
            err = issue(k + 1);
            if (!err.empty()) break;
        }
        if (hipEventSynchronize(g->stage_done[k & 1]) != hipSuccess) {
            err = "hipEventSynchronize failed in the witness copy";
            break;
        }
        ready.store((long)k + 1, std::memory_order_release);
        stripe_copy(0, k);
        consumed[k].fetch_add(1, std::memory_order_release);
    }
    if (!err.empty()) abort.store(true);
    for (auto& t : workers) t.join();
    if (!err.empty()) (void)hipStreamSynchronize(g->copy_stream);
    return err;
}

std::string run_host(gwb_graph* g, const void* inputs, size_t batch, void* witness, uint32_t* set_status) {
    if (batch == 0) return "";
    const size_t in_b = batch * (size_t)g->n_inputs * 32, out_b = batch * (size_t)g->n_witness * 32;
    auto grow = [](void*& p, size_t& have, size_t need) -> std::string {
        if (need <= have) return "";
        if (p) HIP_TRY(hipFree(p));
        p = nullptr;
        have = 0;
        HIP_TRY(hipMalloc(&p, need));
        have = need;
        return "";
    };
    static const bool dbg_steps = getenv("CWC_DEBUG_SINGLE") != nullptr;
    auto now_ms = []() { return std::chrono::duration<double, std::milli>(std::chrono::steady_clock::now().time_since_epoch()).count(); };
    const double t0 = dbg_steps ? now_ms() : 0.0;
    std::string err = grow(g->h_in, g->h_in_bytes, in_b ? in_b : 32);
    if (err.empty()) err = grow(g->h_out, g->h_out_bytes, out_b ? out_b : 32);
    if (err.empty()) err = grow(g->h_st, g->h_st_bytes, batch * 4);
    if (!err.empty()) return err;
    HIP_TRY(hipMemcpy(g->h_in, inputs, in_b, hipMemcpyHostToDevice));
    const double t1 = dbg_steps ? now_ms() : 0.0;
    err = run_device(g, g->h_in, batch, g->h_out, (uint32_t*)g->h_st, nullptr);
    if (!err.empty()) return err;
    const double t2 = dbg_steps ? now_ms() : 0.0;
    HIP_TRY(hipDeviceSynchronize());
    const double t3 = dbg_steps ? now_ms() : 0.0;
    err = device_to_host_rows(g, witness, g->h_out, out_b);
    if (!err.empty()) return err;
    HIP_TRY(hipMemcpy(set_status, g->h_st, batch * 4, hipMemcpyDeviceToHost));
    if (dbg_steps && now_ms() - t0 > 20.0)
        fprintf(stderr, "run_host: device buffers + rows in %.1f ms, run_device (choice, upload, workspace, launches) %.1f ms, wait for the device %.1f ms, rows out %.1f ms\n", t1 - t0, t2 - t1, t3 - t2, now_ms() - t3);
    return "";
}

std::string set_status_text(uint32_t bits) {
    std::string s;
    if (bits & ST_SHL_OVERFLOW) s += "Shl result does not fit the field (reference panics at graph.rs:634)";
    if (bits & 0x80000000u) s += std::string(s.empty() ? "" : "; ") + "internal error: divider mailbox wait timed out";
    if (bits & 0x40000000u) s += std::string(s.empty() ? "" : "; ") + "internal error: wait for another stream's post timed out";
    if (bits & ST_BITOP_EQ_R) s += std::string(s.empty() ? "" : "; ") + "bit operation result equals the modulus (reference panics at graph.rs:686/701/716)";
    return s;
}

void warm_device() {
    struct Joined {
        std::thread t;
        ~Joined() {
            if (t.joinable()) t.join();
        }
    };
    static Joined warm;
    static std::once_flag once;
    std::call_once(once, []() {
        if (getenv("CWC_NO_WARM_THREAD")) return;
        warm.t = std::thread([]() {
            int n = 0;
            if (hipGetDeviceCount(&n) != hipSuccess || n <= 0) {
                (void)hipGetLastError();
                return;
            }
            void* p = nullptr;
            if (hipMalloc(&p, 4096) == hipSuccess) (void)hipFree(p);
            else (void)hipGetLastError();
            if (launch_warm(nullptr) != hipSuccess) (void)hipGetLastError();
        });
    });
}

}
```

### circom-witnesscalc_amd/csrc/program_dev.h

```cpp
#pragma once
#include <stdint.h>

#include "ops.h"

#if defined(__HIPCC__)
#define CWC_HD __host__ __device__ static inline
#define CWC_HDC __host__ __device__ static constexpr
#else
#define CWC_HD static inline
#define CWC_HDC static constexpr
#endif

namespace cwc {

enum BundleClass : uint32_t {
    C_INPUT = 0,
    C_MUL = 1,
    C_LIN = 2,
    C_DIV = 3,
    C_CMPZ = 4,
    C_CMPS = 5,
    C_BIT = 6,
    C_IDIVMOD = 7,
    C_TERN = 8,
    C_DIVREQ = 9,
    C_DIVGET = 10,
    C_MULQ = 11,
    C_SYNC = 12,
    C_MULF = 13,
    C_SCAN = 14,
    C_COUNT = 15
};
static const uint32_t COOP_LANES = 4, COOP_MAX_T = 4, COOP_FUSE_MAX_T = 2, SCAN_MAX_T = 2;
static const uint32_t HDR_SCAN_DIV = 1u << 11, HDR_SCAN_CONV = 1u << 12;
enum SelCode : uint32_t { SEL_LT = 1, SEL_GT = 2, SEL_LEQ = 3, SEL_GEQ = 4, SEL_NEZ = 5, SEL_OUT_MONT = 8 };
static const uint32_t HDR_SCAN_BORROW = 1u << 13, HDR_SCAN_LEX = 1u << 14, HDR_SCAN_KG = 1u << 15, HDR_SCAN_KL = 1u << 16;
static const int HDR_SCAN_SHIFT_SHIFT = 19, HDR_SCAN_ITER_SHIFT = 27;
static const uint32_t SCAN_ROLE_ACC = 1u, SCAN_START = 2u;
enum FusedOp : uint32_t { FOP_NONE = 0, FOP_MUL = 1, FOP_ADD = 2, FOP_SUB = 3 , FOP_RSUB = 4  };
static const uint32_t HDR_F_S2MUL = 1u << 11, HDR_F_S2LIN = 1u << 12, HDR_F_S3LIN = 1u << 13;
CWC_HDC uint32_t coop_nodes(uint32_t T) { return T <= COOP_MAX_T ? 64u / (COOP_LANES * T) : 0u; }

static const uint32_t OFF_NOWHERE = 0xffff0000u;
static const uint32_t HDR_CLASS_MASK = 0xfu;
static const int HDR_COUNT_SHIFT = 4;
static const uint32_t HDR_LIN_SUB = 1u << 11, HDR_LIN_ADD = 1u << 12, HDR_BITX_ALL = 1u << 13;
static const uint32_t HDR_MUL_CC = 1u << 13;
static const uint32_t HDR_BIT_ALL_SHR = 1u << 11, HDR_BIT_ALL_BAND = 1u << 12;
static const uint32_t HDR_B_CANON = 1u << 14, HDR_A_CANON = 1u << 17, HDR_OUT_CANON = 1u << 18;
static const uint32_t HDR_POST = 1u << 15, HDR_WAIT = 1u << 16;
static const uint32_t MAX_STREAMS = 4;
static const uint32_t PROF_WORDS = 96, CENSUS_MAX_WAVES = 8192, CENSUS_WORDS = 3;
static const uint32_t CTRL_SUB_MASK = 7u, CTRL_ACTIVE = 8u, CTRL_MASK = 15u;
static const uint32_t RING_BUNDLES = 4, OPND_AHEAD = 2, REC_AHEAD = 4;
static const uint32_t RING_SLOT_BYTES = 2048, LDS_HALF_BYTES = 1024, STAGE_BYTES = 4096, REC_BYTES = 1024;
CWC_HDC uint32_t mbox_lanes(uint32_t W) { return W <= 1u ? 64u : 32u; }
CWC_HDC uint32_t mbox_bytes(uint32_t W) { return mbox_lanes(W) * 64u; }
CWC_HDC uint32_t lds_area_bytes(uint32_t W, uint32_t lds_bytes) { return (void)W, lds_bytes; }
static const uint32_t LDS_RING_OFF = 0, LDS_STAGE_OFF = LDS_RING_OFF + RING_BUNDLES * RING_SLOT_BYTES,
                      LDS_REC_OFF = LDS_STAGE_OFF + OPND_AHEAD * STAGE_BYTES, LDS_BYTES = LDS_REC_OFF + REC_AHEAD * REC_BYTES;
enum SubOp : uint32_t {
    SUB_ADD = 0, SUB_SUB = 1, SUB_MULT = 2,
    SUB_EQ = 0, SUB_NEQ = 1, SUB_LAND = 2, SUB_LOR = 3,
    SUB_LT = 0, SUB_GT = 1, SUB_LEQ = 2, SUB_GEQ = 3,
    SUB_SHL = 0, SUB_SHR = 1, SUB_BOR = 2, SUB_BAND = 3, SUB_BXOR = 4,
    SUB_BITX = 5,
    SUB_IDIV = 0, SUB_MOD = 1,
};

static const uint32_t REF_CONST = 0x80000000u;
static const uint32_t REF_CANON = 0x40000000u;

enum SetStatus : uint32_t {
    ST_SHL_OVERFLOW = 1u,
    ST_BITOP_EQ_R = 2u,
};

struct ProgramDev {
    const uint32_t* hdr;
    const uint32_t* recs;
    const uint32_t* crefs;
    const uint32_t* consts;
    const uint32_t* witness_refs;
    const uint32_t* div_lanes;
    uint32_t n_bundles, n_slots, n_inputs, n_witness, n_const;
    uint32_t trash_off;
    uint32_t has_fused;
    uint32_t n_streams, stream_first[4], stream_count[4], stream_div_requests[4], stream_cref_first[4];
    const uint32_t* pack_order;
    const uint32_t* pack_entries;
    const uint32_t* pack_ready;
    uint32_t n_inline, n_ready_last;
};
static const uint32_t PACK_ENTRY_PAD = 192;

static const uint32_t WS_MAX_CHUNKS = 32;
struct WsTable {
    void* base[WS_MAX_CHUNKS];
    uint32_t tiles_per_chunk;
    uint32_t n_chunks;
};

CWC_HD uint64_t ws_tile_bytes(uint32_t n_const, uint32_t n_slots, uint32_t T) { return ((uint64_t)n_const + n_slots + 3u) * 32u * T; }
CWC_HD uint64_t ws_sync_offset(uint32_t n_const, uint32_t n_slots, uint32_t T) { return ((uint64_t)n_const + n_slots + 2u) * 32u * T; }

}
```

### circom-witnesscalc_amd/csrc/runtime_internal.hpp

```cpp
#pragma once
#include <dlfcn.h>
#include <sys/stat.h>
#include <sys/types.h>
#include <unistd.h>
#include <hip/hip_runtime_api.h>
#include <stdio.h>
#include <stdlib.h>
#include <string.h>

#include <chrono>
#include <cmath>
#include <condition_variable>
#include <map>
#include <memory>
#include <mutex>
#include <algorithm>
#include <atomic>
#include <deque>
#include <future>
#include <string>
#include <thread>
#include <vector>

#define GW_NO_INLINE_FREE_STATUS
#ifndef CWC_TREE_HASH
#define CWC_TREE_HASH "unstamped"
#endif
#include "../../include/graph_witness_batch.h"
#include "graph.hpp"
#include "program.hpp"

namespace cwc {
hipError_t launch_interp(uint32_t T, uint32_t W, uint32_t pack, uint32_t n_div_requests, const uint32_t* div_lanes, const ProgramDev& p,
                         const WsTable& wst, const void* inputs, uint32_t* status, uint32_t batch, hipStream_t stream, unsigned long long* prof,
                         void* out = nullptr, uint32_t n_inline = 0, bool montgomery = false);
hipError_t launch_pack(uint32_t T, const ProgramDev& p, const WsTable& wst, void* out, uint32_t batch, hipStream_t stream, bool montgomery, uint32_t first = 0);
hipError_t launch_modmul_ubench(uint32_t n_cus, uint32_t waves_per_simd, uint32_t iters, uint32_t* sink, hipStream_t stream, bool block_multiplier);
hipError_t launch_fill_consts(uint32_t T, const ProgramDev& p, const WsTable& wst, uint32_t n_tiles, hipStream_t stream);
hipError_t launch_warm(hipStream_t stream);
}

using namespace cwc;

namespace cwcrt {

void set_status(gw_status_t* st, GW_ERROR_CODE code, const std::string& msg);
int fail(gw_status_t* st, const std::string& msg);
template <class F>
int guarded(gw_status_t* st, F&& f) {
    try {
        return f();
    } catch (const std::bad_alloc&) {
        return fail(st, "out of memory");
    } catch (const std::exception& e) {
        return fail(st, std::string("internal error: ") + e.what());
    } catch (...) {
        return fail(st, "internal error");
    }
}
#define HIP_TRY(expr)                                                                      \
    do {                                                                                   \
        hipError_t e_ = (expr);                                                            \
        if (e_ != hipSuccess) return std::string(#expr) + ": " + hipGetErrorString(e_);    \
    } while (0)

struct PackSchedule {
    std::vector<uint32_t> order;
    std::vector<uint32_t> ready;
    uint32_t n_inline = 0;
};
std::string make_pack_schedule(const Program& p, PackSchedule& out);

struct DeviceProgram {
    Program host;
    PackSchedule sched;
    void* d_blob = nullptr;
    ProgramDev dev{};
    DeviceProgram() = default;
    DeviceProgram(const DeviceProgram&) = delete;
    DeviceProgram& operator=(const DeviceProgram&) = delete;
    ~DeviceProgram() {
        if (d_blob) (void)hipFree(d_blob);
    }
};

}
using namespace cwcrt;

struct gwb_graph {
    Graph graph;
    bool has_graph = false;
    std::vector<InputSignal> inputs;
    std::unordered_map<std::string, uint32_t> input_index;
    uint32_t n_inputs = 0, n_witness = 0;
    ProgramStats stats;
    std::map<uint32_t, std::unique_ptr<DeviceProgram>> progs;
    std::map<uint32_t, std::unique_ptr<Program>> compiled;
    std::map<size_t, uint32_t> chosen;
    uint32_t forced_T = 0;
    uint32_t last_key = 0;
    struct Refined {
        uint32_t best = 0;
        std::map<uint32_t, std::unique_ptr<Program>> programs;
    };
    std::map<size_t, std::future<Refined>> refining;
    std::map<size_t, uint32_t> provisional;
    std::shared_ptr<std::atomic<bool>> refine_gate;
    bool cache_written = false;
    std::string cache_path;
    struct E2eBufs {
        void* h_rows[2] = {nullptr, nullptr};
        void* d_in[2] = {nullptr, nullptr};
        void* d_out[2] = {nullptr, nullptr};
        void* d_st[2] = {nullptr, nullptr};
        void* stage[2][3] = {{nullptr, nullptr, nullptr}, {nullptr, nullptr, nullptr}};
        hipStream_t compute = nullptr, copy[2] = {nullptr, nullptr};
        hipEvent_t done[2] = {nullptr, nullptr}, slice_done[2][3] = {{nullptr, nullptr, nullptr}, {nullptr, nullptr, nullptr}};
        size_t in_bytes = 0, out_bytes = 0, st_bytes = 0, stage_bytes = 0;
        void release() {
            for (int i = 0; i < 2; ++i) {
                if (h_rows[i]) (void)hipHostFree(h_rows[i]);
                if (d_in[i]) (void)hipFree(d_in[i]);
                if (d_out[i]) (void)hipFree(d_out[i]);
                if (d_st[i]) (void)hipFree(d_st[i]);
                h_rows[i] = d_in[i] = d_out[i] = d_st[i] = nullptr;
                for (int b = 0; b < 3; ++b) {
                    if (stage[i][b]) (void)hipHostFree(stage[i][b]);
                    stage[i][b] = nullptr;
                }
            }
            in_bytes = out_bytes = st_bytes = stage_bytes = 0;
        }
    } e2e;
    static const int kMaxLanes = (int)WS_MAX_CHUNKS;
    void* d_vals[kMaxLanes] = {nullptr};
    size_t vals_bytes[kMaxLanes] = {0};
    const DeviceProgram* filled_prog = nullptr;
    uint64_t filled_tiles_per_chunk = 0;
    size_t filled_chunks = 0;
    bool timing_pending = false;
    gwb_timing_t timing{};
    unsigned long long* d_prof = nullptr;
    struct ChunkEvents { hipEvent_t start, after_interp, after_pack; };
    static const size_t kHistory = 256;
    std::deque<ChunkEvents> pending;
    size_t last_call_launches = 0;
    void *h_in = nullptr, *h_out = nullptr, *h_st = nullptr;
    size_t h_in_bytes = 0, h_out_bytes = 0, h_st_bytes = 0;
    void* stage[2] = {nullptr, nullptr};
    size_t stage_bytes = 0;
    hipEvent_t stage_done[2] = {nullptr, nullptr};
    hipStream_t copy_stream = nullptr;
    hipEvent_t last_done = nullptr;
    hipStream_t last_stream = nullptr;
    bool has_last = false;
    std::mutex mu;

    void drop_events() {
        for (auto& c : pending) { (void)hipEventDestroy(c.start); (void)hipEventDestroy(c.after_interp); (void)hipEventDestroy(c.after_pack); }
        pending.clear();
    }

    ~gwb_graph() {
        progs.clear();
        for (int i = 0; i < kMaxLanes; ++i)
            if (d_vals[i]) (void)hipFree(d_vals[i]);
        drop_events();
        for (void* p : {h_in, h_out, h_st})
            if (p) (void)hipFree(p);
        for (int i = 0; i < 2; ++i) {
            if (stage[i]) (void)hipHostFree(stage[i]);
            if (stage_done[i]) (void)hipEventDestroy(stage_done[i]);
        }
        if (copy_stream) (void)hipStreamDestroy(copy_stream);
        if (last_done) (void)hipEventDestroy(last_done);
        e2e.release();
        for (int i = 0; i < 2; ++i) {
            if (e2e.copy[i]) (void)hipStreamDestroy(e2e.copy[i]);
            if (e2e.done[i]) (void)hipEventDestroy(e2e.done[i]);
            for (int b = 0; b < 3; ++b)
                if (e2e.slice_done[i][b]) (void)hipEventDestroy(e2e.slice_done[i][b]);
        }
        if (e2e.compute) (void)hipStreamDestroy(e2e.compute);
    }
};

namespace cwcrt {
std::string upload_program(DeviceProgram& dp);
uint32_t waves_per_workgroup(uint32_t divider, uint64_t tiles, uint32_t streams = 1);
uint64_t workspace_budget();
std::string check_device();
double estimate_cycles(const Program& p, size_t batch);
uint32_t pick_tile_width(gwb_graph* g, size_t batch, bool allow_quick = true);
std::string get_program(gwb_graph* g, uint32_t key, DeviceProgram** out);
std::string run_device(gwb_graph* g, const void* d_inputs, size_t batch, void* d_witness, uint32_t* d_status, hipStream_t stream, bool montgomery = false,
                       hipEvent_t done_event = nullptr);
std::string run_host(gwb_graph* g, const void* inputs, size_t batch, void* witness, uint32_t* set_status);
unsigned env_threads(const char* name, unsigned cap);
std::string set_status_text(uint32_t bits);
void warm_device();
uint64_t fnv1a(const uint8_t* p, size_t n);
uint64_t blob_checksum(const uint8_t* p, size_t n);
uint64_t sampled_fingerprint(const uint8_t* p, size_t n);
size_t exported_size(const Program& p, const std::vector<InputSignal>& inputs);
void exported_write(const Program& p, const std::vector<InputSignal>& inputs, uint8_t* dst);
std::vector<uint8_t> exported_bytes(const Program& p, const std::vector<InputSignal>& inputs);
void write_file_atomically(const std::string& path, const void* data, size_t n);
std::vector<uint8_t> cache_wrap(const std::string& path, const void* blob, size_t n);
bool quirks();
int load_graph(const void* data, size_t len, gwb_graph** out, std::string& err);
}
extern "C" int gwb_kernels_have_diagnostics();
```

### include/graph_witness_batch.h

```cpp
#ifndef CWC_AMD_GRAPH_WITNESS_BATCH_H
#define CWC_AMD_GRAPH_WITNESS_BATCH_H

#include <stddef.h>
#include <stdint.h>

#include "graph_witness.h"

#ifdef __cplusplus
extern "C" {
#endif

typedef struct gwb_graph gwb_graph_t;

typedef struct {
  uint64_t n_nodes;
  uint64_t n_op;
  uint64_t n_input_nodes;
  uint64_t n_const;
  uint64_t n_inputs;
  uint64_t n_witness;
  uint64_t depth;
  uint64_t algorithmic_bytes_per_set;
} gwb_graph_info_t;

typedef struct {
  uint32_t tile_width;
  uint32_t n_launches;
  uint64_t n_bundles;
  uint64_t n_slots;
  float interp_ms;
  float pack_ms;
  uint32_t divider;
  uint32_t streams;
} gwb_timing_t;

int gwb_graph_load(const void *graph_data, size_t graph_data_len, gwb_graph_t **out, gw_status_t *status);
void gwb_graph_free(gwb_graph_t *g);
int gwb_graph_info(const gwb_graph_t *g, gwb_graph_info_t *info);
int gwb_graph_serialize(const gwb_graph_t *g, void **out, size_t *out_len, gw_status_t *status);

typedef struct gwb_builder gwb_builder_t;
#define GWB_BUILDER_BAD 0xffffffffu
gwb_builder_t *gwb_builder_new(void);
void gwb_builder_free(gwb_builder_t *b);
uint32_t gwb_builder_input(gwb_builder_t *b, uint32_t input_index);
uint32_t gwb_builder_constant(gwb_builder_t *b, const void *value_le, size_t value_len);
uint32_t gwb_builder_uno(gwb_builder_t *b, uint32_t op, uint32_t a);
uint32_t gwb_builder_duo(gwb_builder_t *b, uint32_t op, uint32_t a, uint32_t b_idx);
uint32_t gwb_builder_tres(gwb_builder_t *b, uint32_t op, uint32_t a, uint32_t b_idx, uint32_t c);
int gwb_builder_witness(gwb_builder_t *b, uint32_t node);
int gwb_builder_input_signal(gwb_builder_t *b, const char *name, uint32_t offset, uint32_t len);
uint64_t gwb_builder_node_count(const gwb_builder_t *b);
int gwb_builder_finish(const gwb_builder_t *b, void **out, size_t *out_len, gw_status_t *status);

int gwb_graphgen_bigint_class(uint32_t k, uint32_t n_bits, uint32_t rounds, void **out, size_t *out_len, gw_status_t *status);
int gwb_graphgen_rsa_long_div_class(uint32_t n, uint32_t k, uint32_t muls, int range_checks, void **out, size_t *out_len, gw_status_t *status);
int gwb_graph_op_histogram(const gwb_graph_t *g, uint64_t *out, size_t n);

int gwb_inputs_from_json(const gwb_graph_t *g, const char *inputs_json, void *row, gw_status_t *status);

int gwb_inputs_from_json_batch(const gwb_graph_t *g, const char *text, size_t text_len, void *rows, size_t max_rows,
                               size_t *n_rows, gw_status_t *status);
int gwb_wtns_save_batch(const void *witness, size_t n_witness, size_t batch, const char *path_pattern, gw_status_t *status);

typedef struct {
  size_t n_sets, sub_batch;
  uint32_t parse_threads, write_threads;
  double parse_seconds;
  double wait_for_drain_seconds;
  double total_seconds;
  uint64_t witness_bytes;
  uint64_t failed_sets;
} gwb_e2e_stats_t;
int gwb_calc_witness_json_to_wtns(gwb_graph_t *g, const char *text, size_t text_len, const char *path_pattern, size_t first_index,
                                  size_t *n_sets, uint32_t *set_status, size_t max_sets, gwb_e2e_stats_t *stats, gw_status_t *status);

#define GWB_TILE_ASYNC_DIVIDER 0x100u
#define GWB_TILE_GROUP_DIVIDER 0x200u
#define GWB_TILE_TRIPLE_DIVIDER 0x400u
#define GWB_TILE_STREAMS2 0x800u
#define GWB_TILE_STREAMS4 0x1000u
int gwb_set_tile_width(gwb_graph_t *g, uint32_t tile_width);
uint32_t gwb_pick_tile_width(size_t batch);
uint32_t gwb_graph_pick_tile_width(gwb_graph_t *g, size_t batch);

int gwb_calc_witness_batch_device(gwb_graph_t *g, const void *d_inputs, size_t batch, void *d_witness,
                                  uint32_t *d_set_status, void *hip_stream, gw_status_t *status);
#define GWB_FORM_CANONICAL 0u
#define GWB_FORM_MONTGOMERY 1u
typedef struct {
  uint32_t struct_size;
  uint32_t form;
  void *hip_stream;
  void *done_event;
} gwb_handoff_t;
int gwb_calc_witness_batch_handoff(gwb_graph_t *g, const void *d_inputs, size_t batch, void *d_witness,
                                   uint32_t *d_set_status, const gwb_handoff_t *handoff, gw_status_t *status);

int gwb_calc_witness_batch_host(gwb_graph_t *g, const void *inputs, size_t batch, void *witness,
                                uint32_t *set_status, gw_status_t *status);
void *gwb_host_alloc(size_t bytes);
void gwb_host_free(void *p);
int gwb_last_timing(gwb_graph_t *g, gwb_timing_t *t);
int gwb_timing_history(gwb_graph_t *g, size_t max_launches, float *interp_ms, float *pack_ms, size_t *n_out);

int gwb_profile_classes(gwb_graph_t *g, const void *d_inputs, size_t batch, void *d_witness,
                        uint32_t *d_set_status, uint64_t *out64, gw_status_t *status);
int gwb_wave_census(gwb_graph_t *g, const void *d_inputs, size_t batch, void *d_witness,
                    uint32_t *d_set_status, uint64_t *out64, size_t out_words, gw_status_t *status);

double gwb_ubench_modmul(uint32_t waves_per_simd, uint32_t iters);

double gwb_ubench_modmul_block(uint32_t waves_per_simd, uint32_t iters);
double gwb_model_class_cycles(uint32_t bundle_class);
const char* gwb_kernel_source_hash(void);

typedef struct {
  uint32_t tile_width, divider, streams, n_classes;
  uint64_t n_bundles, n_fused_nodes;
  uint64_t class_bundles[16];
  uint64_t class_nodes[16];
  double model_wave_cycles;
  double lanes_active_mean;
  double values_per_bundle_mean;
  double chain_floor_cycles;
  uint64_t n_scan_steps;
  uint64_t n_conv_products;
} gwb_program_stats_t;
int gwb_program_stats(gwb_graph_t *g, uint32_t program_key, gwb_program_stats_t *out);

int gwb_pack_schedule(gwb_graph_t *g, uint32_t program_key, uint32_t *pack_order, size_t order_cap, uint32_t *pack_ready, size_t ready_cap,
                      uint32_t *n_witness, uint32_t *n_ready, uint32_t *n_inline, gw_status_t *status);
int gwb_pack_schedule_of_blob(const void *blob, size_t blob_len, uint32_t *pack_order, size_t order_cap, uint32_t *pack_ready, size_t ready_cap,
                              uint32_t *n_witness, uint32_t *n_ready, uint32_t *n_inline, gw_status_t *status);

size_t gwb_wtns_size(size_t n_witness);
int gwb_wtns_from_witness(const void *witness_row, size_t n_witness, void *out);

int gwb_graph_export(gwb_graph_t *g, uint32_t tile_width, void **blob, size_t *blob_len, gw_status_t *status);
int gwb_graph_import(const void *blob, size_t blob_len, gwb_graph_t **out, gw_status_t *status);

#define GWB_RCCL_UNIQUE_ID_BYTES 128
int gwb_rccl_unique_id(void *id128, gw_status_t *status);
int gwb_rccl_comm_init(const void *id128, int n_ranks, int rank, void **comm, gw_status_t *status);
int gwb_rccl_comm_ranks(void *comm);
void gwb_rccl_comm_destroy(void *comm);
int gwb_graph_broadcast(gwb_graph_t *g, uint32_t tile_width, size_t batch_per_rank, int root, int rank, void *nccl_comm,
                        void *hip_stream, gwb_graph_t **out, gw_status_t *status);

void gwb_free_status(gw_status_t *status);

#ifdef __cplusplus
}
#endif
#endif
```

Baseline: 93510.

## Overlap witness packing with two-stream interpretation using progress marks

Extends inline packing to the two-stream divider configuration. Interpreter waves publish progress marks in LDS every N bundles, and the packing wave reads those marks to pack witness rows whose producers are already done, in a host-computed order. This moves part of the separate pack kernel's work into idle SIMD time during interpretation. In exchange it adds spin-wait synchronisation with a new timeout status, extra LDS words, and a new schedule built on the host, and the tile-width cost model now accounts for the inline share.

```diff
diff --git a/circom-witnesscalc_amd/__init__.py b/circom-witnesscalc_amd/__init__.py
--- a/circom-witnesscalc_amd/__init__.py
+++ b/circom-witnesscalc_amd/__init__.py
@@ -72,7 +72,7 @@
     "gwb_builder_witness", "gwb_builder_input_signal", "gwb_builder_node_count", "gwb_builder_finish",
     "gwb_ubench_modmul_block", "gwb_program_stats", "gwb_calc_witness_json_to_wtns", "gwb_model_class_cycles",
     "gwb_graphgen_bigint_class", "gwb_graphgen_rsa_long_div_class", "gwb_graph_op_histogram",
-    "gwb_kernel_source_hash", "gwb_pack_schedule", "gwb_pack_schedule_of_blob", "gwb_rccl_unique_id", "gwb_rccl_comm_init", "gwb_rccl_comm_ranks", "gwb_rccl_comm_destroy",
+    "gwb_kernel_source_hash", "gwb_pack_schedule", "gwb_pack_schedule_of_blob", "gwb_stream_pack_schedule", "gwb_stream_pack_schedule_of_blob", "gwb_rccl_unique_id", "gwb_rccl_comm_init", "gwb_rccl_comm_ranks", "gwb_rccl_comm_destroy",
     "gwb_wave_census",
 ]
 
@@ -147,6 +147,9 @@
         if hasattr(L, "gwb_pack_schedule"):
             L.gwb_pack_schedule.argtypes = [vp, ctypes.c_uint32, vp, sz, vp, sz, u32p, u32p, u32p, stp]
             L.gwb_pack_schedule_of_blob.argtypes = [vp, sz, vp, sz, vp, sz, u32p, u32p, u32p, stp]
+        if hasattr(L, "gwb_stream_pack_schedule"):
+            L.gwb_stream_pack_schedule.argtypes = [vp, ctypes.c_uint32, vp, sz, vp, sz, vp, sz, vp, stp]
+            L.gwb_stream_pack_schedule_of_blob.argtypes = [vp, sz, vp, sz, vp, sz, vp, sz, vp, stp]
         L.gwb_calc_witness_json_to_wtns.argtypes = [vp, ctypes.c_char_p, sz, ctypes.c_char_p, sz, ctypes.POINTER(sz), vp, sz, ctypes.POINTER(E2eStats), stp]
         L.gwb_graph_pick_tile_width.restype = ctypes.c_uint32
         L.gwb_graph_pick_tile_width.argtypes = [vp, sz]
@@ -451,6 +454,9 @@
     def pack_schedule(self, key):
         return _pack_schedule(lambda *a: lib().gwb_pack_schedule(self._h, key, *a))
 
+    def stream_pack_schedule(self, key):
+        return _stream_pack_schedule(lambda *a: lib().gwb_stream_pack_schedule(self._h, key, *a))
+
     def last_timing(self):
         t = Timing()
         if lib().gwb_last_timing(self._h, ctypes.byref(t)) != 0:
@@ -469,6 +475,21 @@
 def pack_schedule_of_blob(blob):
     blob = bytes(blob)
     return _pack_schedule(lambda *a: lib().gwb_pack_schedule_of_blob(blob, len(blob), *a))
+
+
+def _stream_pack_schedule(call):
+    info, st = np.zeros(8, dtype=np.uint32), GwStatus()
+    _check(call(None, 0, None, 0, None, 0, info.ctypes.data, ctypes.byref(st)), st)
+    nw, m0, m1, passes = (int(v) for v in info[:4])
+    order, marks, need = np.zeros(nw, dtype=np.uint32), np.zeros(m0 + m1, dtype=np.uint32), np.zeros(passes, dtype=np.uint32)
+    _check(call(order.ctypes.data, order.size, marks.ctypes.data, marks.size, need.ctypes.data, need.size, info.ctypes.data, ctypes.byref(st)), st)
+    return {"order": order, "marks": (marks[:m0].copy(), marks[m0:].copy()), "need": need, "pack_stream": int(info[4]), "n_vouched": int(info[5]),
+            "n_inline": int(info[6]), "lag": int(info[7])}
+
+
+def stream_pack_schedule_of_blob(blob):
+    blob = bytes(blob)
+    return _stream_pack_schedule(lambda *a: lib().gwb_stream_pack_schedule_of_blob(blob, len(blob), *a))
 
 
 R1CS_LIB_PATH = os.environ.get("CWC_R1CS_LIB_PATH") or os.path.join(_HERE, "libcwc_r1cs.so")
diff --git a/circom-witnesscalc_amd/csrc/kernels.hip b/circom-witnesscalc_amd/csrc/kernels.hip
--- a/circom-witnesscalc_amd/csrc/kernels.hip
+++ b/circom-witnesscalc_amd/csrc/kernels.hip
@@ -21,9 +21,12 @@
     const uint2* pack_entries;
     const uint32_t* pack_ready;
     uint32_t n_inline, pack_mont, n_witness;
+    const uint32_t* spack_allowed;
+    uint32_t spack_spacing, spack_stream, spack_n, spack_off1;
 };
 static const uint32_t ST_DIVIDER_TIMEOUT = 0x80000000u;
 static const uint32_t ST_SYNC_TIMEOUT = 0x40000000u;
+static const uint32_t ST_PACK_TIMEOUT = 0x20000000u;
 
 __device__ __forceinline__ bool mbox_wait(const volatile uint32_t* seq, uint32_t need) {
     for (uint32_t spins = 0; spins < (1u << 22); ++spins) {
@@ -98,7 +101,9 @@
     const __amdgpu_buffer_rsrc_t rsrc = __builtin_amdgcn_make_buffer_rsrc(tile_base, 0, (int)(uint32_t)tile_bytes, 0x00020000);
     const i32x4 rsrc_rec = make_rsrc_words(recs, (p.n_bundles + REC_AHEAD) * (uint32_t)G * 16u);
     uint32_t* const sync_words = reinterpret_cast<uint32_t*>(tile_base + ws_sync_offset(p.n_const, p.n_slots, T));
-    static_assert(NW + PACK <= 16, "sequence words: 64 bytes");
+    constexpr bool MARKS = W == 1 && PACK == 4;
+    constexpr uint32_t MK = NW + (uint32_t)PACK;
+    static_assert(NW + PACK + (MARKS ? NW + 1u : 0u) <= 16, "sequence and mark words: 64 bytes");
     __shared__ uint4 lds[(NW * AREA + (DIVIDER ? NW * MB + 64u : 0u)) / 16];
     const uint32_t area = wave * AREA;
     const uint32_t lds0 = (uint32_t)(uintptr_t)(lds_char*)(char*)lds + area;
@@ -108,7 +113,8 @@
     char* const mbox = mbox_all + (wave < NW ? wave : 0u) * MB;
     volatile uint32_t* const seq = reinterpret_cast<volatile uint32_t*>(mbox_all + NW * MB);
     if (DIVIDER || NW > 1) {
-        if (DIVIDER && threadIdx.x < NW + (uint32_t)PACK) seq[threadIdx.x] = 0;
+        if (DIVIDER && threadIdx.x < NW + (uint32_t)PACK + (MARKS ? NW : 0u)) seq[threadIdx.x] = 0;
+        if (MARKS && threadIdx.x == MK + NW) seq[MK + NW] = NS == 2 ? p.spack_spacing : 0u;
         if (NS > 1 && wave < NW && stream == 0 && lane < MAX_STREAMS && tile_raw < n_tiles) {
             __hip_atomic_store(sync_words + lane, 0u, __ATOMIC_RELAXED, __HIP_MEMORY_SCOPE_AGENT);
             __builtin_amdgcn_fence(__ATOMIC_RELEASE, "agent");
@@ -131,6 +137,26 @@
             [[maybe_unused]] uint2 pk_e0 = make_uint2(0u, 0u), pk_e1 = pk_e0;
             [[maybe_unused]] unsigned long long pk_cycles = 0, pk_passes = 0;
             const bool inl = W == 1 && NS == 1 && p.n_inline > 0;
+            bool spk = false;
+            if constexpr (MARKS) spk = NS == 2 && p.spack_n > 0 && p.spack_spacing != 0u && first_w % NS == p.spack_stream;
+            const volatile uint32_t* const mk = seq + MK + first_w / NS * NS;
+            auto pk_allowed = [&]() -> uint32_t {
+                uint32_t lim = p.spack_n;
+                if constexpr (MARKS) {
+#pragma unroll
+                    for (uint32_t s = 0; s < 2; ++s) {
+                        const uint32_t b0 = p.stream_first[s], cnt = p.stream_count[s];
+                        if (cnt == 0) continue;
+                        const uint32_t last = b0 + cnt - 1, regular = last > b0 ? (last - b0 - 1) / p.spack_spacing : 0u;
+                        const uint32_t v = (uint32_t)__builtin_amdgcn_readfirstlane((int)mk[s]);
+                        const uint32_t m = v == 0 ? 0u : v - 1 == last ? regular + 1 : (v - 1 - b0) / p.spack_spacing;
+                        const uint32_t a = (uint32_t)__builtin_amdgcn_readfirstlane((int)p.spack_allowed[(s ? p.spack_off1 : 0u) + m]);
+                        lim = a < lim ? a : lim;
+                    }
+                    __builtin_amdgcn_fence(__ATOMIC_ACQUIRE, "workgroup");
+                }
+                return lim;
+            };
             const char* const pk_tile = reinterpret_cast<const char*>(wst.base[first_tile / wst.tiles_per_chunk]) + (uint64_t)(first_tile % wst.tiles_per_chunk) * tile_bytes;
             const uint32_t pk_set = first_tile * T + t;
             auto pk_load = [&](const uint2& e, uint4& lo, uint4& hi) {
@@ -179,16 +205,16 @@
                 if (PROF) pk_cycles += __builtin_amdgcn_s_memtime() - t0;
             };
             if constexpr (W == 1) {
-                if (inl) {
+                if (inl || spk) {
                     pk_e0 = p.pack_entries[j];
                     pk_e1 = p.pack_entries[(uint32_t)G + j];
                 }
             }
             for (uint32_t k = 0; k < n_requests; ++k) {
                 if constexpr (W == 1) {
-                    if (inl) {
+                    if (inl || spk) {
                         const uint32_t lim = p.pack_ready[k] < p.n_inline ? p.pack_ready[k] : p.n_inline;
-                        pk_run(lim / (uint32_t)G * (uint32_t)G, k + 1);
+                        pk_run(spk ? pk_allowed() : lim / (uint32_t)G * (uint32_t)G, k + 1);
                     }
                 }
                 bool ok = true;
@@ -221,8 +247,19 @@
                 if (lane == 0) seq[wave] = k + 1;
             }
             if constexpr (W == 1) {
-                if (inl) {
-                    pk_run(p.pack_ready[n_requests] < p.n_inline ? p.pack_ready[n_requests] : p.n_inline, 0xffffffffu);
+                if (inl || spk) {
+                    const uint32_t last = p.pack_ready[n_requests] < p.n_inline ? p.pack_ready[n_requests] : p.n_inline, share = spk ? p.spack_n : last;
+                    bool ok = true;
+#pragma nounroll
+                    for (uint32_t spins = 0; spins < (1u << 22); ++spins) {
+                        const uint32_t before = pk_next;
+                        pk_run(spk ? pk_allowed() : last, 0xffffffffu);
+                        ok = !spk || pk_next >= share;
+                        if (ok) break;
+                        if (pk_next != before) spins = 0;
+                        __builtin_amdgcn_s_sleep(8);
+                    }
+                    if (!ok && pk_set < batch) atomicOr(&status[pk_set], ST_PACK_TIMEOUT);
                     if (PROF && lane == 0 && first_tile % 64u == 0) {
                         atomicAdd(&prof[94], pk_cycles);
                         atomicAdd(&prof[95], pk_passes);
@@ -237,6 +274,7 @@
     }
     if (tile_raw >= n_tiles) return;
     uint32_t div_seq = 0;
+    [[maybe_unused]] uint32_t mk_next = 0xffffffffu;
     uint32_t n_posts = 0, n_waits = 0;
     uint32_t cref_row = p.stream_cref_first[stream];
 
@@ -255,6 +293,9 @@
     };
     const uint32_t B0 = p.stream_first[stream], NBND = B0 + p.stream_count[stream];
     if (NBND == B0) return;
+    if constexpr (MARKS) {
+        if (NS == 2 && p.spack_spacing != 0u) mk_next = B0 + p.spack_spacing < NBND - 1 ? B0 + p.spack_spacing : NBND - 1;
+    }
     auto clampb = [&](uint32_t b) { return b < NBND ? b : NBND - 1; };
     auto stage_rec = [&](uint32_t bundle) {
         dma16(lds0 + LDS_REC_OFF + (bundle % REC_AHEAD) * REC_BYTES, j16, rsrc_rec, bundle * (uint32_t)G * 16u);
@@ -324,6 +365,16 @@
         CWC_STAMP(st0);
         const uint32_t h = h_cur;
         asm volatile("s_waitcnt vmcnt(7)" ::: "memory");
+        if constexpr (MARKS) {
+            if (__builtin_expect(b == mk_next, 0)) {
+                typedef __attribute__((address_space(3))) uint32_t lds_u32;
+                volatile lds_u32* const mkw = reinterpret_cast<volatile lds_u32*>((lds_char*)(char*)lds + NW * AREA + NW * MB);
+                const uint32_t sp = (uint32_t)__builtin_amdgcn_readfirstlane((int)mkw[MK + NW]);
+                mk_next = b == NBND - 1 ? 0xffffffffu : b + sp < NBND - 1 ? b + sp : NBND - 1;
+                __builtin_amdgcn_fence(__ATOMIC_RELEASE, "workgroup");
+                mkw[MK + wave] = b + 1;
+            }
+        }
         CWC_STAMP(st1);
         if constexpr (COOP) {
             uint32_t cls_q = h & HDR_CLASS_MASK;
@@ -1212,8 +1263,16 @@
     dim3 grid((tiles + tiles_per_wg - 1) / tiles_per_wg), block((W ? (W + 1) * pack : pack) * 64);
     const uint4* in = (const uint4*)inputs;
     InterpDims dims{p.n_bundles, p.n_slots, p.n_inputs, batch, p.n_const, n_div_requests, p.trash_off, div_lanes, ns, {0, 0, 0, 0}, {0, 0, 0, 0}, {0, 0, 0, 0}, {0, 0, 0, 0},
-                    (uint4*)out, reinterpret_cast<const uint2*>(p.pack_entries), p.pack_ready, 0u, montgomery ? 1u : 0u, p.n_witness};
+                    (uint4*)out, reinterpret_cast<const uint2*>(p.pack_entries), p.pack_ready, 0u, montgomery ? 1u : 0u, p.n_witness,
+                    nullptr, 0u, 0u, 0u, 0u};
     if (W == 1 && ns == 1 && out && p.pack_entries && p.pack_ready) dims.n_inline = n_inline < p.n_ready_last ? n_inline : p.n_ready_last;
+    if (W == 1 && pack == 4 && ns == 2 && p.spack_spacing && p.spack_allowed) {
+        dims.spack_allowed = p.spack_allowed;
+        dims.spack_off1 = p.spack_off1;
+        dims.spack_spacing = p.spack_spacing;
+        dims.spack_stream = p.spack_stream;
+        if (out && p.pack_entries) dims.spack_n = n_inline < p.spack_n_vouched ? n_inline : p.spack_n_vouched;
+    }
     for (uint32_t s = 0; s < MAX_STREAMS; ++s) {
         dims.stream_first[s] = p.stream_first[s];
         dims.stream_count[s] = p.stream_count[s];
diff --git a/circom-witnesscalc_amd/csrc/pack_schedule.cc b/circom-witnesscalc_amd/csrc/pack_schedule.cc
--- a/circom-witnesscalc_amd/csrc/pack_schedule.cc
+++ b/circom-witnesscalc_amd/csrc/pack_schedule.cc
@@ -62,6 +62,120 @@
     return "";
 }
 
+
+static const uint32_t kMarkLag = 3;
+static const uint32_t kMarkSpacing = 256;
+static const double kStreamPackDoneBy = 0.97;
+
+std::string make_stream_pack_schedule(const Program& p, StreamPackSchedule& out) {
+    const uint32_t nw = p.n_witness, G = p.G;
+    out = StreamPackSchedule();
+    out.lag = kMarkLag;
+    out.order.resize(nw);
+    for (uint32_t i = 0; i < nw; ++i) out.order[i] = i;
+    out.need.assign(G ? ((size_t)nw + G - 1) / G : 0, STREAM_PACK_NEVER);
+    if (p.divider != 1 || p.n_streams != 2 || nw == 0 || G == 0 || p.n_bundles == 0) return "";
+    if (p.hdr.size() < p.n_bundles || p.recs.size() < (size_t)p.n_bundles * G * 4 || p.witness_refs.size() < nw) return "stream pack schedule: truncated program";
+    const uint32_t NS = 2;
+    uint32_t spacing = kMarkSpacing;
+    if (const char* e = getenv("CWC_STREAM_MARK_SPACING")) spacing = (uint32_t)std::min(1L << 20, std::max(4L, atol(e)));
+    out.spacing = spacing;
+    for (uint32_t s = 0; s < NS; ++s)
+        if ((uint64_t)p.stream_first[s] + p.stream_count[s] > p.n_bundles) return "stream pack schedule: a stream's bundles lie outside the program";
+    std::vector<double> clock(p.n_bundles, 0.0);
+    double work[NS], end[NS], scale[NS];
+    std::vector<double> req_time;
+    for (uint32_t s = 0; s < NS; ++s) {
+        const uint32_t b0 = p.stream_first[s], b1 = b0 + p.stream_count[s];
+        double lone = 0, sum = 0;
+        for (uint32_t b = b0; b < b1; ++b) {
+            const uint32_t cls = p.hdr[b] & HDR_CLASS_MASK;
+            lone += model_class_cycles((int)cls);
+            sum += model_class_cycles((int)cls) + (cls == C_DIVREQ ? model_class_cycles(C_DIV) : 0.0);
+            clock[b] = sum;
+        }
+        work[s] = sum;
+        end[s] = std::max(lone, sum * kTwoWavesPerSimd);
+        scale[s] = sum > 0 ? end[s] / sum : 1.0;
+        for (uint32_t b = b0 + spacing; b + 1 < b1; b += spacing) out.marks[s].push_back(b);
+        if (b1 > b0) out.marks[s].push_back(b1 - 1);
+        if (out.marks[s].size() >= 0xffffu) return "stream pack schedule: too many marks";
+    }
+    out.pack_stream = end[1] < end[0] ? 1u : 0u;
+    const double t_end = std::max(end[0], end[1]);
+    const uint64_t slot_bytes = 32ull * p.T, first_off = (uint64_t)p.n_const * slot_bytes, end_off = ((uint64_t)p.n_const + p.n_slots) * slot_bytes;
+    const uint32_t kNever = 0xffffffffu;
+    std::vector<uint32_t> producer[NS];
+    for (uint32_t s = 0; s < NS; ++s) {
+        producer[s].assign(p.n_slots, kNever);
+        for (uint32_t b = p.stream_first[s]; b < p.stream_first[s] + p.stream_count[s]; ++b)
+            for (uint32_t i = 0; i < G; ++i) {
+                const uint64_t dst = p.recs[((size_t)b * G + i) * 4 + 2] & ~CTRL_MASK;
+                if (dst >= first_off && dst < end_off) producer[s][(dst - first_off) / slot_bytes] = b;
+            }
+    }
+    std::vector<uint32_t> ev[NS];
+    std::vector<double> at(nw, 0.0);
+    for (uint32_t s = 0; s < NS; ++s) ev[s].assign(nw, 0u);
+    for (uint32_t w = 0; w < nw; ++w) {
+        const uint32_t ref = p.witness_refs[w];
+        if (ref & REF_CONST) continue;
+        const uint32_t slot = ref & ~REF_CANON;
+        if (slot >= p.n_slots || (producer[0][slot] == kNever && producer[1][slot] == kNever)) return "stream pack schedule: witness " + std::to_string(w) + " names a slot that no bundle writes";
+        for (uint32_t s = 0; s < NS; ++s) {
+            if (producer[s][slot] == kNever) continue;
+            const auto it = std::lower_bound(out.marks[s].begin(), out.marks[s].end(), producer[s][slot] + kMarkLag);
+            if (it == out.marks[s].end()) {
+                ev[s][w] = kNever;
+                at[w] = 1e300;
+            } else {
+                ev[s][w] = (uint32_t)(it - out.marks[s].begin()) + 1u;
+                at[w] = std::max(at[w], clock[*it] * scale[s]);
+            }
+        }
+    }
+    std::stable_sort(out.order.begin(), out.order.end(), [&](uint32_t a, uint32_t b) { return at[a] < at[b]; });
+    while (out.n_vouched < nw && at[out.order[out.n_vouched]] < 1e299) ++out.n_vouched;
+    std::vector<double> pass_ready(out.need.size(), 0.0);
+    {
+        uint32_t m[NS] = {0, 0};
+        double t = 0;
+        for (uint32_t i = 0; i < out.n_vouched; ++i) {
+            const uint32_t w = out.order[i];
+            for (uint32_t s = 0; s < NS; ++s) m[s] = std::max(m[s], ev[s][w]);
+            t = std::max(t, at[w]);
+            if ((i + 1) % G == 0 || i + 1 == out.n_vouched) {
+                out.need[i / G] = m[0] | m[1] << 16;
+                pass_ready[i / G] = t;
+            }
+        }
+    }
+    out.in_scope = true;
+    double pass_cycles = kCyclesPackPass;
+    if (const char* e = getenv("CWC_PACK_PASS_CYCLES")) pass_cycles = std::max(1.0, atof(e));
+    const uint32_t sp = out.pack_stream;
+    for (uint32_t b = p.stream_first[sp]; b < p.stream_first[sp] + p.stream_count[sp]; ++b)
+        if ((p.hdr[b] & HDR_CLASS_MASK) == C_DIVREQ) req_time.push_back((clock[b] - model_class_cycles(C_DIV)) * scale[sp]);
+    const double serve = model_class_cycles(C_DIV) * scale[sp], deadline = t_end * kStreamPackDoneBy;
+    double pw = 0, shared = 0;
+    size_t k = 0;
+    for (size_t g = 0; g * G < out.n_vouched; ++g) {
+        double start = std::max(pw, pass_ready[g]);
+        while (k < req_time.size() && req_time[k] <= start) {
+            pw = std::max(pw, req_time[k]) + serve;
+            start = std::max(pw, pass_ready[g]);
+            ++k;
+        }
+        const double fin = start + pass_cycles, with = shared + (start < end[sp] ? pass_cycles : 0.0);
+        if (fin > deadline || (work[sp] + with) * kTwoWavesPerSimd > deadline) break;
+        pw = fin;
+        shared = with;
+        out.n_inline = (uint32_t)std::min<size_t>((g + 1) * G, out.n_vouched);
+        out.pass_cycles += pass_cycles;
+    }
+    return "";
+}
+
 }
 
 static int schedule_out(const Program& p, uint32_t* pack_order, size_t order_cap, uint32_t* pack_ready, size_t ready_cap, uint32_t* n_witness, uint32_t* n_ready,
@@ -118,3 +232,64 @@
         return schedule_out(*p, pack_order, order_cap, pack_ready, ready_cap, n_witness, n_ready, n_inline, status);
     });
 }
+
+static int stream_schedule_out(const Program& p, uint32_t* pack_order, size_t order_cap, uint32_t* marks, size_t marks_cap, uint32_t* need, size_t need_cap, uint32_t* info,
+                               gw_status_t* status) {
+    StreamPackSchedule s;
+    const std::string err = make_stream_pack_schedule(p, s);
+    if (!err.empty()) return fail(status, err);
+    const size_t m0 = s.marks[0].size(), m1 = s.marks[1].size();
+    if (info) {
+        const uint32_t v[8] = {(uint32_t)s.order.size(), (uint32_t)m0, (uint32_t)m1, (uint32_t)s.need.size(), s.pack_stream, s.n_vouched, s.n_inline, s.lag};
+        memcpy(info, v, sizeof v);
+    }
+    if (pack_order && order_cap >= s.order.size() && !s.order.empty()) memcpy(pack_order, s.order.data(), s.order.size() * 4);
+    if (marks && marks_cap >= m0 + m1) {
+        if (m0) memcpy(marks, s.marks[0].data(), m0 * 4);
+        if (m1) memcpy(marks + m0, s.marks[1].data(), m1 * 4);
+    }
+    if (need && need_cap >= s.need.size() && !s.need.empty()) memcpy(need, s.need.data(), s.need.size() * 4);
+    set_status(status, OK, "");
+    return 0;
+}
+
+extern "C" int gwb_stream_pack_schedule_of_blob(const void* blob, size_t len, uint32_t* pack_order, size_t order_cap, uint32_t* marks, size_t marks_cap, uint32_t* need,
+                                                size_t need_cap, uint32_t* info, gw_status_t* status) {
+    return guarded(status, [&]() -> int {
+        if (!blob) return fail(status, "null argument");
+        if (len < 24 + 8) return fail(status, "bad blob: too short");
+        const uint8_t* b = (const uint8_t*)blob;
+        uint64_t tr[3];
+        memcpy(tr, b + len - 24, 24);
+        if (tr[2] != blob_checksum(b, len - 24)) return fail(status, "bad blob: checksum mismatch (truncated or corrupted)");
+        if (tr[0] > tr[1] || tr[1] > len - 24) return fail(status, "bad blob trailer");
+        Program p;
+        std::string err;
+        if (!program_from_blob(b, (size_t)tr[0], p, err) || !validate_program(p, err)) return fail(status, "bad program blob: " + err);
+        return stream_schedule_out(p, pack_order, order_cap, marks, marks_cap, need, need_cap, info, status);
+    });
+}
+
+extern "C" int gwb_stream_pack_schedule(gwb_graph_t* g, uint32_t program_key, uint32_t* pack_order, size_t order_cap, uint32_t* marks, size_t marks_cap, uint32_t* need,
+                                        size_t need_cap, uint32_t* info, gw_status_t* status) {
+    return guarded(status, [&]() -> int {
+        if (!g) return fail(status, "null argument");
+        std::lock_guard<std::mutex> lk(g->mu);
+        Program tmp;
+        const Program* p = nullptr;
+        if ((program_key & ~KEY_MODE_MASK) == 64) program_key = 64;
+        auto it = g->progs.find(program_key);
+        auto pre = g->compiled.find(program_key);
+        std::string err;
+        if (it != g->progs.end()) {
+            p = &it->second->host;
+        } else if (pre != g->compiled.end()) {
+            p = pre->second.get();
+        } else {
+            if (!g->has_graph) return fail(status, "imported handle has no program for that key");
+            if (!compile_program(g->graph, program_key & ~KEY_MODE_MASK, key_divider_waves(program_key), tmp, err, key_streams(program_key))) return fail(status, err);
+            p = &tmp;
+        }
+        return stream_schedule_out(*p, pack_order, order_cap, marks, marks_cap, need, need_cap, info, status);
+    });
+}
diff --git a/circom-witnesscalc_amd/csrc/pipeline.cc b/circom-witnesscalc_amd/csrc/pipeline.cc
--- a/circom-witnesscalc_amd/csrc/pipeline.cc
+++ b/circom-witnesscalc_amd/csrc/pipeline.cc
@@ -24,11 +24,15 @@
                  o_consts = o_crefs + al(p.crefs.size() * 4 + 256), o_wit = o_consts + al(p.consts.size() * 4 + 32),
                  o_div = o_wit + al(p.witness_refs.size() * 4 + 4), o_order = o_div + al(p.div_lanes.size() * 4 + 4),
                  o_entries = o_order + al(p.witness_refs.size() * 4 + 4), o_ready = o_entries + al((p.witness_refs.size() + PACK_ENTRY_PAD) * 8),
-                 total = o_ready + al(((size_t)p.n_div_requests + 1) * 4);
+                 o_marks = o_ready + al(((size_t)p.n_div_requests + 1) * 4);
     {
         const std::string serr = make_pack_schedule(p, dp.sched);
         if (!serr.empty()) return serr;
-    }
+        const std::string sserr = make_stream_pack_schedule(p, dp.ssched);
+        if (!sserr.empty()) return sserr;
+    }
+    const StreamPackSchedule& ss = dp.ssched;
+    const size_t total = o_marks + al((ss.marks[0].size() + ss.marks[1].size() + 2) * 4);
     HIP_TRY(hipMalloc(&dp.d_blob, total));
     char* d = (char*)dp.d_blob;
     HIP_TRY(hipMemset(d, 0, total));
@@ -62,12 +66,13 @@
             }
     {
         const PackSchedule& sc = dp.sched;
-        std::vector<uint32_t> entries(sc.order.size() * 2);
-        for (size_t i = 0; i < sc.order.size(); ++i) {
-            entries[2 * i] = sc.order[i];
-            entries[2 * i + 1] = p.witness_refs[sc.order[i]];
-        }
-        if (!sc.order.empty()) HIP_TRY(hipMemcpy(d + o_order, sc.order.data(), sc.order.size() * 4, hipMemcpyHostToDevice));
+        const std::vector<uint32_t>& order = ss.in_scope ? ss.order : sc.order;
+        std::vector<uint32_t> entries(order.size() * 2);
+        for (size_t i = 0; i < order.size(); ++i) {
+            entries[2 * i] = order[i];
+            entries[2 * i + 1] = p.witness_refs[order[i]];
+        }
+        if (!order.empty()) HIP_TRY(hipMemcpy(d + o_order, order.data(), order.size() * 4, hipMemcpyHostToDevice));
         if (!entries.empty()) HIP_TRY(hipMemcpy(d + o_entries, entries.data(), entries.size() * 4, hipMemcpyHostToDevice));
         HIP_TRY(hipMemcpy(d + o_ready, sc.ready.data(), sc.ready.size() * 4, hipMemcpyHostToDevice));
         dp.dev.pack_order = (const uint32_t*)(d + o_order);
@@ -75,6 +80,33 @@
         dp.dev.pack_ready = (const uint32_t*)(d + o_ready);
         dp.dev.n_inline = sc.n_inline;
         dp.dev.n_ready_last = sc.ready.back();
+        dp.dev.spack_allowed = nullptr;
+        dp.dev.spack_off1 = 0;
+        dp.dev.spack_spacing = dp.dev.spack_stream = dp.dev.spack_n_inline = dp.dev.spack_n_vouched = 0;
+        if (ss.in_scope) {
+            for (uint32_t s = 0; s < 2; ++s) {
+                std::vector<uint32_t> want;
+                const uint32_t b0 = p.stream_first[s], b1 = b0 + p.stream_count[s];
+                for (uint32_t b = b0 + ss.spacing; b + 1 < b1; b += ss.spacing) want.push_back(b);
+                if (b1 > b0) want.push_back(b1 - 1);
+                if (want != ss.marks[s]) return "stream pack schedule: the marks of a stream are not evenly spaced";
+            }
+            std::vector<uint32_t> allowed;
+            for (uint32_t s = 0; s < 2; ++s) {
+                if (s == 1) dp.dev.spack_off1 = (uint32_t)allowed.size();
+                size_t g = 0;
+                for (uint32_t m = 0; m <= ss.marks[s].size(); ++m) {
+                    while (g < ss.need.size() && ss.need[g] != STREAM_PACK_NEVER && ((ss.need[g] >> (16 * s)) & 0xffffu) <= m) ++g;
+                    allowed.push_back((uint32_t)std::min<size_t>(g * p.G, ss.n_vouched));
+                }
+            }
+            HIP_TRY(hipMemcpy(d + o_marks, allowed.data(), allowed.size() * 4, hipMemcpyHostToDevice));
+            dp.dev.spack_allowed = (const uint32_t*)(d + o_marks);
+            dp.dev.spack_spacing = ss.spacing;
+            dp.dev.spack_stream = ss.pack_stream;
+            dp.dev.spack_n_inline = ss.n_inline;
+            dp.dev.spack_n_vouched = ss.n_vouched;
+        }
     }
     dp.dev.n_streams = p.n_streams;
     for (uint32_t s = 0; s < MAX_STREAMS; ++s) {
@@ -147,15 +179,20 @@
     if (p.n_streams > 1) {
         const double tiles = (double)((batch + p.T - 1) / p.T);
         if (stream_pair_workgroups(p.divider, (uint64_t)tiles, p.n_streams)) {
-            constexpr double kTwoWaves = 0.62, kPackCyclesPerValue = 0.028;
+            constexpr double kTwoWaves = kTwoWavesPerSimd, kPackCyclesPerValue = 0.028;
+            StreamPackSchedule ss;
+            const char* sw = getenv("CWC_STREAM_PACK");
+            const bool inline_share = p.T <= 2 && !(sw && atoi(sw) <= 0) && make_stream_pack_schedule(p, ss).empty() && ss.in_scope;
+            const uint32_t n_in = inline_share ? (sw && atoi(sw) >= 2 ? ss.n_vouched : ss.n_inline) : 0u;
+            const double in_cycles = inline_share ? (ss.n_inline ? ss.pass_cycles * (double)n_in / (double)ss.n_inline : 0.0) : 0.0;
             double t = 0;
             for (uint32_t s = 0; s < p.n_streams; ++s) {
                 const double own = std::max(p.stream_cycles[s], p.stream_chain_cycles[s]);
-                const double simd = (p.stream_cycles[s] + model_class_cycles(C_DIV) * p.stream_div_requests[s]) * kTwoWaves;
+                const double simd = (p.stream_cycles[s] + model_class_cycles(C_DIV) * p.stream_div_requests[s] + (inline_share && s == ss.pack_stream ? in_cycles : 0.0)) * kTwoWaves;
                 t = std::max(t, std::max(own, simd));
             }
             const double rounds = std::max(1.0, tiles / 512.0);
-            return t * (p.T >= 4 ? 1.2 * wide : 1.0) * rounds + kPackCyclesPerValue * (double)p.n_witness * (double)batch;
+            return t * (p.T >= 4 ? 1.2 * wide : 1.0) * rounds + kPackCyclesPerValue * (double)(p.n_witness - n_in) * (double)batch;
         }
         const double t = program_wave_cycles(p);
         double busy = 0;
@@ -461,6 +498,9 @@
     uint32_t n_inline = kInlinePackDefault ? dp->dev.n_inline : 0u;
     if (const char* e = getenv("CWC_INLINE_PACK")) n_inline = atoi(e) >= 2 ? dp->dev.n_ready_last : atoi(e) == 1 ? dp->dev.n_inline : 0u;
     if (const char* e = getenv("CWC_INLINE_PACK_ROWS")) n_inline = std::min<uint32_t>(n_inline, (uint32_t)atol(e));
+    uint32_t n_stream_inline = dp->dev.spack_spacing ? dp->dev.spack_n_inline : 0u;
+    if (const char* e = getenv("CWC_STREAM_PACK")) n_stream_inline = !dp->dev.spack_spacing || atoi(e) <= 0 ? 0u : atoi(e) >= 2 ? dp->dev.spack_n_vouched : dp->dev.spack_n_inline;
+    if (const char* e = getenv("CWC_STREAM_PACK_ROWS")) n_stream_inline = std::min<uint32_t>(n_stream_inline, (uint32_t)atol(e));
     const size_t launch_sets = per_launch * chunk_sets;
     for (size_t s0 = 0; s0 < batch; s0 += launch_sets) {
         const uint32_t nb = (uint32_t)((batch - s0) < launch_sets ? (batch - s0) : launch_sets);
@@ -485,10 +525,12 @@
         g->pending.push_back(gwb_graph::ChunkEvents{e0, e1, e2});
         HIP_TRY(hipEventRecord(e0, stream));
         void* const out = (char*)d_witness + s0 * (size_t)p.n_witness * 32;
-        HIP_TRY(launch_interp(T, p.divider, waves_per_workgroup(p.divider, (nb + T - 1) / T, p.n_streams), p.n_div_requests, dp->dev.div_lanes, dp->dev, wst, (const char*)d_inputs + s0 * p.n_inputs * 32, d_status + s0, nb, stream, g->d_prof,
-                              out, n_inline, montgomery));
+        const uint32_t wpw = waves_per_workgroup(p.divider, (nb + T - 1) / T, p.n_streams);
+        const uint32_t n_in = p.n_streams == 2 && p.divider == 1 ? (wpw == 4 ? n_stream_inline : 0u) : n_inline;
+        HIP_TRY(launch_interp(T, p.divider, wpw, p.n_div_requests, dp->dev.div_lanes, dp->dev, wst, (const char*)d_inputs + s0 * p.n_inputs * 32, d_status + s0, nb, stream, g->d_prof,
+                              out, n_in, montgomery));
         HIP_TRY(hipEventRecord(e1, stream));
-        HIP_TRY(launch_pack(T, dp->dev, wst, out, nb, stream, montgomery, n_inline));
+        HIP_TRY(launch_pack(T, dp->dev, wst, out, nb, stream, montgomery, n_in));
         HIP_TRY(hipEventRecord(e2, stream));
         g->last_call_launches++;
         g->timing.n_launches++;
@@ -649,6 +691,7 @@
     std::string s;
     if (bits & ST_SHL_OVERFLOW) s += "Shl result does not fit the field (reference panics at graph.rs:634)";
     if (bits & 0x80000000u) s += std::string(s.empty() ? "" : "; ") + "internal error: divider mailbox wait timed out";
+    if (bits & 0x20000000u) s += std::string(s.empty() ? "" : "; ") + "internal error: the packing wave's wait for a progress mark timed out";
     if (bits & 0x40000000u) s += std::string(s.empty() ? "" : "; ") + "internal error: wait for another stream's post timed out";
     if (bits & ST_BITOP_EQ_R) s += std::string(s.empty() ? "" : "; ") + "bit operation result equals the modulus (reference panics at graph.rs:686/701/716)";
     return s;
diff --git a/circom-witnesscalc_amd/csrc/program_dev.h b/circom-witnesscalc_amd/csrc/program_dev.h
--- a/circom-witnesscalc_amd/csrc/program_dev.h
+++ b/circom-witnesscalc_amd/csrc/program_dev.h
@@ -91,6 +91,10 @@
     const uint32_t* pack_entries;
     const uint32_t* pack_ready;
     uint32_t n_inline, n_ready_last;
+    const uint32_t* spack_allowed;
+    uint32_t spack_off1;
+    uint32_t spack_spacing;
+    uint32_t spack_stream, spack_n_inline, spack_n_vouched;
 };
 static const uint32_t PACK_ENTRY_PAD = 192;
 
diff --git a/circom-witnesscalc_amd/csrc/runtime_internal.hpp b/circom-witnesscalc_amd/csrc/runtime_internal.hpp
--- a/circom-witnesscalc_amd/csrc/runtime_internal.hpp
+++ b/circom-witnesscalc_amd/csrc/runtime_internal.hpp
@@ -70,10 +70,26 @@
     uint32_t n_inline = 0;
 };
 std::string make_pack_schedule(const Program& p, PackSchedule& out);
+struct StreamPackSchedule {
+    bool in_scope = false;
+    std::vector<uint32_t> order;
+    std::vector<uint32_t> marks[MAX_STREAMS];
+    std::vector<uint32_t> need;
+    uint32_t spacing = 0;
+    uint32_t lag = 0;
+    uint32_t pack_stream = 0;
+    uint32_t n_vouched = 0;
+    uint32_t n_inline = 0;
+    double pass_cycles = 0;
+};
+static const uint32_t STREAM_PACK_NEVER = 0xffffffffu;
+constexpr double kTwoWavesPerSimd = 0.62;
+std::string make_stream_pack_schedule(const Program& p, StreamPackSchedule& out);
 
 struct DeviceProgram {
     Program host;
     PackSchedule sched;
+    StreamPackSchedule ssched;
     void* d_blob = nullptr;
     ProgramDev dev{};
     DeviceProgram() = default;
diff --git a/include/graph_witness_batch.h b/include/graph_witness_batch.h
--- a/include/graph_witness_batch.h
+++ b/include/graph_witness_batch.h
@@ -134,6 +134,11 @@
 int gwb_pack_schedule_of_blob(const void *blob, size_t blob_len, uint32_t *pack_order, size_t order_cap, uint32_t *pack_ready, size_t ready_cap,
                               uint32_t *n_witness, uint32_t *n_ready, uint32_t *n_inline, gw_status_t *status);
 
+int gwb_stream_pack_schedule(gwb_graph_t *g, uint32_t program_key, uint32_t *pack_order, size_t order_cap, uint32_t *marks, size_t marks_cap,
+                             uint32_t *need, size_t need_cap, uint32_t *info, gw_status_t *status);
+int gwb_stream_pack_schedule_of_blob(const void *blob, size_t blob_len, uint32_t *pack_order, size_t order_cap, uint32_t *marks, size_t marks_cap,
+                                     uint32_t *need, size_t need_cap, uint32_t *info, gw_status_t *status);
+
 size_t gwb_wtns_size(size_t n_witness);
 int gwb_wtns_from_witness(const void *witness_row, size_t n_witness, void *out);
 
```

New measurement: 90120. 0.964x the previous value.
